# tenpy/cyten

Measured on AMD Instinct MI355X. Metric: block-sparse tdot+SVD GFLOP/s (fp64), higher is better.
Workload: dtype f64

## Files before the change

### cyten_amd/csrc/blocked_qr.hip

```cpp
#include "blocked_qr.h"

#include <algorithm>
#include <cstdlib>
#include <utility>

namespace cyb {
namespace {

#define GLOBAL_AS __attribute__((address_space(1)))
typedef GLOBAL_AS double* gp;
typedef const GLOBAL_AS double* gcp;
typedef double d4 __attribute__((ext_vector_type(4)));

constexpr int PNT = 512;
constexpr int PNW = PNT / 64;

__device__ __forceinline__ double wave_sum(double v)
{
#pragma unroll
    for (int o = 32; o > 0; o >>= 1) v += __shfl_xor(v, o);
    return v;
}

struct PanelDesc {
// ... 866 lines not shown
            if (tid == 0) {
                __builtin_amdgcn_fence(__ATOMIC_RELEASE, "agent");
                __hip_atomic_store(la_flags + (d.next_off - 1), la_tag, __ATOMIC_RELAXED, __HIP_MEMORY_SCOPE_AGENT);
            }
        }
    }
    if constexpr (FUSE_PANEL) {
        __shared__ PanelShared psh;
        if (d.next_off) {
            __syncthreads();
            const PanelDesc pd = *reinterpret_cast<const PanelDesc*>(reinterpret_cast<const char*>(descs) + d.next_off);
            panel_reg_body<RP_RPT_FUSED>(pd, psh, tid);
        }
    }
}

struct ChunkDesc {
    double* C;
    const double* V;
    const double* T;
    double* wpart;
    int64_t ldc, ldv;
    int32_t mr, nc, pw, transT;
    int32_t slot, n_slots, row0, step;
    const double* ctl;
    double* part_out;
};

__global__ void __launch_bounds__(ST_NT) strip_w1_kernel(const ChunkDesc* __restrict__ descs)
{
    __shared__ double part[ST_NW][NBK][ST_LS];
    const ChunkDesc d = descs[blockIdx.x];
    if (d.ctl) {
        const double stopped = *(gcp)d.ctl;
        if (stopped != 0.0 && (double)d.step >= stopped - 1.0) return;
    }
    const int tid = threadIdx.x, lane = tid & 63, wave = tid >> 6;
    const int x = lane & 15, kq = lane >> 4;
    gcp V = (gcp)d.V;
    gp C = (gp)d.C;
    const int mr = d.mr, nc = d.nc, pw = d.pw;
    const int64_t ldv = d.ldv, ldc = d.ldc;
    {
        const int64_t vo0 = (int64_t)(x < pw ? x : 0) * ldv, vo1 = (int64_t)(x + 16 < pw ? x + 16 : 0) * ldv;
        const int64_t co0 = (int64_t)(x < nc ? x : 0) * ldc, co1 = (int64_t)(x + 16 < nc ? x + 16 : 0) * ldc;
        d4 acc[2][2];
#pragma unroll
        for (int i = 0; i < 2; ++i)
#pragma unroll
            for (int j = 0; j < 2; ++j) acc[i][j] = d4{0.0, 0.0, 0.0, 0.0};
        const int nstep = (mr + 7) / 8;
        double va[ST_UN][2][2], ca[ST_UN][2][2], vn[ST_UN][2][2], cn[ST_UN][2][2];
        auto load = [&](double (&v)[ST_UN][2][2], double (&c)[ST_UN][2][2], int s0) {
#pragma unroll
            for (int u = 0; u < ST_UN; ++u) {
                const int i = (s0 + ST_NW * u) * 8 + 2 * kq;
#pragma unroll
                for (int h = 0; h < 2; ++h) {
                    const bool ok = i + h < mr;
                    const int ii = ok ? i + h : 0;
                    v[u][0][h] = ok ? V[vo0 + ii] : 0.0;
                    v[u][1][h] = ok ? V[vo1 + ii] : 0.0;
                    c[u][0][h] = ok ? C[co0 + ii] : 0.0;
                    c[u][1][h] = ok ? C[co1 + ii] : 0.0;
                }
            }
        };
        if (wave < nstep) load(va, ca, wave);
        for (int s0 = wave; s0 < nstep; s0 += ST_NW * ST_UN) {
            const bool more = s0 + ST_NW * ST_UN < nstep;
            if (more) load(vn, cn, s0 + ST_NW * ST_UN);
#pragma unroll
            for (int u = 0; u < ST_UN; ++u) {
                if (s0 + ST_NW * u < nstep) {
#pragma unroll
                    for (int h = 0; h < 2; ++h)
#pragma unroll
                        for (int i = 0; i < 2; ++i)
#pragma unroll
                            for (int j = 0; j < 2; ++j)
                                acc[i][j] = __builtin_amdgcn_mfma_f64_16x16x4f64(va[u][i][h], ca[u][j][h], acc[i][j], 0, 0, 0);
                }
            }
            if (more) {
#pragma unroll
                for (int u = 0; u < ST_UN; ++u)
#pragma unroll
                    for (int i = 0; i < 2; ++i)
#pragma unroll
                        for (int h = 0; h < 2; ++h) {
                            va[u][i][h] = vn[u][i][h];
                            ca[u][i][h] = cn[u][i][h];
                        }
            }
        }
#pragma unroll
        for (int i = 0; i < 2; ++i)
#pragma unroll
            for (int j = 0; j < 2; ++j)
#pragma unroll
                for (int r = 0; r < 4; ++r) part[wave][i * 16 + kq + 4 * r][j * 16 + x] = acc[i][j][r];
    }
    __syncthreads();
    gp out = (gp)d.wpart + (size_t)d.slot * (NBK * NBK);
    for (int e = tid; e < NBK * NBK; e += ST_NT) {
        const int a = e / NBK, c = e % NBK;
        double t = 0.0;
#pragma unroll
        for (int w = 0; w < ST_NW; ++w) t += part[w][a][c];
        out[e] = t;
    }
}

template <bool NORM>
__global__ void __launch_bounds__(ST_NT) strip_apply_kernel(const ChunkDesc* __restrict__ descs)
{
    __shared__ double W1s[NBK][ST_LS], W2s[NBK][ST_LS], Ps[NBK][ST_LS];
    const ChunkDesc d = descs[blockIdx.x];
    if (d.ctl) {
        const double stopped = *(gcp)d.ctl;
        if (stopped != 0.0 && (double)d.step >= stopped - 1.0) return;
    }
    const int tid = threadIdx.x, lane = tid & 63, wave = tid >> 6;
    const int x = lane & 15, kq = lane >> 4;
    gcp V = (gcp)d.V;
    gp C = (gp)d.C;
    gcp T = (gcp)d.T;
    const int mr = d.mr, nc = d.nc, pw = d.pw;
    const int64_t ldv = d.ldv, ldc = d.ldc;
    gcp wp = (gcp)d.wpart;
    for (int e = tid; e < NBK * NBK; e += ST_NT) {
        const int a = e / NBK, b = e % NBK;
        Ps[a][b] = T[d.transT ? b * NBK + a : e];
        double t = 0.0;
        for (int sl = 0; sl < d.n_slots; ++sl) t += wp[(size_t)sl * (NBK * NBK) + e];
        W1s[a][b] = t;
    }
    __syncthreads();
    if (wave < 4) {
        const int ta = wave >> 1, tc = wave & 1;
        d4 acc = d4{0.0, 0.0, 0.0, 0.0};
#pragma unroll
        for (int kk = 0; kk < NBK / 4; ++kk)
            acc = __builtin_amdgcn_mfma_f64_16x16x4f64(Ps[ta * 16 + x][4 * kk + kq], W1s[4 * kk + kq][tc * 16 + x], acc, 0, 0, 0);
#pragma unroll
        for (int r = 0; r < 4; ++r) W2s[ta * 16 + kq + 4 * r][tc * 16 + x] = acc[r];
    }
    __syncthreads();
    {
        double w2[2][NBK / 4];
#pragma unroll
        for (int ct = 0; ct < 2; ++ct)
#pragma unroll
            for (int kk = 0; kk < NBK / 4; ++kk) w2[ct][kk] = -W2s[4 * kk + kq][ct * 16 + x];
        int64_t vcol[NBK / 4], ccol[2][4];
#pragma unroll
        for (int kk = 0; kk < NBK / 4; ++kk) vcol[kk] = (int64_t)(4 * kk + kq < pw ? 4 * kk + kq : 0) * ldv;
#pragma unroll
        for (int ct = 0; ct < 2; ++ct)
#pragma unroll
            for (int r = 0; r < 4; ++r) {
                const int c = ct * 16 + kq + 4 * r;
                ccol[ct][r] = (int64_t)(c < nc ? c : 0) * ldc;
            }
        const int ntile = (mr + 15) / 16;
        struct Tile {
            double v[NBK / 4];
            d4 c[2];
        };
        auto load = [&](Tile& t, int rt) {
            const int i = rt * 16 + x;
            const bool ok = i < mr;
            const int ii = ok ? i : 0;
#pragma unroll
            for (int kk = 0; kk < NBK / 4; ++kk) t.v[kk] = ok ? V[vcol[kk] + ii] : 0.0;
#pragma unroll
            for (int ct = 0; ct < 2; ++ct)
#pragma unroll
                for (int r = 0; r < 4; ++r) t.c[ct][r] = C[ccol[ct][r] + ii];
        };
        double nrm2 = 0.0;
        auto finish = [&](Tile& t, int rt) {
#pragma unroll
            for (int kk = 0; kk < NBK / 4; ++kk) {
                t.c[0] = __builtin_amdgcn_mfma_f64_16x16x4f64(w2[0][kk], t.v[kk], t.c[0], 0, 0, 0);
                t.c[1] = __builtin_amdgcn_mfma_f64_16x16x4f64(w2[1][kk], t.v[kk], t.c[1], 0, 0, 0);
            }
            const int i = rt * 16 + x;
            if (i < mr) {
                const double below = i + d.row0 >= pw ? 1.0 : 0.0;
#pragma unroll
                for (int ct = 0; ct < 2; ++ct)
#pragma unroll
                    for (int r = 0; r < 4; ++r)
                        if (ct * 16 + kq + 4 * r < nc) {
                            C[ccol[ct][r] + i] = t.c[ct][r];
                            if constexpr (NORM) nrm2 = fma(below * t.c[ct][r], t.c[ct][r], nrm2);
                        }
            }
        };
        Tile t0, t1, t2;
        if (wave < ntile) load(t0, wave);
        if (wave + ST_NW < ntile) load(t1, wave + ST_NW);
        for (int rt = wave; rt < ntile; rt += 3 * ST_NW) {
            if (rt + 2 * ST_NW < ntile) load(t2, rt + 2 * ST_NW);
            finish(t0, rt);
            if (rt + ST_NW < ntile) {
                if (rt + 3 * ST_NW < ntile) load(t0, rt + 3 * ST_NW);
                finish(t1, rt + ST_NW);
            }
            if (rt + 2 * ST_NW < ntile) {
                if (rt + 4 * ST_NW < ntile) load(t1, rt + 4 * ST_NW);
                finish(t2, rt + 2 * ST_NW);
            }
        }
        if constexpr (NORM) if (d.part_out) {
#pragma unroll
            for (int o = 32; o > 0; o >>= 1) nrm2 += __shfl_xor(nrm2, o);
            __syncthreads();
            if (lane == 0) W1s[0][wave] = nrm2;
            __syncthreads();
            if (tid == 0) {
                double t = 0.0;
#pragma unroll
                for (int w = 0; w < ST_NW; ++w) t += W1s[0][w];
                *(gp)d.part_out = t;
            }
        }
    }
}

struct MergeDesc {
    const double* G;
    const double* T;
    double* TS;
    int64_t g_stride;
    int32_t w, W, n_gp, pad;
};
constexpr int MG_NT = 256;
template <int AMAX>
__global__ void __launch_bounds__(MG_NT) merge_t_kernel(const MergeDesc* __restrict__ descs)
{
    constexpr bool TS_LDS = AMAX <= 96;
    __shared__ double Gs[AMAX][NBK + 1], X[AMAX][NBK + 1];
    __shared__ double Tb[NBK][NBK + 1];
    __shared__ double TSs[TS_LDS ? AMAX : 1][TS_LDS ? AMAX + 1 : 1];
    const MergeDesc d = descs[blockIdx.x];
    const int tid = threadIdx.x;
    const int W = d.W, w = d.w;
    gcp G = (gcp)d.G;
    gcp T = (gcp)d.T;
    gp TS = (gp)d.TS;
    for (int e = tid; e < W * W; e += MG_NT) {
        const int r = e / W, c = e % W;
        double v = 0.0;
        if (r / NBK == c / NBK && r < w && c < w) v = T[(size_t)(r / NBK) * (NBK * NBK) + (r % NBK) * NBK + (c % NBK)];
        TS[e] = v;
        if constexpr (TS_LDS)
            if (r < AMAX && c < AMAX) TSs[r][c] = v;
    }
    const int nb = (w + NBK - 1) / NBK;
    for (int b = 1; b < nb; ++b) {
        const int a = b * NBK, wb = min(NBK, w - a);
        __syncthreads();
        for (int e = tid; e < NBK * NBK; e += MG_NT) Tb[e / NBK][e % NBK] = T[(size_t)b * (NBK * NBK) + e];
        for (int e = tid; e < a * NBK; e += MG_NT) {
            const int i = e / NBK, l = e % NBK;
            double g = 0.0;
            if (l < wb)
                for (int p = 0; p < d.n_gp; ++p) g += G[(size_t)p * d.g_stride + (size_t)i * W + a + l];
            Gs[i][l] = g;
        }
        __syncthreads();
        for (int e = tid; e < a * NBK; e += MG_NT) {
            const int i = e / NBK, c = e % NBK;
            double acc = 0.0;
#pragma unroll
            for (int l = 0; l < NBK; ++l) acc += Gs[i][l] * Tb[l][c];
            X[i][c] = acc;
        }
        __syncthreads();
        for (int e = tid; e < a * NBK; e += MG_NT) {
            const int i = e / NBK, c = e % NBK;
            double acc = 0.0;
            if constexpr (TS_LDS) {
                for (int l = i; l < a; ++l) acc += TSs[i][l] * X[l][c];
            } else {
                for (int l = i; l < a; ++l) acc += TS[(size_t)i * W + l] * X[l][c];
            }
            if (c < wb) {
                TS[(size_t)i * W + a + c] = -acc;
                if constexpr (TS_LDS)
                    if (a + c < AMAX) TSs[i][a + c] = -acc;
            }
        }
    }
}

struct SumDesc {
    double* W1;
    int64_t n, stride;
    int32_t ns, pad;
};
__global__ void __launch_bounds__(256) sum_partials_kernel(const SumDesc* __restrict__ descs)
{
    const SumDesc d = descs[blockIdx.y];
    gp W1 = (gp)d.W1;
    for (int64_t e = (int64_t)blockIdx.x * 256 + threadIdx.x; e < d.n; e += (int64_t)gridDim.x * 256) {
        double t = W1[e];
        for (int sidx = 1; sidx < d.ns; ++sidx) t += W1[e + (int64_t)sidx * d.stride];
        W1[e] = t;
    }
}

inline size_t al256(size_t b) { return (b + 255) / 256 * 256; }

__global__ void __launch_bounds__(256) xpose_kernel(const XposeDesc* __restrict__ descs)
{
    __shared__ double tile[32][33];
    const XposeDesc d = descs[blockIdx.y];
    gcp in = (gcp)d.in;
    gp out = (gp)d.out;
    const int tx = threadIdx.x & 31, ty = threadIdx.x >> 5;
    if (d.plain) {
        const int64_t tot = (int64_t)d.R * d.C;
        for (int64_t e = (int64_t)blockIdx.x * 256 + threadIdx.x; e < tot; e += (int64_t)gridDim.x * 256) {
            const int64_t r = e / d.C, c = e % d.C;
            out[r * d.ldo + c] = in[r * d.ldi + c];
        }
        return;
    }
    const int tr = (d.R + 31) / 32, tc = (d.C + 31) / 32;
    for (int t = blockIdx.x; t < tr * tc; t += gridDim.x) {
        const int r0 = (t / tc) * 32, c0 = (t % tc) * 32;
        __syncthreads();
#pragma unroll
        for (int q = 0; q < 4; ++q) {
            const int c = c0 + ty + 8 * q, r = r0 + tx;
            tile[ty + 8 * q][tx] = (c < d.C && r < d.R) ? in[(int64_t)c * d.ldi + r] : 0.0;
        }
        __syncthreads();
#pragma unroll
        for (int q = 0; q < 4; ++q) {
            const int r = r0 + ty + 8 * q, c = c0 + tx;
            if (r < d.R && c < d.C) {
                double v = tile[tx][ty + 8 * q];
                if (d.upper && (r > c || r >= d.rlim)) v = 0.0;
                out[(int64_t)r * d.ldo + c] = v;
            }
        }
    }
}

__global__ void __launch_bounds__(256) eye_cols_kernel(const EyeDesc* __restrict__ descs)
{
    const EyeDesc d = descs[blockIdx.y];
    gp C = (gp)d.C;
    const int64_t tot = (int64_t)d.m * d.kc;
    for (int64_t e = (int64_t)blockIdx.x * 256 + threadIdx.x; e < tot; e += (int64_t)gridDim.x * 256) {
        const int64_t c = e / d.m, i = e % d.m;
        C[c * d.ld + i] = (i == c + d.col0) ? 1.0 : 0.0;
    }
}

}

int xpose_batched(cyb_ctx_t ctx, const std::vector<XposeDesc>& descs)
{
    if (descs.empty()) return CYB_OK;
    void* d = nullptr;
    CYB_TRY(ctx->upload(descs.data(), sizeof(XposeDesc) * descs.size(), &d));
    hipLaunchKernelGGL(xpose_kernel, dim3(helper_grid_x(descs.size()), (unsigned)descs.size()), dim3(256), 0, ctx->stream, static_cast<const XposeDesc*>(d));
    CYB_HIP(hipGetLastError());
    return CYB_OK;
}

int eye_cols_batched(cyb_ctx_t ctx, const std::vector<EyeDesc>& descs)
{
    if (descs.empty()) return CYB_OK;
    void* d = nullptr;
    CYB_TRY(ctx->upload(descs.data(), sizeof(EyeDesc) * descs.size(), &d));
    hipLaunchKernelGGL(eye_cols_kernel, dim3(64, (unsigned)descs.size()), dim3(256), 0, ctx->stream, static_cast<const EyeDesc*>(d));
    CYB_HIP(hipGetLastError());
    return CYB_OK;
}

constexpr int kWSplit = 8;
static inline int w_split(int64_t mr)
{
    static const int env = getenv("CYB_QR_WSPLIT") ? atoi(getenv("CYB_QR_WSPLIT")) : 0;
    if (env > 0) return (int)std::min<int64_t>(std::min(env, kWSplit), std::max<int64_t>(1, (mr + 255) / 256));
    return mr >= 2600 ? 4 : mr >= 1800 ? 3 : mr >= 700 ? 2 : 1;
}

static inline bool use_strips()
{
    static const bool off = getenv("CYB_QR_GEMM_UPDATE") != nullptr;
    return !off;
}
static void add_strips(std::vector<StripDesc>& out, double* C, int64_t ldc, int64_t ncols, const double* V, int64_t ldv,
                       const double* T, int64_t mr, int pw, int transT, int64_t next_tag = -1)
{
    for (int64_t c0 = 0; c0 < ncols; c0 += NBK)
        out.push_back(StripDesc{C + (size_t)c0 * ldc, V, T, ldc, ldv, (int32_t)mr, (int32_t)std::min<int64_t>(NBK, ncols - c0), pw, transT,
                                c0 == 0 && next_tag >= 0 ? next_tag + 1 : 0});
}
static void sort_strips(std::vector<StripDesc>& v)
{
    std::stable_sort(v.begin(), v.end(), [](const StripDesc& a, const StripDesc& b) { return a.mr > b.mr; });
}

constexpr int kChunkRowsMin = 192;
static const int kChunkRowsChoices[] = {192, 256, 384, 512, 768, 1024, 1536};
static int strip_split_mode()
{
    static const int v = getenv("CYB_QR_CHUNK_ROWS") ? atoi(getenv("CYB_QR_CHUNK_ROWS")) : -1;
    return v < 0 ? -1 : v / 16 * 16;
}
int bqr_strip_slots(int64_t rows)
{
    if (strip_split_mode() == 0) return 1;
    const int ch = strip_split_mode() > 0 ? std::min(strip_split_mode(), kChunkRowsMin) : kChunkRowsMin;
    return (int)std::max<int64_t>(1, (rows + ch - 1) / ch);
}
static int strip_chunk_share(int mr, int ch)
{
    if (ch <= 0 || mr <= ch) return std::max(mr, 1);
    const int ns = (mr + ch - 1) / ch;
    return ((mr + ns - 1) / ns + 15) / 16 * 16;
}
static int strip_chunks(int mr, int ch)
{
    const int share = strip_chunk_share(mr, ch);
    return std::max(1, (mr + share - 1) / share);
}
static int choose_chunk_rows(const std::vector<std::pair<int, int>>& strips, int n_cu)
{
    const int mode = strip_split_mode();
    if (mode == 0) return 0;
    if (mode > 0) return mode;
    int64_t n_strips = 0;
    for (const auto& s : strips) n_strips += s.second;
    if (n_strips == 0 || n_strips * 4 > (int64_t)n_cu * 3) return 0;
    static const int ch_min = getenv("CYB_QR_CHUNK_MIN") ? atoi(getenv("CYB_QR_CHUNK_MIN")) : kChunkRowsMin;
    for (int ch : kChunkRowsChoices) {
        if (ch < ch_min) continue;
        int64_t tot = 0;
        bool any = false;
        for (const auto& s : strips) {
            const int c = strip_chunks(s.first, ch);
            tot += (int64_t)c * s.second;
            any = any || c > 1;
        }
        if (tot <= n_cu) return any ? ch : 0;
    }
    return 0;
}
static void make_chunks(const std::vector<StripDesc>& sd, double* wbase, int ch, std::vector<ChunkDesc>& out)
{
    out.clear();
    size_t slot_base = 0;
    for (const StripDesc& d : sd) {
        const int share = strip_chunk_share(d.mr, ch), nch = strip_chunks(d.mr, ch);
        for (int sl = 0; sl < nch; ++sl) {
            const int r0 = sl * share;
            out.push_back(ChunkDesc{d.C + r0, d.V + r0, d.T, wbase + slot_base * (size_t)(NBK * NBK), d.ldc, d.ldv, std::min(share, d.mr - r0), d.nc, d.pw,
                                    d.transT, sl, nch, r0, d.step, d.ctl, d.part_out ? d.part_out + sl : nullptr});
        }
        slot_base += (size_t)nch;
    }
}

static int wide_mode()
{
    static const int v = getenv("CYB_QR_APPLY_WIDE") ? (atoi(getenv("CYB_QR_APPLY_WIDE")) != 0 ? 1 : 0) : -1;
    return v;
}
static int wide_width()
{
    static const int v = [] {
        const int e = getenv("CYB_QR_APPLY_WIDTH") ? atoi(getenv("CYB_QR_APPLY_WIDTH")) : 128;
        return (e == 64 || e == 256) ? e : 128;
    }();
    return v;
}
constexpr int64_t kWideMinK = 256, kWideMinKc = 256, kWideMinCols = 4096;
static bool wide_target(const BqrMat& q, const BqrTarget& t)
{
    const int mode = wide_mode();
    if (mode == 0 || q.k <= NBK || t.kc <= 0) return false;
    if (q.ctl && q.stop_rel2 > 0.0 && t.n_pan < 0) return false;
    if (mode == 1) return true;
    return q.k >= kWideMinK && t.kc >= kWideMinKc;
}
static size_t scratch_doubles(int64_t m, int64_t n, int64_t kc)
{
    const size_t strips = (size_t)(1 + kWSplit) * NBK * (size_t)std::max<int64_t>(std::max(n, kc), 1);
    const size_t wide = (size_t)w_split(m) * (size_t)wide_width() * (size_t)std::max<int64_t>(kc, 1);
    return std::max(strips, wide);
}

size_t bqr_aux_bytes(int64_t m, int64_t n, int64_t ld, int64_t kc)
{
    const int64_t k = std::min(m, n);
    const int64_t npan = (k + NBK - 1) / NBK;
    return al256(sizeof(double) * (size_t)ld * (size_t)std::max<int64_t>(k, 1)) + al256(sizeof(double) * (size_t)npan * NBK * NBK) +
           al256(sizeof(double) * (size_t)std::max<int64_t>(k, 1)) + al256(sizeof(double) * scratch_doubles(m, n, kc));
}

size_t bqr_carve(BqrMat& q, char* base, int64_t kc)
{
    const int64_t k = q.k;
    const int64_t npan = (k + NBK - 1) / NBK;
    size_t off = 0;
    q.V = reinterpret_cast<double*>(base + off);
    off += al256(sizeof(double) * (size_t)q.ld * (size_t)std::max<int64_t>(k, 1));
    q.T = reinterpret_cast<double*>(base + off);
    off += al256(sizeof(double) * (size_t)npan * NBK * NBK);
    q.tau = reinterpret_cast<double*>(base + off);
    off += al256(sizeof(double) * (size_t)std::max<int64_t>(k, 1));
    q.scratch = reinterpret_cast<double*>(base + off);
    q.scr_half = (int64_t)NBK * std::max<int64_t>(std::max<int64_t>(q.n, kc), 1);
    q.scr_total = (int64_t)scratch_doubles(q.m, q.n, kc);
    off += al256(sizeof(double) * (size_t)q.scr_total);
    return off;
}

int bqr_factor(cyb_ctx_t ctx, const std::vector<BqrMat>& mats)
{
    auto pflags = [](const BqrMat& q) { return (q.v_zeroed ? PANEL_V_ZEROED : 0) | (q.reflect_always ? PANEL_REFLECT_ALWAYS : 0); };
    int max_pan = 0;
    for (const auto& q : mats) max_pan = std::max(max_pan, (q.k + NBK - 1) / NBK);
    static const bool want_la = getenv("CYB_QR_LOOKAHEAD") != nullptr;
    hipStream_t side = nullptr;
    const bool strips = use_strips();
    const bool lookahead = !strips && want_la && max_pan >= 6 && ctx->aux(&side) == CYB_OK;
    struct Step {
        size_t off_pd = 0, off_pdr = 0;
        unsigned n_pd = 0, n_pdr = 0;
        GemmStaged s1, s3;
        GemmStaged r1, r3;
        bool has_rest = false;
        size_t off_sd = 0;
        unsigned n_sd = 0;
        bool fused = false;
        bool norm = false;
        unsigned n_la = 0;
        size_t off_pn = 0;
        size_t off_cd = 0;
        unsigned n_cd = 0;
        int wave = 0;
        size_t off_pdm = 0;
        unsigned n_pdm = 0;
    };
    std::vector<Step> steps;
    std::vector<char> image;
    auto put = [&image](const void* src, size_t bytes) {
        const size_t off = (image.size() + 255) / 256 * 256;
        image.resize(off + bytes);
        memcpy(image.data() + off, src, bytes);
        return off;
    };
    static const bool no_fuse = getenv("CYB_QR_FUSE") == nullptr;
    static const int fuse_rows = getenv("CYB_QR_FUSE_ROWS") ? atoi(getenv("CYB_QR_FUSE_ROWS")) : 768;
    std::vector<char> fused(mats.size(), 0);
    static const bool la_on = getenv("CYB_QR_LA") && atoi(getenv("CYB_QR_LA")) != 0;
    static const int la_min_rows = getenv("CYB_QR_LA_MIN") ? atoi(getenv("CYB_QR_LA_MIN")) : 4 * RP_WAVE_ROWS;
    unsigned int* la_flags = nullptr;
    const int la_err = (int)mats.size();
    bool la_used = false;
    static const bool no_multi = getenv("CYB_QR_NOMULTI") != nullptr;
    std::vector<size_t> x_off(mats.size(), 0);
    size_t x_bytes = 0, n_multi_wg = 0;
    const size_t t_bytes = (sizeof(unsigned int) * NBK * mats.size() + 255) / 256 * 256;
    for (size_t qi = 0; qi < mats.size(); ++qi) {
        const int wmax = (mats[qi].m + RPM_ROWS - 1) / RPM_ROWS;
        if (mats[qi].m > RPM_ROWS && std::min(mats[qi].m, mats[qi].n) > 0) {
            x_off[qi] = t_bytes + 256 + x_bytes;
            x_bytes += sizeof(double) * NBK * (size_t)wmax * 64;
            n_multi_wg += (size_t)wmax;
        }
    }
    const bool multi = !no_multi && x_bytes > 0 && n_multi_wg <= (size_t)ctx->n_cu;
    char* xbase = nullptr;
    bool la_any = false;
    if (la_on && use_strips())
        for (const auto& q : mats) la_any = la_any || (q.k > NBK && q.m - NBK > la_min_rows);
    if (multi || la_any) {
        const size_t x_total = multi ? (t_bytes + 256 + x_bytes + 255) / 256 * 256 : 0;
        void* xw = nullptr;
        CYB_TRY(ctx->workspace(x_total + 256 + sizeof(unsigned int) * (mats.size() + 1), &xw, 3));
        xbase = static_cast<char*>(xw);
        if (multi) CYB_HIP(hipMemsetAsync(xbase + t_bytes, 0, 256, ctx->stream));
        if (la_any) {
            la_flags = reinterpret_cast<unsigned int*>(xbase + x_total);
            CYB_HIP(hipMemsetAsync(la_flags, 0, sizeof(unsigned int) * (mats.size() + 1), ctx->stream));
        }
    }
    const bool multi_ok = multi;
    static const bool no_stop = getenv("CYB_QR_NOSTOP") != nullptr;
    static const bool no_reg_g = getenv("CYB_QR_PANEL_GLOBAL") != nullptr;
    auto stoppable = [&](const BqrMat& q) {
        return !no_stop && strips && !no_reg_g && q.ctl && q.parts && q.stop_rel2 > 0.0 && (q.m <= RP_NT * RP_RPT || multi_ok);
    };
    const bool split = strips && strip_split_mode() != 0 && no_fuse && !la_on;
    double* wsplit = nullptr;
    if (split) {
        size_t n_ch = 0;
        for (const auto& q : mats) n_ch += (size_t)((q.n + NBK - 1) / NBK) * (size_t)bqr_strip_slots(q.m);
        void* w = nullptr;
        CYB_TRY(ctx->workspace(sizeof(double) * NBK * NBK * std::max<size_t>(n_ch, 1), &w, 4));
        wsplit = static_cast<double*>(w);
    }
    std::vector<int> n_parts_prev(mats.size(), 0);
    static const int stop_every = std::max(1, getenv("CYB_QR_STOP_EVERY") ? atoi(getenv("CYB_QR_STOP_EVERY")) : 2);
    bool all_done = false;
    int last_rest = -1;
    const int side_cu = ctx->n_cu - (ctx->n_cu + 15) / 16;
    int chunk = lookahead ? max_pan : 2;
    for (int c0 = 0; c0 < max_pan && !all_done; c0 += chunk, chunk *= 3) {
    const int c1 = std::min(max_pan, c0 + chunk);
    steps.clear();
    image.clear();
    for (int p = c0; p < c1; ++p) {
        std::vector<PanelDesc> pd, pd_reg, pd_next;
        std::vector<PanelDescM> pdm;
        std::vector<StripDesc> sd;
        GemmBatch g1, g3, h1, h3;
        int n_active = 0;
        int max_m = 0;
        for (const auto& q : mats)
            if (p * NBK < q.k) max_m = std::max(max_m, q.m);
        const bool step_fuse = !no_fuse && max_m <= fuse_rows;
        const bool step_la = la_on && strips && !step_fuse && la_flags != nullptr;
        bool step_has_la = false;
        bool step_norm = false;
        int step_ch = 0;
        if (split && !step_fuse) {
            std::vector<std::pair<int, int>> cnt;
            for (const auto& q : mats) {
                const int j0 = p * NBK;
                if (j0 >= q.k) continue;
                const int64_t nt = q.n - (j0 + std::min(NBK, q.k - j0));
                if (nt > 0) cnt.push_back({q.m - j0, (int)((nt + NBK - 1) / NBK)});
            }
            step_ch = choose_chunk_rows(cnt, ctx->n_cu);
        }
        for (size_t qi = 0; qi < mats.size(); ++qi) {
            const auto& q = mats[qi];
            const int j0 = p * NBK;
            if (j0 >= q.k) continue;
            ++n_active;
            const int pw = std::min(NBK, q.k - j0);
            static const bool no_reg = getenv("CYB_QR_PANEL_GLOBAL") != nullptr;
            if (fused[qi]) fused[qi] = 0;
            else if (!no_reg && q.m - j0 <= RP_NT * RP_RPT) {
                pd_reg.push_back(PanelDesc{q.Ac, q.V, q.T + (size_t)p * NBK * NBK, q.tau, q.ld, q.m, j0, pw, pflags(q)});
                if (stoppable(q)) {
                    PanelDesc& d = pd_reg.back();
                    d.ctl = q.ctl;
                    d.parts = q.parts;
                    d.rel2 = q.stop_rel2;
                    d.n_parts = n_parts_prev[qi];
                    d.step = p;
                }
            } else if (multi && !no_reg) {
                const int n_wg = (q.m - j0 + RPM_ROWS - 1) / RPM_ROWS;
                for (int w = 0; w < n_wg; ++w)
                {
                    pdm.push_back(PanelDescM{q.Ac, q.V, q.T + (size_t)p * NBK * NBK, q.tau, reinterpret_cast<double*>(xbase + x_off[qi]),
                                             reinterpret_cast<unsigned int*>(xbase) + qi * NBK, reinterpret_cast<unsigned int*>(xbase + t_bytes),
                                             q.ld, q.m, j0, pw, pflags(q), w, n_wg, 0, 0});
                    if (stoppable(q)) {
                        PanelDescM& d = pdm.back();
                        d.ctl = q.ctl;
                        d.parts = q.parts;
                        d.rel2 = q.stop_rel2;
                        d.n_parts = n_parts_prev[qi];
                        d.step = p;
                    }
                }
            } else
                pd.push_back(PanelDesc{q.Ac, q.V, q.T + (size_t)p * NBK * NBK, q.tau, q.ld, q.m, j0, pw, pflags(q) & PANEL_REFLECT_ALWAYS});
            const int j1 = j0 + pw;
            const int64_t nt = q.n - j1, mr = q.m - j0;
// ... 106 lines not shown
            CYB_TRY(h3.stage(ctx, image, st.r3));
            st.has_rest = true;
        }
        steps.push_back(st);
    }
    if (steps.empty()) break;
    void* d_image = nullptr;
    CYB_TRY(ctx->upload(image.data(), image.size(), &d_image));
    char* dbase = static_cast<char*>(d_image);
    if (lookahead) CYB_TRY(ctx->events(2 * steps.size()));
    for (size_t p = 0; p < steps.size(); ++p) {
        const Step& st = steps[p];
        if (st.n_pd)
            hipLaunchKernelGGL(qr_panel_kernel, dim3(st.n_pd), dim3(PNT), 0, ctx->stream,
                               reinterpret_cast<const PanelDesc*>(dbase + st.off_pd));
        if (st.n_pdm) {
            CYB_HIP(hipMemsetAsync(xbase, 0, t_bytes, ctx->stream));
            hipLaunchKernelGGL(qr_panel_multi_kernel, dim3(st.n_pdm), dim3(RP_NT), 0, ctx->stream,
                               reinterpret_cast<const PanelDescM*>(dbase + st.off_pdm));
        }
        if (st.n_pdr && st.wave == 1)
            hipLaunchKernelGGL(qr_panel_wave_kernel, dim3(st.n_pdr), dim3(64), 0, ctx->stream,
                               reinterpret_cast<const PanelDesc*>(dbase + st.off_pdr));
        else if (st.n_pdr && st.wave == 2)
            hipLaunchKernelGGL(qr_panel_wave2_kernel, dim3(st.n_pdr), dim3(128), 0, ctx->stream,
                               reinterpret_cast<const PanelDesc*>(dbase + st.off_pdr));
        else if (st.n_pdr && st.wave == 4)
            hipLaunchKernelGGL(qr_panel_wave4_kernel, dim3(st.n_pdr), dim3(256), 0, ctx->stream,
                               reinterpret_cast<const PanelDesc*>(dbase + st.off_pdr));
        else if (st.n_pdr)
            hipLaunchKernelGGL(qr_panel_reg_kernel, dim3(st.n_pdr), dim3(RP_NT), 0, ctx->stream,
                               reinterpret_cast<const PanelDesc*>(dbase + st.off_pdr));
        CYB_HIP(hipGetLastError());
        if (lookahead && st.has_rest) {
            hipEvent_t evP = ctx->ev_pool[2 * p], evR = ctx->ev_pool[2 * p + 1];
            CYB_HIP(hipEventRecord(evP, ctx->stream));
            CYB_HIP(hipStreamWaitEvent(side, evP, 0));
            CYB_TRY(gemm_launch_staged(ctx, st.r1, d_image, side, side_cu));
            CYB_TRY(gemm_launch_staged(ctx, st.r3, d_image, side, side_cu));
            CYB_HIP(hipEventRecord(evR, side));
            if (last_rest >= 0) CYB_HIP(hipStreamWaitEvent(ctx->stream, ctx->ev_pool[2 * (size_t)last_rest + 1], 0));
            last_rest = (int)p;
        } else if (lookahead && last_rest >= 0) {
            CYB_HIP(hipStreamWaitEvent(ctx->stream, ctx->ev_pool[2 * (size_t)last_rest + 1], 0));
            last_rest = -1;
        }
        if (st.n_sd) {
            const StripDesc* sdp = reinterpret_cast<const StripDesc*>(dbase + st.off_sd);
            const PanelDesc* pnp = reinterpret_cast<const PanelDesc*>(dbase + st.off_pn);
            const unsigned la_tag = (unsigned)(c0 + (int)p + 1);
            const PanelDesc* no_pn = nullptr;
            unsigned int* no_fl = nullptr;
            if (st.n_cd) {
                const ChunkDesc* cdp = reinterpret_cast<const ChunkDesc*>(dbase + st.off_cd);
                hipLaunchKernelGGL(strip_w1_kernel, dim3(st.n_cd), dim3(ST_NT), 0, ctx->stream, cdp);
                if (st.norm) hipLaunchKernelGGL(strip_apply_kernel<true>, dim3(st.n_cd), dim3(ST_NT), 0, ctx->stream, cdp);
                else hipLaunchKernelGGL(strip_apply_kernel<false>, dim3(st.n_cd), dim3(ST_NT), 0, ctx->stream, cdp);
            } else if (st.n_la && st.norm)
                hipLaunchKernelGGL((reflector_strip_kernel<false, true, true>), dim3(st.n_sd + st.n_la), dim3(ST_NT), 0, ctx->stream, sdp,
                                   (int)st.n_sd, pnp, la_flags, la_tag, la_err);
            else if (st.n_la)
                hipLaunchKernelGGL((reflector_strip_kernel<false, false, true>), dim3(st.n_sd + st.n_la), dim3(ST_NT), 0, ctx->stream, sdp,
                                   (int)st.n_sd, pnp, la_flags, la_tag, la_err);
            else if (st.fused)
                hipLaunchKernelGGL(reflector_strip_kernel<true>, dim3(st.n_sd), dim3(ST_NT), 0, ctx->stream, sdp, (int)st.n_sd, no_pn, no_fl, 0u, 0);
            else if (st.norm)
                hipLaunchKernelGGL((reflector_strip_kernel<false, true>), dim3(st.n_sd), dim3(ST_NT), 0, ctx->stream, sdp, (int)st.n_sd, no_pn, no_fl, 0u, 0);
            else
                hipLaunchKernelGGL(reflector_strip_kernel<false>, dim3(st.n_sd), dim3(ST_NT), 0, ctx->stream, sdp, (int)st.n_sd, no_pn, no_fl, 0u, 0);
            CYB_HIP(hipGetLastError());
        }
        CYB_TRY(gemm_launch_staged(ctx, st.s1, d_image));
        CYB_TRY(gemm_launch_staged(ctx, st.s3, d_image));
    }
    }
    if (last_rest >= 0) CYB_HIP(hipStreamWaitEvent(ctx->stream, ctx->ev_pool[2 * (size_t)last_rest + 1], 0));
    if (la_used) {
        unsigned int h_err = 0;
        CYB_HIP(hipMemcpyAsync(&h_err, la_flags + la_err, sizeof(unsigned int), hipMemcpyDeviceToHost, ctx->stream));
        CYB_HIP(hipStreamSynchronize(ctx->stream));
        if (h_err) {
            set_error("blocked QR: a look-ahead panel workgroup waited more than a second for its strip");
            return CYB_ERR_HIP;
        }
    }
    if (multi) {
        unsigned int h_err = 0;
        CYB_HIP(hipMemcpyAsync(&h_err, xbase + t_bytes, sizeof(unsigned int), hipMemcpyDeviceToHost, ctx->stream));
        CYB_HIP(hipStreamSynchronize(ctx->stream));
        if (h_err) {
            set_error("blocked QR: a workgroup of the multi-workgroup panel kernel waited more than a second for its partners");
            return CYB_ERR_HIP;
        }
    }
    return CYB_OK;
}

static int apply_q_strips(cyb_ctx_t ctx, const std::vector<BqrMat>& mats, const std::vector<BqrTarget>& targets)
{
    int max_pan = 0;
    for (const auto& t : targets) max_pan = std::max(max_pan, (mats[(size_t)t.mat].k + NBK - 1) / NBK);
    const bool strips = use_strips();
    struct Step {
        GemmStaged s1, s3;
        size_t off_sd = 0;
        unsigned n_sd = 0;
        size_t off_cd = 0;
        unsigned n_cd = 0;
    };
    const bool split = strips && strip_split_mode() != 0;
    double* wsplit = nullptr;
    if (split) {
        size_t n_ch = 0;
        for (const auto& t : targets) n_ch += (size_t)((t.kc + NBK - 1) / NBK) * (size_t)bqr_strip_slots(mats[(size_t)t.mat].m);
        void* w = nullptr;
        CYB_TRY(ctx->workspace(sizeof(double) * NBK * NBK * std::max<size_t>(n_ch, 1), &w, 4));
        wsplit = static_cast<double*>(w);
    }
    std::vector<Step> steps;
    std::vector<char> image;
    int chunk = 2;
    for (int c0 = max_pan - 1; c0 >= 0; c0 -= chunk, chunk *= 3) {
    const int c1 = std::max(-1, c0 - chunk);
    steps.clear();
    image.clear();
    for (int p = c0; p > c1; --p) {
        GemmBatch g1, g3;
        std::vector<StripDesc> sd;
        for (const auto& t : targets) {
            const BqrMat& q = mats[(size_t)t.mat];
            const int j0 = p * NBK;
            if (j0 >= q.k || t.kc <= 0) continue;
            const int pw = std::min(NBK, q.k - j0);
            const int64_t mr = q.m - j0;
            double* W1 = q.scratch + q.scr_half;
            CYB_REQUIRE((int64_t)NBK * t.kc <= q.scr_half, "bqr_apply_q: target wider than the carved scratch");
            const double* Vp = q.V + (size_t)j0 * q.ld + j0;
            double* Ct = t.C + j0;
            const double* Tp = q.T + (size_t)p * NBK * NBK;
            if (strips) {
                const size_t s_begin = sd.size();
                add_strips(sd, Ct, t.ldc, t.kc, Vp, q.ld, Tp, mr, pw, 0);
                if (q.ctl && q.stop_rel2 > 0.0)
                    for (size_t si = s_begin; si < sd.size(); ++si) {
                        sd[si].ctl = q.ctl;
                        sd[si].step = p;
                    }
                continue;
            }
            const int ns = w_split(mr);
            const int64_t chunk = ((mr + ns - 1) / ns + 15) / 16 * 16;
            const int32_t seg0 = (int32_t)g3.segs.size();
            for (int sidx = 0; sidx < ns; ++sidx) {
                const int64_t r0 = chunk * sidx, rows = std::min(chunk, mr - r0);
                if (rows <= 0) break;
                double* W2s = W1 + (size_t)sidx * q.scr_half;
                g1.add_post(W2s, pw, t.kc, t.kc, Vp + r0, q.ld, 1, Ct + r0, 1, t.ldc, rows, 1.0, 0.0, Tp, NBK, 1);
                g3.segs.push_back(cyb_gemm_seg{W2s, Vp, pw, 1, t.kc, q.ld, 1});
            }
            g3.probs.push_back(cyb_gemm_prob{Ct, t.kc, mr, t.ldc, seg0, (int32_t)g3.segs.size(), -1.0, 1.0});
        }
        if (g1.empty() && sd.empty()) continue;
        Step st;
        if (!g1.empty()) {
            CYB_TRY(g1.stage(ctx, image, st.s1));
            CYB_TRY(g3.stage(ctx, image, st.s3));
        }
        if (!sd.empty()) {
            sort_strips(sd);
            st.n_sd = (unsigned)sd.size();
            const size_t off = (image.size() + 255) / 256 * 256;
            image.resize(off + sizeof(StripDesc) * sd.size());
            memcpy(image.data() + off, sd.data(), sizeof(StripDesc) * sd.size());
            st.off_sd = off;
            std::vector<std::pair<int, int>> cnt;
            for (const auto& d : sd) cnt.push_back({d.mr, 1});
            const int step_ch = split ? choose_chunk_rows(cnt, ctx->n_cu) : 0;
            if (step_ch > 0) {
                std::vector<ChunkDesc> cd;
                make_chunks(sd, wsplit, step_ch, cd);
                st.n_cd = (unsigned)cd.size();
                const size_t offc = (image.size() + 255) / 256 * 256;
                image.resize(offc + sizeof(ChunkDesc) * cd.size());
                memcpy(image.data() + offc, cd.data(), sizeof(ChunkDesc) * cd.size());
                st.off_cd = offc;
            }
        }
        steps.push_back(st);
    }
    if (steps.empty()) continue;
    void* d_image = nullptr;
    CYB_TRY(ctx->upload(image.data(), image.size(), &d_image));
    for (const auto& st : steps) {
        if (st.n_cd) {
            const ChunkDesc* cdp = reinterpret_cast<const ChunkDesc*>(static_cast<char*>(d_image) + st.off_cd);
            hipLaunchKernelGGL(strip_w1_kernel, dim3(st.n_cd), dim3(ST_NT), 0, ctx->stream, cdp);
            hipLaunchKernelGGL(strip_apply_kernel<false>, dim3(st.n_cd), dim3(ST_NT), 0, ctx->stream, cdp);
            CYB_HIP(hipGetLastError());
        } else if (st.n_sd) {
            hipLaunchKernelGGL(reflector_strip_kernel<false>, dim3(st.n_sd), dim3(ST_NT), 0, ctx->stream,
                               reinterpret_cast<const StripDesc*>(static_cast<char*>(d_image) + st.off_sd), (int)st.n_sd,
                               static_cast<const PanelDesc*>(nullptr), static_cast<unsigned int*>(nullptr), 0u, 0);
            CYB_HIP(hipGetLastError());
        }
        CYB_TRY(gemm_launch_staged(ctx, st.s1, d_image));
        CYB_TRY(gemm_launch_staged(ctx, st.s3, d_image));
    }
    }
    return CYB_OK;
}

static int apply_q_wide(cyb_ctx_t ctx, const std::vector<BqrMat>& mats, const std::vector<BqrTarget>& targets)
{
    const int W = wide_width();
    struct Tgt {
        const BqrMat* q;
        const BqrTarget* t;
        int k_eff, ng;
        double* VT;
        double* TS;
        double* G;
        std::vector<int> n_gp;
    };
    std::vector<Tgt> tg;
    size_t bytes = 0;
    int max_ng = 0;
    for (const auto& t : targets) {
        const BqrMat& q = mats[(size_t)t.mat];
        const int npan = (q.k + NBK - 1) / NBK;
        const int nf = t.n_pan >= 0 ? std::min(npan, (int)t.n_pan) : npan;
        const int k_eff = std::min<int>(q.k, nf * NBK);
        if (k_eff <= 0 || t.kc <= 0) continue;
        Tgt g{&q, &t, k_eff, (k_eff + W - 1) / W, nullptr, nullptr, nullptr, {}};
        CYB_REQUIRE((int64_t)w_split(q.m) * W * t.kc <= q.scr_total, "bqr_apply_q: target wider than the carved scratch");
        for (int s = 0; s < g.ng; ++s) {
            const int j0 = s * W, w = std::min(W, k_eff - j0);
            const int min_rows = q.m - j0 - (w - 1) / NBK * NBK;
            g.n_gp.push_back(std::max(1, std::min(4, min_rows / 256)));
        }
        max_ng = std::max(max_ng, g.ng);
        tg.push_back(std::move(g));
    }
    if (tg.empty()) return CYB_OK;
    std::vector<size_t> o_vt(tg.size()), o_ts(tg.size()), o_g(tg.size());
    for (size_t i = 0; i < tg.size(); ++i) {
        size_t n_g = 0;
        for (int n : tg[i].n_gp) n_g += (size_t)n;
        o_vt[i] = bytes;
        bytes += al256(sizeof(double) * (size_t)tg[i].q->ld * (size_t)tg[i].k_eff);
        o_ts[i] = bytes;
        bytes += al256(sizeof(double) * (size_t)tg[i].ng * W * W);
        o_g[i] = bytes;
        bytes += al256(sizeof(double) * n_g * W * W);
    }
    void* ws = nullptr;
    CYB_TRY(ctx->workspace(bytes, &ws, 5));
    for (size_t i = 0; i < tg.size(); ++i) {
        tg[i].VT = reinterpret_cast<double*>(static_cast<char*>(ws) + o_vt[i]);
        tg[i].TS = reinterpret_cast<double*>(static_cast<char*>(ws) + o_ts[i]);
        tg[i].G = reinterpret_cast<double*>(static_cast<char*>(ws) + o_g[i]);
    }
    std::vector<char> image;
    {
        GemmBatch gg, gv;
        std::vector<MergeDesc> md;
        for (const Tgt& g : tg) {
            const BqrMat& q = *g.q;
            size_t gp0 = 0;
            for (int s = 0; s < g.ng; ++s) {
                const int j0 = s * W, w = std::min(W, g.k_eff - j0), n_gp = g.n_gp[(size_t)s];
                const double* Vs = q.V + (size_t)j0 * q.ld + j0;
                double* Gs = g.G + gp0 * (size_t)W * W;
                double* TSs = g.TS + (size_t)s * W * W;
                for (int a = NBK; a < w; a += NBK) {
                    const int wb = std::min(NBK, w - a);
                    const int64_t rows = q.m - j0 - a, chunk = (rows + n_gp - 1) / n_gp;
                    for (int p = 0; p < n_gp; ++p) {
                        const int64_t r0 = a + chunk * p, kr = std::min(chunk, rows - chunk * p);
                        gg.add(Gs + (size_t)p * W * W + a, a, wb, W, Vs + r0, q.ld, 1, Vs + (size_t)a * q.ld + r0, 1, q.ld, kr, 1.0, 0.0);
                    }
                }
                md.push_back(MergeDesc{Gs, q.T + (size_t)(j0 / NBK) * NBK * NBK, TSs, (int64_t)W * W, w, W, n_gp, 0});
                gv.add(g.VT + (size_t)j0 * q.ld + j0, w, q.m - j0, q.ld, TSs, 1, W, Vs, q.ld, 1, w, 1.0, 0.0);
                gp0 += (size_t)n_gp;
            }
        }
        GemmStaged sg, sv;
        CYB_TRY(gg.stage(ctx, image, sg));
        CYB_TRY(gv.stage(ctx, image, sv));
        const size_t off_md = (image.size() + 255) / 256 * 256;
        image.resize(off_md + sizeof(MergeDesc) * md.size());
        memcpy(image.data() + off_md, md.data(), sizeof(MergeDesc) * md.size());
        void* d_image = nullptr;
        CYB_TRY(ctx->upload(image.data(), image.size(), &d_image));
        CYB_TRY(gemm_launch_staged(ctx, sg, d_image));
        const MergeDesc* mdp = reinterpret_cast<const MergeDesc*>(static_cast<char*>(d_image) + off_md);
        if (W <= 128) hipLaunchKernelGGL(merge_t_kernel<96>, dim3((unsigned)md.size()), dim3(MG_NT), 0, ctx->stream, mdp);
        else hipLaunchKernelGGL(merge_t_kernel<224>, dim3((unsigned)md.size()), dim3(MG_NT), 0, ctx->stream, mdp);
        CYB_HIP(hipGetLastError());
        CYB_TRY(gemm_launch_staged(ctx, sv, d_image));
    }
    struct Step {
        GemmStaged s1, s2;
        size_t off_sum = 0;
        unsigned n_sum = 0;
    };
    std::vector<Step> steps;
    int chunk = 2;
    for (int c0 = max_ng - 1; c0 >= 0; c0 -= chunk, chunk *= 3) {
        const int c1 = std::max(-1, c0 - chunk);
        steps.clear();
        image.clear();
        for (int s = c0; s > c1; --s) {
            GemmBatch g1, g2;
            std::vector<SumDesc> sums;
            for (const Tgt& g : tg) {
                if (s >= g.ng) continue;
                const BqrMat& q = *g.q;
                const BqrTarget& t = *g.t;
                const int j0 = s * W, w = std::min(W, g.k_eff - j0);
                const int64_t mr = q.m - j0;
                const double* Vs = q.V + (size_t)j0 * q.ld + j0;
                const double* VTs = g.VT + (size_t)j0 * q.ld + j0;
                double* Ct = t.C + j0;
                const int ns = w_split(mr);
                const int64_t rch = ((mr + ns - 1) / ns + 15) / 16 * 16;
                const int64_t stride = (int64_t)W * t.kc;
                int n_part = 0;
                for (int sidx = 0; sidx < ns; ++sidx) {
                    const int64_t r0 = rch * sidx, rows = std::min(rch, mr - r0);
                    if (rows <= 0) break;
                    g1.add(q.scratch + (size_t)sidx * (size_t)stride, w, t.kc, t.kc, Vs + r0, q.ld, 1, Ct + r0, 1, t.ldc, rows, 1.0, 0.0);
                    ++n_part;
                }
                if (n_part > 1) sums.push_back(SumDesc{q.scratch, (int64_t)w * t.kc, stride, n_part, 0});
                g2.add(Ct, t.kc, mr, t.ldc, q.scratch, 1, t.kc, VTs, q.ld, 1, w, -1.0, 1.0);
            }
            if (g1.empty()) continue;
            Step st;
            CYB_TRY(g1.stage(ctx, image, st.s1));
            CYB_TRY(g2.stage(ctx, image, st.s2));
            if (!sums.empty()) {
                st.n_sum = (unsigned)sums.size();
                st.off_sum = (image.size() + 255) / 256 * 256;
                image.resize(st.off_sum + sizeof(SumDesc) * sums.size());
                memcpy(image.data() + st.off_sum, sums.data(), sizeof(SumDesc) * sums.size());
            }
            steps.push_back(st);
        }
        if (steps.empty()) continue;
        void* d_image = nullptr;
        CYB_TRY(ctx->upload(image.data(), image.size(), &d_image));
        for (const auto& st : steps) {
            CYB_TRY(gemm_launch_staged(ctx, st.s1, d_image));
            if (st.n_sum) {
                hipLaunchKernelGGL(sum_partials_kernel, dim3(helper_grid_x(st.n_sum), st.n_sum), dim3(256), 0, ctx->stream,
                                   reinterpret_cast<const SumDesc*>(static_cast<char*>(d_image) + st.off_sum));
                CYB_HIP(hipGetLastError());
            }
            CYB_TRY(gemm_launch_staged(ctx, st.s2, d_image));
        }
    }
    return CYB_OK;
}

int bqr_apply_q(cyb_ctx_t ctx, const std::vector<BqrMat>& mats, const std::vector<BqrTarget>& targets)
{
    std::vector<BqrTarget> narrow, wide;
    for (const auto& t : targets) (wide_target(mats[(size_t)t.mat], t) ? wide : narrow).push_back(t);
    int64_t cols = 0;
    for (const auto& t : wide) cols += t.kc;
    if (wide_mode() < 0 && cols < kWideMinCols) {
        narrow = targets;
        wide.clear();
    }
    if (!narrow.empty()) CYB_TRY(apply_q_strips(ctx, mats, narrow));
    if (!wide.empty()) CYB_TRY(apply_q_wide(ctx, mats, wide));
    return CYB_OK;
}

}
```

### cyten_amd/csrc/common.h

```cpp
#pragma once
#include <hip/hip_runtime.h>
#include <cstdarg>
#include <cstdint>
#include <cstdio>
#include <cstring>
#include <string>
#include <initializer_list>
#include <vector>

#include "../../include/cyten_amd.h"

namespace cyb {

void set_error(const char* fmt, ...);

#define CYB_HIP(call)                                                                   \
    do {                                                                                \
        hipError_t _e = (call);                                                         \
        if (_e != hipSuccess) {                                                         \
            cyb::set_error("%s failed: %s (%s:%d)", #call, hipGetErrorString(_e),       \
                           __FILE__, __LINE__);                                         \
            return CYB_ERR_HIP;                                                         \
        }                                                                               \
    } while (0)

#define CYB_REQUIRE(cond, ...)                                                          \
    do {                                                                                \
        if (!(cond)) {                                                                  \
            cyb::set_error(__VA_ARGS__);                                                \
            return CYB_ERR_INVALID;                                                     \
        }                                                                               \
    } while (0)

#define CYB_TRY(call)                                                                   \
    do {                                                                                \
        int _s = (call);                                                                \
        if (_s != CYB_OK) return _s;                                                    \
    } while (0)

}

struct cyb_ctx_s {
    int device = 0;
    hipStream_t stream = nullptr;
    int n_cu = 256;
    int lds_bytes = 160 * 1024;
    int64_t hbm_bytes = 0;
    char arch[64] = {0};

    static constexpr int kSlots = 32;
    static constexpr int kEvStride = 8;
    struct Slot {
        void* dev = nullptr;
        void* host = nullptr;
        size_t cap = 0;
        hipEvent_t ev = nullptr;
        hipEvent_t copied = nullptr;
        bool ev_valid = false;
    };
    hipStream_t copy_stream = nullptr;
    hipStream_t aux_stream = nullptr;
    int aux_state = 0;
    std::vector<hipEvent_t> ev_pool;
    int aux(hipStream_t* out);
    int events(size_t n);
    Slot slots[kSlots];
    uint64_t n_uploads = 0;
    uint64_t ev_waited = 0;
    static constexpr size_t kBigBytes = 128 * 1024;
    static constexpr int kBig = 8;
    Slot big[kBig];
    uint64_t n_big = 0;
    size_t slot_cap_max = 0;

    int upload(const void* src, size_t bytes, void** dev_out);

    static constexpr int kWork = 7;
    void* work[kWork] = {nullptr, nullptr, nullptr, nullptr, nullptr, nullptr, nullptr};
    size_t work_cap[kWork] = {0, 0, 0, 0, 0, 0, 0};
    int workspace(size_t bytes, void** out, int slot = 0);
    static constexpr size_t kReadback = 64 * 1024;
    void* readback = nullptr;
    int d2h(void* dst, const void* src, size_t bytes);
    hipEvent_t time_start = nullptr, time_stop = nullptr;
};

namespace cyb {
struct UploadPart {
    const void* src;
    size_t bytes;
    void** out;
};
inline int upload_packed(cyb_ctx_t ctx, std::initializer_list<UploadPart> parts)
{
    size_t tot = 0;
    for (const auto& p : parts) tot = (tot + 255) / 256 * 256 + p.bytes;
    if (tot == 0) {
        for (const auto& p : parts) *p.out = nullptr;
        return CYB_OK;
    }
    std::vector<char> img(tot);
    size_t off = 0;
    for (const auto& p : parts) {
        off = (off + 255) / 256 * 256;
        if (p.bytes) memcpy(img.data() + off, p.src, p.bytes);
        off += p.bytes;
    }
    void* d = nullptr;
    int rc = ctx->upload(img.data(), tot, &d);
    if (rc != CYB_OK) return rc;
    off = 0;
    for (const auto& p : parts) {
        off = (off + 255) / 256 * 256;
        *p.out = p.bytes ? static_cast<char*>(d) + off : nullptr;
        off += p.bytes;
    }
    return CYB_OK;
}
}

namespace cyb {
struct GemmPost {
    const double* L;
    int64_t rs, cs;
};
int gemm_launch_async(cyb_ctx_t ctx, const cyb_gemm_prob* probs, int64_t n_probs, const cyb_gemm_seg* segs, int64_t n_segs,
                      const GemmPost* post = nullptr);

struct GemmStaged {
    size_t offset = 0;
    size_t off_p = 0, off_s = 0, off_t = 0, off_c = 0;
    int64_t n_tiles = 0;
};
int gemm_stage(cyb_ctx_t ctx, const cyb_gemm_prob* probs, int64_t n_probs, const cyb_gemm_seg* segs, int64_t n_segs,
               const GemmPost* post, std::vector<char>& image, GemmStaged& st);
int gemm_launch_staged(cyb_ctx_t ctx, const GemmStaged& st, void* dev_image, hipStream_t stream = nullptr, int n_cu = 0);

struct GemmBatch {
    std::vector<cyb_gemm_prob> probs;
    std::vector<cyb_gemm_seg> segs;
    std::vector<GemmPost> post;
    void add(double* C, int64_t M, int64_t N, int64_t ldc, const double* A, int64_t a_rs, int64_t a_cs, const double* B,
             int64_t b_rs, int64_t b_cs, int64_t K, double alpha, double beta)
    {
        if (M <= 0 || N <= 0) return;
        cyb_gemm_seg s{A, B, K, a_rs, a_cs, b_rs, b_cs};
        cyb_gemm_prob p{C, M, N, ldc, (int32_t)segs.size(), (int32_t)segs.size() + 1, alpha, beta};
        segs.push_back(s);
        probs.push_back(p);
    }
    void add_post(double* C, int64_t M, int64_t N, int64_t ldc, const double* A, int64_t a_rs, int64_t a_cs, const double* B,
                  int64_t b_rs, int64_t b_cs, int64_t K, double alpha, double beta, const double* L, int64_t l_rs, int64_t l_cs)
    {
        if (M <= 0 || N <= 0) return;
        post.resize(probs.size(), GemmPost{nullptr, 0, 0});
        add(C, M, N, ldc, A, a_rs, a_cs, B, b_rs, b_cs, K, alpha, beta);
        post.push_back(GemmPost{L, l_rs, l_cs});
    }
    int launch(cyb_ctx_t ctx)
    {
        if (!post.empty()) post.resize(probs.size(), GemmPost{nullptr, 0, 0});
        return gemm_launch_async(ctx, probs.data(), (int64_t)probs.size(), segs.data(), (int64_t)segs.size(),
                                 post.empty() ? nullptr : post.data());
    }
    int stage(cyb_ctx_t ctx, std::vector<char>& image, GemmStaged& st)
    {
        if (!post.empty()) post.resize(probs.size(), GemmPost{nullptr, 0, 0});
        return gemm_stage(ctx, probs.data(), (int64_t)probs.size(), segs.data(), (int64_t)segs.size(),
                          post.empty() ? nullptr : post.data(), image, st);
    }
    bool empty() const { return probs.empty(); }
};
}

namespace cyb {
struct MatRef {
    const double* A;
    int64_t lda, m, n;
};
struct ScaleJob {
    const double* src;
    int64_t lds;
    double* dst;
    int64_t ldd, rows, cols;
    double s;
};
int matrix_amax(cyb_ctx_t ctx, const std::vector<MatRef>& mats, std::vector<double>& amax);
double range_scale(double amax);
int scale_copy_batched(cyb_ctx_t ctx, const std::vector<ScaleJob>& jobs);
inline unsigned helper_grid_x(size_t n_lists)
{
    const size_t g = 2048 / (n_lists ? n_lists : 1);
    return (unsigned)(g < 64 ? 64 : (g > 512 ? 512 : g));
}

}

static inline int64_t cdiv64(int64_t a, int64_t b) { return (a + b - 1) / b; }
```

### cyten_amd/csrc/scaling.hip

```cpp
#include "common.h"

#include <algorithm>
#include <cmath>

namespace cyb {
namespace {

#define GLOBAL_AS __attribute__((address_space(1)))
typedef const GLOBAL_AS double* gcp;
typedef GLOBAL_AS double* gp;

struct AmaxDesc {
    const double* A;
    int64_t lda;
    int32_t m, n;
    double* out;
};

__global__ void __launch_bounds__(256) matrix_amax_kernel(const AmaxDesc* __restrict__ descs)
{
    __shared__ double red[4];
    const AmaxDesc d = descs[blockIdx.y];
    gcp A = (gcp)d.A;
    double mx = 0.0;
    bool bad = false;
    if (d.lda == d.n) {
        const int64_t tot = (int64_t)d.m * d.n;
        for (int64_t e = (int64_t)blockIdx.x * 256 + threadIdx.x; e < tot; e += (int64_t)gridDim.x * 256) {
            const double v = A[e];
            bad = bad || !(fabs(v) <= 1.7e308);
            mx = fmax(mx, fabs(v));
        }
    } else {
        for (int r = blockIdx.x; r < d.m; r += gridDim.x) {
            gcp row = A + (int64_t)r * d.lda;
            for (int c = threadIdx.x; c < d.n; c += 256) {
                const double v = row[c];
                bad = bad || !(fabs(v) <= 1.7e308);
                mx = fmax(mx, fabs(v));
            }
        }
    }
    if (bad) mx = __builtin_nan("");
#pragma unroll
    for (int o = 32; o > 0; o >>= 1) {
        const double other = __shfl_xor(mx, o);
        mx = (mx != mx || other != other) ? __builtin_nan("") : fmax(mx, other);
    }
    if ((threadIdx.x & 63) == 0) red[threadIdx.x >> 6] = mx;
    __syncthreads();
    if (threadIdx.x == 0) {
        double r = red[0];
        for (int w = 1; w < 4; ++w) r = (r != r || red[w] != red[w]) ? __builtin_nan("") : fmax(r, red[w]);
        ((gp)d.out)[blockIdx.x] = r;
    }
}

struct ScaleDesc {
    const double* src;
    int64_t lds;
    double* dst;
    int64_t ldd;
    int32_t rows, cols;
    double s;
};

__global__ void __launch_bounds__(256) scale_copy_kernel(const ScaleDesc* __restrict__ descs)
{
    const ScaleDesc d = descs[blockIdx.y];
    gcp src = (gcp)d.src;
    gp dst = (gp)d.dst;
    const int64_t tot = (int64_t)d.rows * d.cols;
    for (int64_t e = (int64_t)blockIdx.x * 256 + threadIdx.x; e < tot; e += (int64_t)gridDim.x * 256) {
        const int64_t r = e / d.cols, c = e % d.cols;
        dst[r * d.ldd + c] = src[r * d.lds + c] * d.s;
    }
}

}

int matrix_amax(cyb_ctx_t ctx, const std::vector<MatRef>& mats, std::vector<double>& amax)
{
    const size_t n = mats.size();
    amax.assign(n, 0.0);
    if (n == 0) return CYB_OK;
    constexpr int kParts = 32;
    void* d_out = nullptr;
    CYB_TRY(ctx->workspace(sizeof(double) * n * kParts, &d_out, 2));
    std::vector<AmaxDesc> ds(n);
    for (size_t i = 0; i < n; ++i)
        ds[i] = AmaxDesc{mats[i].A, mats[i].lda, (int32_t)mats[i].m, (int32_t)mats[i].n, static_cast<double*>(d_out) + i * kParts};
    void* d_ds = nullptr;
    CYB_TRY(ctx->upload(ds.data(), sizeof(AmaxDesc) * n, &d_ds));
    hipLaunchKernelGGL(matrix_amax_kernel, dim3(kParts, (unsigned)n), dim3(256), 0, ctx->stream, static_cast<const AmaxDesc*>(d_ds));
    CYB_HIP(hipGetLastError());
    std::vector<double> parts(n * kParts);
    CYB_TRY(ctx->d2h(parts.data(), d_out, sizeof(double) * parts.size()));
    for (size_t i = 0; i < n; ++i) {
        double r = 0.0;
        for (int p = 0; p < kParts; ++p) {
            const double v = parts[i * kParts + p];
            r = (r != r || v != v) ? std::nan("") : std::max(r, v);
        }
        amax[i] = r;
    }
    return CYB_OK;
}

double range_scale(double amax)
{
    if (!(amax > 0.0) || !(amax <= 1.7e308)) return 1.0;
    if (amax <= 1e90 && amax >= 1e-90) return 1.0;
    int e = 0;
    (void)std::frexp(amax, &e);
    return std::ldexp(1.0, -e);
}

int scale_copy_batched(cyb_ctx_t ctx, const std::vector<ScaleJob>& jobs)
{
    if (jobs.empty()) return CYB_OK;
    std::vector<ScaleDesc> ds(jobs.size());
    for (size_t i = 0; i < jobs.size(); ++i)
        ds[i] = ScaleDesc{jobs[i].src, jobs[i].lds, jobs[i].dst, jobs[i].ldd, (int32_t)jobs[i].rows, (int32_t)jobs[i].cols, jobs[i].s};
    void* d_ds = nullptr;
    CYB_TRY(ctx->upload(ds.data(), sizeof(ScaleDesc) * ds.size(), &d_ds));
    hipLaunchKernelGGL(scale_copy_kernel, dim3(64, (unsigned)ds.size()), dim3(256), 0, ctx->stream, static_cast<const ScaleDesc*>(d_ds));
    CYB_HIP(hipGetLastError());
    return CYB_OK;
}

}
```

### cyten_amd/csrc/svd_jacobi.hip

```cpp
#include "blocked_qr.h"
#include "jacobi_engine.h"

#include <algorithm>
#include <cmath>
#include <cstdlib>

namespace cyb {
namespace {

#define GLOBAL_AS __attribute__((address_space(1)))
typedef GLOBAL_AS double* gp;
typedef const GLOBAL_AS double* gcp;

struct PrepDesc {
    const double* A;
    int64_t lda;
    int32_t m, n;
    double* W;
    double* J;
    int32_t nvp, lenp;
    int32_t transpose;
    int32_t pad;
    const double* shift;
};

__global__ void __launch_bounds__(256) prep_kernel(const PrepDesc* __restrict__ descs)
{
    __shared__ double tile[32][33];
    const PrepDesc d = descs[blockIdx.y];
    gcp A = (gcp)d.A;
    gp W = (gp)d.W;
    const int tx = threadIdx.x & 31, ty = threadIdx.x >> 5;
    const int tiles_n = (d.n + 31) / 32, tiles_m = (d.m + 31) / 32;
    const double shift = d.shift ? *(gcp)d.shift : 0.0;
    for (int t = blockIdx.x; t < tiles_m * tiles_n; t += gridDim.x) {
        const int ti = t / tiles_n, tj = t % tiles_n;
        const int i0 = ti * 32, j0 = tj * 32;
        if (d.transpose) {
#pragma unroll
            for (int r = 0; r < 4; ++r) {
                const int i = i0 + ty + 8 * r, j = j0 + tx;
                tile[ty + 8 * r][tx] = (i < d.m && j < d.n) ? A[(int64_t)i * d.lda + j] : 0.0;
            }
            __syncthreads();
#pragma unroll
            for (int r = 0; r < 4; ++r) {
                const int j = j0 + ty + 8 * r, i = i0 + tx;
                if (j < d.n && i < d.m) W[(int64_t)j * d.lenp + i] = tile[tx][ty + 8 * r];
            }
            __syncthreads();
        } else {
#pragma unroll
            for (int r = 0; r < 4; ++r) {
                const int i = i0 + ty + 8 * r, j = j0 + tx;
                if (i < d.m && j < d.n) {
                    double v = A[(int64_t)i * d.lda + j];
                    if (i == j) v += shift;
                    W[(int64_t)i * d.lenp + j] = v;
                }
            }
        }
    }
    if (d.J) {
        gp J = (gp)d.J;
        for (int i = blockIdx.x * 256 + threadIdx.x; i < d.nvp; i += gridDim.x * 256) J[(int64_t)i * d.nvp + i] = 1.0;
    }
}

struct NormDesc {
    const double* A;
    int64_t lda;
    int32_t m, n;
    double* out;
};
__global__ void __launch_bounds__(256) fro_shift_kernel(const NormDesc* __restrict__ descs)
{
    __shared__ double red[4];
    const NormDesc d = descs[blockIdx.x];
    gcp A = (gcp)d.A;
    double s = 0.0;
    const int64_t tot = (int64_t)d.m * d.n;
    for (int64_t e = threadIdx.x; e < tot; e += 256) {
        const double v = A[(e / d.n) * d.lda + (e % d.n)];
        s += v * v;
    }
#pragma unroll
    for (int o = 32; o > 0; o >>= 1) s += __shfl_xor(s, o);
    if ((threadIdx.x & 63) == 0) red[threadIdx.x >> 6] = s;
    __syncthreads();
    if (threadIdx.x == 0) {
        const double f = sqrt(red[0] + red[1] + red[2] + red[3]);
        *(gp)d.out = (f > 0.0) ? 2.0 * f : 1.0;
    }
}

struct PostDesc {
    const double* W;
    const double* J;
    int32_t nvp, lenp, nv, len;
    int32_t transposed;
    int32_t mode;
    double* sig;
    int32_t* rank;
    double* S;
    double* U;
    int64_t ldu;
    double* Vh;
    int64_t ldvh;
    const double* shift;
    double* scratch;
    int32_t* n_null;
    double null_scale;
    int32_t cplx = 0;
    int32_t pad_ = 0;
    const double* sig_lq = nullptr;
};

__global__ void __launch_bounds__(256) row_norm_kernel(const PostDesc* __restrict__ descs)
{
    const PostDesc d = descs[blockIdx.y];
    gcp W = (gcp)d.W;
    const int lane = threadIdx.x & 63;
    for (int j = blockIdx.x * 4 + (threadIdx.x >> 6); j < d.nv; j += gridDim.x * 4) {
        double s = 0.0;
        for (int c = lane; c < d.len; c += 64) {
            const double v = W[(int64_t)j * d.lenp + c];
            s += v * v;
        }
#pragma unroll
        for (int o = 32; o > 0; o >>= 1) s += __shfl_xor(s, o);
        if (lane == 0) {
            const double o = d.sig_lq ? ((gcp)d.sig_lq)[j] : 0.0;
            ((gp)d.sig)[j] = (o > 0.0 && s > 0.0) ? o : sqrt(s);
        }
    }
}

__global__ void __launch_bounds__(256) rank_kernel(const PostDesc* __restrict__ descs)
{
    constexpr int CH = 2048;
    __shared__ double keys[CH];
    const PostDesc d = descs[blockIdx.y];
    gcp sig = (gcp)d.sig;
    const double shift = d.shift ? *(gcp)d.shift : 0.0;
    const int msk = d.cplx ? ~1 : ~0;
    const int per = (d.nv + (int)gridDim.x * 256 - 1) / ((int)gridDim.x * 256);
    for (int it = 0; it < per; ++it) {
        const int j = (it * (int)gridDim.x + (int)blockIdx.x) * 256 + (int)threadIdx.x;
        const bool mine = j < d.nv;
        const double sj = mine ? sig[j & msk] : 0.0;
        int r = 0;
        for (int k0 = 0; k0 < d.nv; k0 += CH) {
            const int kn = min(CH, d.nv - k0);
            __syncthreads();
            for (int k = threadIdx.x; k < kn; k += 256) keys[k] = sig[(k0 + k) & msk];
            __syncthreads();
            if (mine) {
                if (d.mode == 0) {
                    for (int k = 0; k < kn; ++k) {
                        const double sk = keys[k];
                        r += (sk > sj || (sk == sj && k0 + k < j)) ? 1 : 0;
                    }
                } else {
                    for (int k = 0; k < kn; ++k) {
                        const double sk = keys[k];
                        r += (sk < sj || (sk == sj && k0 + k < j)) ? 1 : 0;
                    }
                }
            }
        }
        if (mine) {
            d.rank[j] = r;
            d.S[r] = (d.mode == 0) ? sj : sj - shift;
        }
    }
}

__global__ void __launch_bounds__(256) write_factors_kernel(const PostDesc* __restrict__ descs)
{
    __shared__ double tile[32][33];
    __shared__ int rk[32];
    __shared__ double sc[32];
    const PostDesc d = descs[blockIdx.y];
    gcp W = (gcp)d.W;
    gcp J = (gcp)d.J;
    const int tx = threadIdx.x & 31, ty = threadIdx.x >> 5;
    double smax = 0.0;
    if (d.mode == 0) smax = ((gcp)d.S)[0];
    const double thresh = fmax(smax * 1e-280, 1e-300);

    const bool col_from_W = (d.mode == 1) || d.transposed;
    gcp csrc = col_from_W ? W : J;
    const int csrc_ld = col_from_W ? d.lenp : d.nvp;
    const int c_rows = col_from_W ? d.len : d.nv;
    gcp rsrc = col_from_W ? J : W;
    const int rsrc_ld = col_from_W ? d.nvp : d.lenp;
    const int r_cols = col_from_W ? d.nv : d.len;

    const int tj = (d.nv + 31) / 32;
    if (d.U) {
        const int ti_n = (c_rows + 31) / 32;
        for (int t = blockIdx.x; t < tj * ti_n; t += gridDim.x) {
            const int j0 = (t / ti_n) * 32, i0 = (t % ti_n) * 32;
            __syncthreads();
            if (threadIdx.x < 32) {
                const int j = j0 + threadIdx.x;
                double s = 1.0;
                int r = 0;
                if (j < d.nv) {
                    r = d.rank[j];
                    if (col_from_W) {
                        const double sj = ((gcp)d.sig)[j];
                        s = (d.mode == 0 && sj <= thresh) ? d.null_scale : 1.0 / sj;
                    }
                }
                rk[threadIdx.x] = r;
                sc[threadIdx.x] = s;
            }
            __syncthreads();
#pragma unroll
            for (int q = 0; q < 4; ++q) {
                const int j = j0 + ty + 8 * q, i = i0 + tx;
                tile[ty + 8 * q][tx] = (j < d.nv && i < c_rows) ? csrc[(int64_t)j * csrc_ld + i] * sc[ty + 8 * q] : 0.0;
            }
            __syncthreads();
#pragma unroll
            for (int q = 0; q < 4; ++q) {
                const int i = i0 + ty + 8 * q, j = j0 + tx;
                if (i < c_rows && j < d.nv) ((gp)d.U)[(int64_t)i * d.ldu + rk[tx]] = tile[tx][ty + 8 * q];
            }
        }
    }
    if (d.mode == 0 && d.Vh) {
        for (int j = blockIdx.x; j < d.nv; j += gridDim.x) {
            const int r = d.rank[j];
            double s = 1.0;
            if (!col_from_W) {
                const double sj = ((gcp)d.sig)[j];
                s = (sj <= thresh) ? d.null_scale : 1.0 / sj;
            }
            for (int c = threadIdx.x; c < r_cols; c += 256)
                ((gp)d.Vh)[(int64_t)r * d.ldvh + c] = rsrc[(int64_t)j * rsrc_ld + c] * s;
        }
    }
    if (d.mode == 0 && blockIdx.x == 0) {
        __syncthreads();
        int cnt = 0;
        for (int j = threadIdx.x; j < d.nv; j += 256) cnt += (((gcp)d.sig)[j] <= thresh) ? 1 : 0;
#pragma unroll
        for (int o = 32; o > 0; o >>= 1) cnt += __shfl_xor(cnt, o);
        if ((threadIdx.x & 63) == 0) rk[threadIdx.x >> 6] = cnt;
        __syncthreads();
        if (threadIdx.x == 0) *d.n_null = rk[0] + rk[1] + rk[2] + rk[3];
    }
}

__global__ void __launch_bounds__(256) complete_null_kernel(const PostDesc* __restrict__ descs)
{
    __shared__ double red[4];
    __shared__ int redi[4];
    __shared__ int s_pick;
    const PostDesc d = descs[blockIdx.x];
    if (d.mode != 0 || *d.n_null == 0) return;
    const int tid = threadIdx.x;
    gp F = (gp)(d.transposed ? d.U : d.Vh);
    if (!F) return;
    const int64_t es = d.transposed ? d.ldu : 1;
    const int64_t vs = d.transposed ? 1 : d.ldvh;
    gp v = (gp)d.scratch;
    gp resid = v + d.lenp;
    const int n_null = *d.n_null;
    const int first_null = d.nv - n_null;
    for (int i = tid; i < d.len; i += 256) {
        double s = 1.0;
        for (int q = 0; q < first_null; ++q) {
            const double f = F[(int64_t)i * es + q * vs];
            s -= f * f;
        }
        resid[i] = s;
    }
    __syncthreads();
    for (int r = first_null; r < d.nv; ++r) {
        double best = -1.0;
        int bi = 0;
        for (int i = tid; i < d.len; i += 256)
            if (resid[i] > best) {
                best = resid[i];
                bi = i;
            }
#pragma unroll
        for (int o = 32; o > 0; o >>= 1) {
            const double ob = __shfl_xor(best, o);
            const int oi = __shfl_xor(bi, o);
            if (ob > best || (ob == best && oi < bi)) {
                best = ob;
                bi = oi;
            }
        }
        if ((tid & 63) == 0) {
            red[tid >> 6] = best;
            redi[tid >> 6] = bi;
        }
        __syncthreads();
        if (tid == 0) {
            int p = 0;
            for (int w = 1; w < 4; ++w)
                if (red[w] > red[p] || (red[w] == red[p] && redi[w] < redi[p])) p = w;
            s_pick = redi[p];
        }
        __syncthreads();
        const int cand = s_pick;
        for (int i = tid; i < d.len; i += 256) v[i] = (i == cand) ? 1.0 : 0.0;
        __syncthreads();
        for (int pass = 0; pass < 2; ++pass) {
            for (int q = 0; q < r; ++q) {
                double s = 0.0;
                for (int i = tid; i < d.len; i += 256) s += F[(int64_t)i * es + q * vs] * v[i];
#pragma unroll
                for (int o = 32; o > 0; o >>= 1) s += __shfl_xor(s, o);
                __syncthreads();
                if ((tid & 63) == 0) red[tid >> 6] = s;
                __syncthreads();
                const double dot = red[0] + red[1] + red[2] + red[3];
                for (int i = tid; i < d.len; i += 256) v[i] -= dot * F[(int64_t)i * es + q * vs];
                __syncthreads();
            }
        }
        double s = 0.0;
        for (int i = tid; i < d.len; i += 256) s += v[i] * v[i];
#pragma unroll
        for (int o = 32; o > 0; o >>= 1) s += __shfl_xor(s, o);
        __syncthreads();
        if ((tid & 63) == 0) red[tid >> 6] = s;
        __syncthreads();
        const double nrm2 = red[0] + red[1] + red[2] + red[3];
        const double inv = (nrm2 > 0.0) ? 1.0 / sqrt(nrm2) : 0.0;
        for (int i = tid; i < d.len; i += 256) {
            const double f = v[i] * inv;
            F[(int64_t)i * es + r * vs] = f;
            resid[i] = (i == cand) ? -1.0 : resid[i] - f * f;
        }
        __syncthreads();
    }
}

inline int round_up(int x, int m) { return (x + m - 1) / m * m; }

struct Layout {
    std::vector<JMat> mats;
    std::vector<PrepDesc> prep;
    std::vector<PostDesc> post;
    size_t bytes = 0;
};

}

static inline int row_blocks(int nv, int nvp)
{
    const int nb = 2 * ((nv + 2 * cyb::JB - 1) / (2 * cyb::JB));
    return std::min(std::max(nb, 4), nvp / cyb::JB);
}

static int run_jacobi(cyb_ctx_t ctx, int mode, int64_t nmat, const cyb_svd_desc* sd, const cyb_eigh_desc* ed,
                      int32_t* info, bool cplx = false)
{
    if (nmat == 0) return CYB_OK;
    hipStream_t st = ctx->stream;
    std::vector<JMat> mats((size_t)nmat);
    std::vector<PrepDesc> prep((size_t)nmat);
    std::vector<PostDesc> post((size_t)nmat);
    std::vector<NormDesc> nd;
    size_t off = 0;
    auto take = [&](size_t bytes) {
        const size_t o = off;
        off += (bytes + 255) / 256 * 256;
        return o;
    };
    struct Offs {
        size_t W, J, sig, rank, shift, scratch, nnull;
    };
    std::vector<Offs> offs((size_t)nmat);
    for (int64_t b = 0; b < nmat; ++b) {
        int m, n;
        if (mode == 0) {
            CYB_REQUIRE(sd[b].m >= 0 && sd[b].n >= 0 && sd[b].m < (1 << 30) && sd[b].n < (1 << 30),
                        "svd block %lld: bad shape", (long long)b);
            m = (int)sd[b].m;
            n = (int)sd[b].n;
            CYB_REQUIRE(m == 0 || n == 0 || (sd[b].A && sd[b].S), "svd block %lld: NULL pointer", (long long)b);
            CYB_REQUIRE(sd[b].lda >= n, "svd block %lld: lda < n", (long long)b);
        } else {
            CYB_REQUIRE(ed[b].n >= 0 && ed[b].n < (1 << 30), "eigh block %lld: bad shape", (long long)b);
            m = n = (int)ed[b].n;
            CYB_REQUIRE(n == 0 || (ed[b].A && ed[b].W), "eigh block %lld: NULL pointer", (long long)b);
            CYB_REQUIRE(ed[b].lda >= n, "eigh block %lld: lda < n", (long long)b);
        }
        const int nv = std::min(m, n), len = std::max(m, n);
        const int nvp = std::max(round_up(nv, 64), 64), lenp = std::max(round_up(len, 64), 64);
        const bool need_J = (mode == 0);
        Offs& o = offs[(size_t)b];
        o.W = take(sizeof(double) * (size_t)nvp * lenp);
        o.J = need_J ? take(sizeof(double) * (size_t)nvp * nvp) : 0;
        o.sig = take(sizeof(double) * (size_t)nvp);
        o.rank = take(sizeof(int32_t) * (size_t)nvp);
        o.shift = take(sizeof(double));
        o.scratch = take(sizeof(double) * (size_t)lenp * 2);
        o.nnull = take(sizeof(int32_t));
        JMat& jm = mats[(size_t)b];
        jm.nvp = nvp;
        jm.lenp = lenp;
        jm.nb = row_blocks(nv, nvp);
        jm.nv = nv;
        jm.len = len;
        jm.rec_j = 0;
        jm.tol = 2.220446049250313e-16 * std::max(16.0, 4.0 * std::sqrt((double)len));
        jm.thr2 = 0.0;
    }
    void* ws = nullptr;
    CYB_TRY(ctx->workspace(off, &ws));
    char* base = static_cast<char*>(ws);
    CYB_HIP(hipMemsetAsync(ws, 0, off, st));
    for (int64_t b = 0; b < nmat; ++b) {
        const Offs& o = offs[(size_t)b];
        JMat& jm = mats[(size_t)b];
        jm.W = reinterpret_cast<double*>(base + o.W);
        jm.J = (mode == 0) ? reinterpret_cast<double*>(base + o.J) : nullptr;
        PrepDesc& p = prep[(size_t)b];
        PostDesc& q = post[(size_t)b];
        if (mode == 0) {
            p.A = sd[b].A;
            p.lda = sd[b].lda;
            p.m = (int)sd[b].m;
            p.n = (int)sd[b].n;
            p.transpose = (sd[b].m >= sd[b].n) ? 1 : 0;
            p.shift = nullptr;
            q.U = sd[b].U;
            q.ldu = sd[b].ldu;
            q.Vh = sd[b].Vh;
            q.ldvh = sd[b].ldvh;
            q.S = sd[b].S;
            q.shift = nullptr;
        } else {
            p.A = ed[b].A;
            p.lda = ed[b].lda;
            p.m = p.n = (int)ed[b].n;
            p.transpose = 0;
            p.shift = reinterpret_cast<double*>(base + o.shift);
            q.U = ed[b].V;
            q.ldu = ed[b].ldv;
            q.Vh = nullptr;
            q.ldvh = 0;
            q.S = ed[b].W;
            q.shift = p.shift;
            nd.push_back(NormDesc{ed[b].A, ed[b].lda, (int)ed[b].n, (int)ed[b].n, reinterpret_cast<double*>(base + o.shift)});
        }
        p.W = jm.W;
        p.J = jm.J;
        p.nvp = jm.nvp;
        p.lenp = jm.lenp;
        p.pad = 0;
        q.W = jm.W;
        q.J = jm.J;
        q.nvp = jm.nvp;
        q.lenp = jm.lenp;
        q.nv = jm.nv;
        q.len = jm.len;
        q.transposed = p.transpose;
        q.mode = mode;
        q.sig = reinterpret_cast<double*>(base + o.sig);
        q.rank = reinterpret_cast<int32_t*>(base + o.rank);
        q.scratch = reinterpret_cast<double*>(base + o.scratch);
        q.n_null = reinterpret_cast<int32_t*>(base + o.nnull);
        q.null_scale = 0.0;
        q.cplx = cplx ? 1 : 0;
    }
    void* d_prep = nullptr;
    CYB_TRY(ctx->upload(prep.data(), sizeof(PrepDesc) * prep.size(), &d_prep));
    if (mode == 1) {
        void* d_nd = nullptr;
        CYB_TRY(ctx->upload(nd.data(), sizeof(NormDesc) * nd.size(), &d_nd));
        hipLaunchKernelGGL(fro_shift_kernel, dim3((unsigned)nmat), dim3(256), 0, st, static_cast<const NormDesc*>(d_nd));
    }
    hipLaunchKernelGGL(prep_kernel, dim3(64, (unsigned)nmat), dim3(256), 0, st, static_cast<const PrepDesc*>(d_prep));
    CYB_HIP(hipGetLastError());
    std::vector<int32_t> sweeps;
    const int jst = jacobi_orthogonalise(ctx, mats, 40, sweeps, cplx);
    if (info)
        for (int64_t b = 0; b < nmat; ++b) info[b] = sweeps[(size_t)b];
    if (jst != CYB_OK && jst != CYB_ERR_NOCONV) return jst;
    void* d_post = nullptr;
    CYB_TRY(ctx->upload(post.data(), sizeof(PostDesc) * post.size(), &d_post));
    const PostDesc* dp = static_cast<const PostDesc*>(d_post);
    hipLaunchKernelGGL(row_norm_kernel, dim3(helper_grid_x((size_t)nmat), (unsigned)nmat), dim3(256), 0, st, dp);
    hipLaunchKernelGGL(rank_kernel, dim3(8, (unsigned)nmat), dim3(256), 0, st, dp);
    hipLaunchKernelGGL(write_factors_kernel, dim3(helper_grid_x((size_t)nmat), (unsigned)nmat), dim3(256), 0, st, dp);
    if (mode == 0) hipLaunchKernelGGL(complete_null_kernel, dim3((unsigned)nmat), dim3(256), 0, st, dp);
    CYB_HIP(hipGetLastError());
    if (info) CYB_HIP(hipStreamSynchronize(st));
    return jst;
}


namespace {

struct RowsDesc {
    double* W;
    const double* sig;
    const int32_t* idx;
    double* buf;
    int32_t kp, k, cnt, pad;
    const int32_t* col;
};
__global__ void __launch_bounds__(256) gather_rows_kernel(const RowsDesc* __restrict__ descs)
{
    const RowsDesc d = descs[blockIdx.y];
    gcp W = (gcp)d.W;
    gp buf = (gp)d.buf;
    const int lane = threadIdx.x & 63;
    for (int c = blockIdx.x * 4 + (threadIdx.x >> 6); c < d.cnt; c += gridDim.x * 4) {
        const int j = d.idx[c];
        const double inv = 1.0 / ((gcp)d.sig)[j];
        for (int i = lane; i < d.k; i += 64) buf[(int64_t)c * d.k + i] = W[(int64_t)j * d.kp + i] * inv;
    }
}
__global__ void __launch_bounds__(256) scatter_rows_kernel(const RowsDesc* __restrict__ descs)
{
    const RowsDesc d = descs[blockIdx.y];
    gp W = (gp)d.W;
    gcp buf = (gcp)d.buf;
    const int lane = threadIdx.x & 63;
    for (int c = blockIdx.x * 4 + (threadIdx.x >> 6); c < d.cnt; c += gridDim.x * 4) {
        const int j = d.idx[c];
        const int cc = d.col ? d.col[c] : c;
        for (int i = lane; i < d.k; i += 64) W[(int64_t)j * d.kp + i] = buf[(int64_t)cc * d.k + i];
    }
}

struct JcqDesc {
    const double* J;
    const int32_t* rank;
    double* Cq;
    int64_t L;
    int32_t kp, k;
};
__global__ void __launch_bounds__(256) j_to_cq_kernel(const JcqDesc* __restrict__ descs)
{
    const JcqDesc d = descs[blockIdx.y];
    gcp J = (gcp)d.J;
    gp Cq = (gp)d.Cq;
    const int lane = threadIdx.x & 63;
    for (int j = blockIdx.x * 4 + (threadIdx.x >> 6); j < d.k; j += gridDim.x * 4) {
        const int r = d.rank[j];
        for (int i = lane; i < d.k; i += 64) Cq[(int64_t)r * d.L + i] = J[(int64_t)j * d.kp + i];
    }
}


struct RowMoveDesc {
    const double* src;
    double* dst;
    const int32_t* idx;
    int64_t lds, ldd;
    int32_t cnt, ncols;
    int32_t mode, pad;
};
__global__ void __launch_bounds__(256) row_move_kernel(const RowMoveDesc* __restrict__ descs)
{
    const RowMoveDesc d = descs[blockIdx.y];
    gcp src = (gcp)d.src;
    gp dst = (gp)d.dst;
    const int lane = threadIdx.x & 63;
    for (int g = blockIdx.x * 4 + (threadIdx.x >> 6); g < d.cnt; g += gridDim.x * 4) {
        const int j = d.idx[g];
        if (d.mode == 0) {
            for (int c = lane; c < d.ncols; c += 64) dst[(int64_t)g * d.ldd + c] = src[(int64_t)j * d.lds + c];
        } else if (d.mode == 1) {
            for (int c = lane; c < d.ncols; c += 64) dst[(int64_t)j * d.ldd + c] = src[(int64_t)g * d.lds + c];
        } else {
            for (int c = lane; c < d.ncols; c += 64) dst[(int64_t)j * d.ldd + c] = 0.0;
        }
    }
}
__global__ void __launch_bounds__(256) j_scatter_kernel(const RowMoveDesc* __restrict__ descs)
{
    const RowMoveDesc d = descs[blockIdx.y];
    gcp src = (gcp)d.src;
    gp dst = (gp)d.dst;
    const int lane = threadIdx.x & 63;
    for (int g = blockIdx.x * 4 + (threadIdx.x >> 6); g < d.cnt; g += gridDim.x * 4) {
        const int j = d.idx[g];
        for (int h = lane; h < d.cnt; h += 64) dst[(int64_t)j * d.ldd + d.idx[h]] = src[(int64_t)g * d.lds + h];
    }
}

struct PairDesc {
    double* W;
    int64_t ld;
    int32_t nv, len;
};
__global__ void __launch_bounds__(256) embed_pairs_kernel(const PairDesc* __restrict__ descs)
{
    const PairDesc d = descs[blockIdx.y];
    gp W = (gp)d.W;
    const int lane = threadIdx.x & 63;
    for (int a = blockIdx.x * 4 + (threadIdx.x >> 6); a < d.nv / 2; a += gridDim.x * 4) {
        gp e = W + (int64_t)(2 * a) * d.ld, o = e + d.ld;
        for (int j = lane; j < d.len / 2; j += 64) {
            const double x = 0.5 * (e[2 * j] + o[2 * j + 1]), y = 0.5 * (o[2 * j] - e[2 * j + 1]);
            e[2 * j] = x;
            e[2 * j + 1] = -y;
            o[2 * j] = y;
            o[2 * j + 1] = x;
        }
    }
}

struct LqDesc {
    double* Wq;
    double* Jc;
    double* Wc;
    double* Cq2;
    double* sig2;
    double* bad;
    double thr2;
    int32_t rp, kp, k, r0;
    int32_t cplx, jrec;
    double* Ws;
    double* G;
    double* dev;
    double* sigo;
    const int32_t* idx;
};
constexpr double JREC_BOUND = 2e-11;
constexpr int JREC_NB = 128;
__global__ void __launch_bounds__(256) lq_pack_kernel(const LqDesc* __restrict__ descs)
{
    const LqDesc d = descs[blockIdx.y];
    gcp Jc = (gcp)d.Jc;
    gp C = (gp)d.Cq2;
    const int lane = threadIdx.x & 63;
    for (int i = blockIdx.x * 4 + (threadIdx.x >> 6); i < d.k; i += gridDim.x * 4) {
        for (int c = lane; c < d.k; c += 64) {
            double v;
            if (i < d.r0) {
                if (c < d.r0 && d.jrec) continue;
                v = c < d.r0 ? Jc[(int64_t)i * d.rp + c] : 0.0;
            } else v = c == i ? 1.0 : 0.0;
            C[(int64_t)i * d.k + c] = v;
        }
    }
}
__global__ void __launch_bounds__(256) lq_rows_kernel(const LqDesc* __restrict__ descs)
{
    const LqDesc d = descs[blockIdx.y];
    gcp Wq = (gcp)d.Wq;
    gp Jc = (gp)d.Jc;
    const int lane = threadIdx.x & 63;
    for (int i = blockIdx.x * 4 + (threadIdx.x >> 6); i < d.r0; i += gridDim.x * 4) {
        double s = 0.0;
        for (int c = lane; c < d.r0; c += 64) {
            const double v = Wq[(int64_t)i * d.rp + c];
            s += v * v;
        }
#pragma unroll
        for (int o = 32; o > 0; o >>= 1) s += __shfl_xor(s, o);
        const double sg = sqrt(s);
        if (lane == 0) {
            ((gp)d.sig2)[i] = sg;
            if (!(sg > 0.0)) *(gp)d.bad = 1.0;
            if (d.jrec && !(sg * sg > d.thr2)) *(gp)d.bad = 1.0;
        }
        const double inv = sg > 0.0 ? 1.0 / sg : 0.0;
        for (int c = lane; c < d.r0; c += 64) Jc[(int64_t)i * d.rp + c] = Wq[(int64_t)i * d.rp + c] * inv;
        if (d.jrec) {
            gp Ws = (gp)d.Ws;
            const double inv2 = inv * inv;
            for (int c = lane; c < d.r0; c += 64) Ws[(int64_t)i * d.r0 + c] = Wq[(int64_t)i * d.rp + c] * inv2;
        }
    }
}
__global__ void __launch_bounds__(256) jrec_check_kernel(const LqDesc* __restrict__ descs)
{
    const LqDesc d = descs[blockIdx.y];
    if (!d.jrec) return;
    gcp G = (gcp)d.G;
    const int lane = threadIdx.x & 63;
    double mx = 0.0;
    bool nan = false;
    for (int i = blockIdx.x * 4 + (threadIdx.x >> 6); i < d.r0; i += gridDim.x * 4) {
        for (int c = i / JREC_NB * JREC_NB + lane; c < d.r0; c += 64) {
            const double v = fabs(G[(int64_t)i * d.r0 + c] - (c == i ? 1.0 : 0.0));
            nan = nan || !(v == v);
            mx = fmax(mx, v);
        }
    }
#pragma unroll
    for (int o = 32; o > 0; o >>= 1) mx = fmax(mx, __shfl_xor(mx, o));
    nan = __any(nan);
    if (lane == 0) {
        if (nan) mx = __builtin_huge_val();
        atomicMax((unsigned long long*)d.dev, (unsigned long long)__double_as_longlong(mx));
        if (!(mx <= JREC_BOUND)) *(gp)d.bad = 1.0;
    }
}
__global__ void __launch_bounds__(256) lq_check_kernel(const LqDesc* __restrict__ descs)
{
    const LqDesc d = descs[blockIdx.y];
    gcp Jc = (gcp)d.Jc;
    const int lane = threadIdx.x & 63;
    const int wid = blockIdx.x * 4 + (threadIdx.x >> 6), nw = gridDim.x * 4;
    for (int i0 = 0; i0 < d.r0; i0 += 64) {
        bool fl = false;
        if (i0 + lane < d.r0) {
            const double sg = ((gcp)d.sig2)[i0 + lane];
            fl = !(sg * sg > d.thr2);
        }
        unsigned long long msk = __ballot(fl);
        while (msk) {
            const int i = i0 + __ffsll((long long)msk) - 1;
            msk &= msk - 1;
            double worst = 0.0;
            for (int j = wid; j < d.r0; j += nw) {
                if (j == i) continue;
                double t = 0.0;
                for (int c = lane; c < d.r0; c += 64) t = fma(Jc[(int64_t)i * d.rp + c], Jc[(int64_t)j * d.rp + c], t);
#pragma unroll
                for (int o = 32; o > 0; o >>= 1) t += __shfl_xor(t, o);
                worst = fmax(worst, fabs(t));
            }
            if (lane == 0 && !(worst <= 1e-12)) *(gp)d.bad = 1.0;
        }
    }
}
__global__ void __launch_bounds__(256) lq_unpack_kernel(const LqDesc* __restrict__ descs)
{
    const LqDesc d = descs[blockIdx.y];
    gcp C = (gcp)d.Cq2;
    gp Wc = (gp)d.Wc;
    const int lane = threadIdx.x & 63;
    for (int i = blockIdx.x * 4 + (threadIdx.x >> 6); i < d.r0; i += gridDim.x * 4) {
        const double sg = ((gcp)d.sig2)[i];
        const double sm = d.cplx ? fmax(sg, ((gcp)d.sig2)[i ^ 1]) : sg;
        double f = sm * sm > d.thr2 ? sg : 0.0;
        double n2 = 0.0;
        for (int c = lane; c < d.k; c += 64) n2 = fma(C[(int64_t)i * d.k + c], C[(int64_t)i * d.k + c], n2);
#pragma unroll
        for (int o = 32; o > 0; o >>= 1) n2 += __shfl_xor(n2, o);
        if (lane == 0) ((gp)d.sigo)[d.idx[i]] = n2 > 0.0 ? f : 0.0;
        f = n2 > 0.0 ? f / sqrt(n2) : 0.0;
        for (int c = lane; c < d.kp; c += 64) Wc[(int64_t)i * d.kp + c] = c < d.k ? f * C[(int64_t)i * d.k + c] : 0.0;
    }
}

static int launch_row_moves(cyb_ctx_t ctx, const std::vector<RowMoveDesc>& v, bool jscatter = false)
{
    if (v.empty()) return CYB_OK;
    void* d = nullptr;
    CYB_TRY(ctx->upload(v.data(), sizeof(RowMoveDesc) * v.size(), &d));
    if (jscatter)
        hipLaunchKernelGGL(j_scatter_kernel, dim3(64, (unsigned)v.size()), dim3(256), 0, ctx->stream, static_cast<const RowMoveDesc*>(d));
    else
        hipLaunchKernelGGL(row_move_kernel, dim3(helper_grid_x(v.size()), (unsigned)v.size()), dim3(256), 0, ctx->stream, static_cast<const RowMoveDesc*>(d));
    CYB_HIP(hipGetLastError());
    return CYB_OK;
}

}

static int run_svd_qr(cyb_ctx_t ctx, int64_t nmat, const cyb_svd_desc* sd, int32_t* info, int flags, int32_t* rank_out)
{
    if (nmat == 0) return CYB_OK;
    const bool cplx = (flags & CYB_SVD_EMBEDDED_COMPLEX) != 0;
    hipStream_t st = ctx->stream;
    auto al = [](size_t b) { return (b + 255) / 256 * 256; };
    struct Lay {
        int m, n, k, L, kp;
        bool tall;
        size_t Ac, aux, W, J, sig, rank, thr, nnull, Cq, Fc, aux2, Cn, idx, Wc, Jc;
        size_t bad, Wq, aux3, Cq2, sig2;
        size_t stop;
        size_t ctl;
        int n_fac = -1;
        size_t sigo;
        size_t dev;
        bool lq = false;
        bool jrec = false;
        int r0 = 0;
        std::vector<int32_t> good0;
    };
    std::vector<Lay> lay((size_t)nmat);
    size_t off = 0;
    size_t sig_begin = off;
    for (int64_t b = 0; b < nmat; ++b) {
        Lay& l = lay[(size_t)b];
        l.m = (int)sd[b].m;
        l.n = (int)sd[b].n;
        l.k = std::min(l.m, l.n);
        l.L = std::max(l.m, l.n);
        l.kp = round_up(l.k, 64);
        l.tall = l.m >= l.n;
        l.sig = off;
        off += sizeof(double) * (size_t)l.kp;
    }
    for (int64_t b = 0; b < nmat; ++b) {
        lay[(size_t)b].thr = off;
        off += sizeof(double);
    }
    for (int64_t b = 0; b < nmat; ++b) {
        lay[(size_t)b].bad = off;
        off += sizeof(double);
    }
    for (int64_t b = 0; b < nmat; ++b) {
        lay[(size_t)b].dev = off;
        off += sizeof(double);
    }
    for (int64_t b = 0; b < nmat; ++b) {
        lay[(size_t)b].ctl = off;
        off += 2 * sizeof(double);
    }
    const size_t sig_bytes = off - sig_begin;
    off = al(off);
    for (int64_t b = 0; b < nmat; ++b) {
        Lay& l = lay[(size_t)b];
        auto take = [&](size_t bytes) {
            const size_t o = off;
            off += al(bytes);
            return o;
        };
        l.Ac = take(sizeof(double) * (size_t)l.L * l.k);
        l.aux = take(bqr_aux_bytes(l.L, l.k, l.L, l.k));
        l.stop = take(sizeof(double) * (size_t)std::max(1, (l.k + cyb::NBK - 1) / cyb::NBK * cyb::bqr_strip_slots(l.L)));
        l.W = take(sizeof(double) * (size_t)l.kp * l.kp);
        l.J = take(sizeof(double) * (size_t)l.kp * l.kp);
        l.rank = take(sizeof(int32_t) * (size_t)l.kp);
        l.nnull = take(sizeof(int32_t));
        l.Cq = take(sizeof(double) * (size_t)l.L * l.k);
        l.Fc = take(sizeof(double) * (size_t)l.k * l.k);
        l.aux2 = take(bqr_aux_bytes(l.k, l.k, l.k, l.k));
        l.Cn = take(sizeof(double) * (size_t)l.k * l.k);
        l.Wc = take(sizeof(double) * (size_t)l.kp * l.kp);
        l.Jc = take(sizeof(double) * (size_t)l.kp * l.kp);
        l.Wq = take(sizeof(double) * (size_t)l.kp * l.kp);
        l.aux3 = take(bqr_aux_bytes(l.k, l.k, l.kp, l.k));
        l.Cq2 = take(sizeof(double) * (size_t)l.k * l.k);
        l.sig2 = take(sizeof(double) * (size_t)l.kp);
        l.sigo = take(sizeof(double) * (size_t)l.kp);
    }
    const size_t idx_begin = off;
    for (int64_t b = 0; b < nmat; ++b) {
        lay[(size_t)b].idx = off;
        off += sizeof(int32_t) * (size_t)lay[(size_t)b].k;
    }
    off = al(off);
    void* ws = nullptr;
    CYB_TRY(ctx->workspace(off, &ws, 0));
    char* base = static_cast<char*>(ws);
    CYB_HIP(hipMemsetAsync(ws, 0, off, st));
    auto dp = [&](size_t o) { return reinterpret_cast<double*>(base + o); };

    std::vector<BqrMat> qm((size_t)nmat);
    std::vector<XposeDesc> x_in, x_r;
    std::vector<EyeDesc> eyeJ;
    std::vector<JMat> jm((size_t)nmat);
    for (int64_t b = 0; b < nmat; ++b) {
        const Lay& l = lay[(size_t)b];
        BqrMat& q = qm[(size_t)b];
        q.Ac = dp(l.Ac);
        q.ld = l.L;
        q.m = l.L;
        q.n = l.k;
        q.k = l.k;
        bqr_carve(q, base + l.aux, l.k);
        q.v_zeroed = 1;
        q.reflect_always = cplx ? 1 : 0;
        q.ctl = dp(l.ctl);
        q.parts = dp(l.stop);
        q.stop_rel2 = ((double)l.L * 2.220446049250313e-16) * ((double)l.L * 2.220446049250313e-16);
        if (l.tall)
            x_in.push_back(XposeDesc{sd[b].A, q.Ac, sd[b].lda, l.L, l.n, l.m, 0, 0, 0, 0});
        else
            x_in.push_back(XposeDesc{sd[b].A, q.Ac, sd[b].lda, l.L, l.m, l.n, 0, 0, 1, 0});
        x_r.push_back(XposeDesc{q.Ac, dp(l.W), l.L, l.kp, l.k, l.k, 1, l.k, 0, 0});
        eyeJ.push_back(EyeDesc{dp(l.J), l.kp, l.kp, l.kp, 0, 0});
        JMat& j = jm[(size_t)b];
        j.W = dp(l.W);
        j.J = dp(l.J);
        j.nvp = l.kp;
        j.lenp = l.kp;
        j.nb = row_blocks(l.k, l.kp);
        j.nv = l.k;
        j.len = l.k;
        j.rec_j = 0;
        j.tol = 2.220446049250313e-16 * std::max(16.0, 4.0 * std::sqrt((double)l.k));
        j.thr2 = 0.0;
    }
    CYB_TRY(xpose_batched(ctx, x_in));
    CYB_TRY(bqr_factor(ctx, qm));
    CYB_TRY(xpose_batched(ctx, x_r));
    CYB_TRY(eye_cols_batched(ctx, eyeJ));
    std::vector<PostDesc> post((size_t)nmat);
    for (int64_t b = 0; b < nmat; ++b) {
        const Lay& l = lay[(size_t)b];
        PostDesc& q = post[(size_t)b];
        q.W = dp(l.W);
        q.J = dp(l.J);
        q.nvp = l.kp;
        q.lenp = l.kp;
        q.nv = l.k;
        q.len = l.k;
        q.transposed = l.tall ? 0 : 1;
        q.mode = 0;
        q.sig = dp(l.sig);
        q.rank = reinterpret_cast<int32_t*>(base + l.rank);
        q.S = sd[b].S;
        q.U = l.tall ? nullptr : sd[b].U;
        q.ldu = sd[b].ldu;
        q.Vh = l.tall ? sd[b].Vh : nullptr;
        q.ldvh = sd[b].ldvh;
        q.shift = nullptr;
        q.scratch = nullptr;
        q.n_null = reinterpret_cast<int32_t*>(base + l.nnull);
        q.null_scale = 1.0;
        q.cplx = cplx ? 1 : 0;
    }
    void* d_post = nullptr;
    const PostDesc* dpost = nullptr;
    std::vector<double> h_sig(sig_bytes / sizeof(double));
    auto sig_of = [&](const Lay& l) { return h_sig.data() + (l.sig - sig_begin) / sizeof(double); };
    CYB_TRY(ctx->upload(post.data(), sizeof(PostDesc) * post.size(), &d_post));
    dpost = static_cast<const PostDesc*>(d_post);
    hipLaunchKernelGGL(row_norm_kernel, dim3(helper_grid_x((size_t)nmat), (unsigned)nmat), dim3(256), 0, st, dpost);
    CYB_HIP(hipGetLastError());
    CYB_TRY(ctx->d2h(h_sig.data(), base + sig_begin, sig_bytes));
    {
        std::vector<int32_t> idx_all;
        std::vector<size_t> idx_off((size_t)nmat, 0);
        for (int64_t b = 0; b < nmat; ++b) {
            Lay& l = lay[(size_t)b];
            const double* sg = sig_of(l);
            const double stopped = h_sig[(l.ctl - sig_begin) / sizeof(double)];
            l.n_fac = stopped != 0.0 ? (int)stopped - 1 : -1;
            double fro2 = 0.0;
            for (int j = 0; j < l.k; ++j) fro2 += sg[j] * sg[j];
            const double sc = (double)l.L * 2.220446049250313e-16;
            const double thr2 = fro2 * sc * sc;
            jm[(size_t)b].thr2 = thr2;
            std::vector<int32_t> nul;
            for (int j = 0; j < l.k; ++j) {
                const double v = cplx ? std::max(sg[j & ~1], sg[std::min(j | 1, l.k - 1)]) : sg[j];
                (v * v > thr2 ? l.good0 : nul).push_back(j);
            }
            l.r0 = (int)l.good0.size();
            idx_off[(size_t)b] = idx_all.size();
            idx_all.insert(idx_all.end(), l.good0.begin(), l.good0.end());
            idx_all.insert(idx_all.end(), nul.begin(), nul.end());
        }
        static const bool no_lq = getenv("CYB_SVD_NOLQ") != nullptr;
        static const bool lq_always = getenv("CYB_SVD_LQ_ALWAYS") != nullptr;
        static const int lq_skip_k = getenv("CYB_SVD_LQ_SKIP_K") ? atoi(getenv("CYB_SVD_LQ_SKIP_K")) : 128;
        static const double lq_skip_ratio = getenv("CYB_SVD_LQ_SKIP_RATIO") ? atof(getenv("CYB_SVD_LQ_SKIP_RATIO")) : 1e4;
        for (int64_t b = 0; b < nmat; ++b) {
            Lay& l = lay[(size_t)b];
            bool skip = false;
            if (!lq_always && l.r0 == l.k && l.k >= lq_skip_k) {
                const double* sg = sig_of(l);
                double lo = 1e300, hi = 0.0;
                for (int j = 0; j < l.k; ++j) {
                    lo = std::min(lo, sg[j]);
                    hi = std::max(hi, sg[j]);
                }
                skip = hi <= lq_skip_ratio * lo;
            }
            l.lq = !no_lq && l.r0 >= 2 && !skip;
        }
        static const bool no_jrec = getenv("CYB_SVD_NOJREC") != nullptr;
        static const double jrec_ratio = getenv("CYB_SVD_JREC_RATIO") ? atof(getenv("CYB_SVD_JREC_RATIO")) : 1e1;
        static const int jrec_min = getenv("CYB_SVD_JREC_MIN") ? atoi(getenv("CYB_SVD_JREC_MIN")) : 256;
        for (int64_t b = 0; b < nmat; ++b) {
            Lay& l = lay[(size_t)b];
            if (!l.lq || no_jrec || cplx || l.r0 < jrec_min) continue;
            const double* sg = sig_of(l);
            double lo = 1e300, hi = 0.0;
            for (int32_t j : l.good0) {
                lo = std::min(lo, sg[j]);
                hi = std::max(hi, sg[j]);
            }
            l.jrec = hi <= jrec_ratio * lo;
        }
        void* d_idx_v = nullptr;
        CYB_TRY(ctx->upload(idx_all.data(), sizeof(int32_t) * idx_all.size(), &d_idx_v));
        CYB_HIP(hipMemcpyAsync(base + idx_begin, d_idx_v, sizeof(int32_t) * idx_all.size(), hipMemcpyDeviceToDevice, st));
    }
    const std::vector<JMat> jm0 = jm;
    std::vector<BqrMat> qm3;
    std::vector<int> qm3_of((size_t)nmat, -1);
    std::vector<int32_t> sweeps;
    auto iterate = [&](bool allow_lq, int& jst) -> int {
        jm = jm0;
        qm3.clear();
        std::fill(qm3_of.begin(), qm3_of.end(), -1);
        std::vector<RowMoveDesc> gat, zer;
        std::vector<EyeDesc> eyeJc;
        std::vector<XposeDesc> x_r2;
        std::vector<LqDesc> lqd;
        std::vector<int> jrec_blocks;
        std::vector<BqrTarget> tg3;
        for (int64_t b = 0; b < nmat; ++b) {
            Lay& l = lay[(size_t)b];
            l.lq = l.lq && allow_lq;
            if (l.r0 == l.k && !l.lq) continue;
            const int32_t* didx = reinterpret_cast<const int32_t*>(base + l.idx);
            const int rp = std::max(round_up(l.r0, 64), 64);
            gat.push_back(RowMoveDesc{dp(l.W), dp(l.Wc), didx, l.kp, l.kp, l.r0, l.kp, 0, 0});
            if (l.r0 < l.k) zer.push_back(RowMoveDesc{nullptr, dp(l.W), didx + l.r0, 0, l.kp, l.k - l.r0, l.kp, 2, 0});
            const bool jrec = l.lq && l.jrec && allow_lq;
            if (!jrec) eyeJc.push_back(EyeDesc{dp(l.Jc), rp, rp, rp, 0, 0});
            JMat& j = jm[(size_t)b];
            j.W = dp(l.Wc);
            j.J = dp(l.Jc);
            j.nvp = rp;
            j.nb = row_blocks(l.r0, rp);
            j.nv = l.r0;
            if (l.lq) {
                BqrMat q;
                q.Ac = dp(l.Wc);
                q.ld = l.kp;
                q.m = l.k;
                q.n = l.r0;
                q.k = l.r0;
                bqr_carve(q, base + l.aux3, l.k);
                q.v_zeroed = allow_lq ? 1 : 0;
                q.reflect_always = cplx ? 1 : 0;
                x_r2.push_back(XposeDesc{dp(l.Wc), dp(l.Wq), l.kp, rp, l.r0, l.r0, 1, l.r0, 0, 0});
                j.W = dp(l.Wq);
                j.lenp = rp;
                j.len = l.r0;
                const double thr2 = j.thr2;
                j.thr2 = 0.0;
                lqd.push_back(LqDesc{dp(l.Wq), dp(l.Jc), dp(l.Wc), dp(l.Cq2), dp(l.sig2), dp(l.bad), thr2, rp, l.kp, l.k, l.r0, cplx ? 1 : 0,
                                     jrec ? 1 : 0, dp(l.Fc), dp(l.Fc), dp(l.dev), dp(l.sigo), didx});
                if (jrec) {
                    j.J = nullptr;
                    j.rec_j = 1;
                    x_r2.push_back(XposeDesc{dp(l.Wc), dp(l.Cn), l.kp, l.r0, l.r0, l.r0, 1, l.r0, 0, 0});
                    jrec_blocks.push_back((int)b);
                }
                tg3.push_back(BqrTarget{(int)qm3.size(), dp(l.Cq2), l.k, l.k});
                qm3_of[(size_t)b] = (int)qm3.size();
                qm3.push_back(q);
            }
        }
        CYB_TRY(launch_row_moves(ctx, gat));
        CYB_TRY(launch_row_moves(ctx, zer));
        CYB_TRY(eye_cols_batched(ctx, eyeJc));
        if (!qm3.empty()) {
            CYB_TRY(bqr_factor(ctx, qm3));
            CYB_TRY(xpose_batched(ctx, x_r2));
        }
        if (cplx) {
            std::vector<PairDesc> prs;
            for (const JMat& j : jm)
                if (j.nv >= 2) prs.push_back(PairDesc{const_cast<double*>(j.W), j.lenp, j.nv & ~1, j.len & ~1});
            if (!prs.empty()) {
                void* d = nullptr;
                CYB_TRY(ctx->upload(prs.data(), sizeof(PairDesc) * prs.size(), &d));
                hipLaunchKernelGGL(embed_pairs_kernel, dim3(64, (unsigned)prs.size()), dim3(256), 0, st, static_cast<const PairDesc*>(d));
                CYB_HIP(hipGetLastError());
            }
        }
        jst = jacobi_orthogonalise(ctx, jm, 40, sweeps, cplx);
        if (jst != CYB_OK && jst != CYB_ERR_NOCONV) return jst;
        if (!qm3.empty()) {
            void* d = nullptr;
            CYB_TRY(ctx->upload(lqd.data(), sizeof(LqDesc) * lqd.size(), &d));
            const LqDesc* dl = static_cast<const LqDesc*>(d);
            hipLaunchKernelGGL(lq_pack_kernel, dim3(64, (unsigned)lqd.size()), dim3(256), 0, st, dl);
            hipLaunchKernelGGL(lq_rows_kernel, dim3(64, (unsigned)lqd.size()), dim3(256), 0, st, dl);
            if (!jrec_blocks.empty()) {
                int64_t tiles = 0;
                for (int b : jrec_blocks) tiles += (int64_t)((lay[(size_t)b].r0 + 127) / 128) * ((lay[(size_t)b].r0 + 127) / 128);
                const int nbc = tiles >= 2 * (int64_t)ctx->n_cu ? 128 : 64;
                GemmBatch g_rec, g_chk;
                for (int b : jrec_blocks) {
                    const Lay& l = lay[(size_t)b];
                    const int64_t r0 = l.r0, k = l.k;
                    for (int64_t c0 = 0; c0 < r0; c0 += nbc)
                        g_rec.add(dp(l.Cq2) + c0, r0, std::min<int64_t>(nbc, r0 - c0), k, dp(l.Fc) + c0, r0, 1, dp(l.Cn) + c0 * r0 + c0, 1, r0,
                                  r0 - c0, 1.0, 0.0);
                    for (int64_t i0 = 0; i0 < r0; i0 += JREC_NB)
                        g_chk.add(dp(l.Fc) + i0 * r0 + i0, std::min<int64_t>(JREC_NB, r0 - i0), r0 - i0, r0, dp(l.Cq2) + i0 * k, k, 1,
                                  dp(l.Cq2) + i0 * k, 1, k, r0, 1.0, 0.0);
                }
                CYB_TRY(g_rec.launch(ctx));
                CYB_TRY(g_chk.launch(ctx));
                CYB_TRY(ctx->upload(lqd.data(), sizeof(LqDesc) * lqd.size(), &d));
                dl = static_cast<const LqDesc*>(d);
                hipLaunchKernelGGL(jrec_check_kernel, dim3(16, (unsigned)lqd.size()), dim3(256), 0, st, dl);
            }
            hipLaunchKernelGGL(lq_check_kernel, dim3(helper_grid_x(lqd.size()), (unsigned)lqd.size()), dim3(256), 0, st, dl);
            CYB_HIP(hipGetLastError());
            CYB_TRY(bqr_apply_q(ctx, qm3, tg3));
            CYB_TRY(ctx->upload(lqd.data(), sizeof(LqDesc) * lqd.size(), &d));
            hipLaunchKernelGGL(lq_unpack_kernel, dim3(64, (unsigned)lqd.size()), dim3(256), 0, st, static_cast<const LqDesc*>(d));
            CYB_HIP(hipGetLastError());
        }
        return CYB_OK;
    };
    int jst = CYB_OK;
    CYB_TRY(iterate(true, jst));
    if (!qm3.empty()) {
        std::vector<double> bad((size_t)nmat * 2, 0.0);
        CYB_TRY(ctx->d2h(bad.data(), base + lay[0].bad, sizeof(double) * (size_t)nmat * 2));
        const std::vector<double> jdev(bad.begin() + nmat, bad.end());
        bad.resize((size_t)nmat);
        static const bool force_redo = getenv("CYB_SVD_LQ_FORCE_REDO") != nullptr;
        static const bool force_jredo = getenv("CYB_SVD_JREC_FORCE_REDO") != nullptr;
        bool redo = jst == CYB_ERR_NOCONV || force_redo;
        for (double v : bad) redo = redo || v != 0.0;
        for (const Lay& l : lay) redo = redo || (force_jredo && l.lq && l.jrec);
        static const bool trace_redo = getenv("CYB_SVD_TRACE_REDO") != nullptr;
        if (trace_redo)
            for (int64_t b = 0; b < nmat; ++b) {
                const Lay& l = lay[(size_t)b];
                const char* route = !l.lq ? "no LQ step" : !l.jrec ? "excluded" : redo ? "recovered then redone" : "recovered";
                fprintf(stderr, "[cyb] svd jrec: block %lld (%d x %d, r0 %d): %s (deviation %.2e, flagged %d)\n", (long long)b, l.m, l.n, l.r0,
                        route, jdev[(size_t)b], (int)(bad[(size_t)b] != 0.0));
            }
        if (redo && trace_redo) {
            int nb = 0;
            for (double v : bad) nb += v != 0.0;
            fprintf(stderr, "[cyb] svd: plain iteration after the LQ one (%d of %lld blocks flagged, noconv %d)\n", nb, (long long)nmat,
                    (int)(jst == CYB_ERR_NOCONV));
        }
        if (redo) CYB_TRY(iterate(false, jst));
    } else if (getenv("CYB_SVD_TRACE_REDO") != nullptr) {
        for (int64_t b = 0; b < nmat; ++b)
            fprintf(stderr, "[cyb] svd jrec: block %lld (%d x %d, r0 %d): no LQ step (deviation %.2e, flagged 0)\n", (long long)b,
                    lay[(size_t)b].m, lay[(size_t)b].n, lay[(size_t)b].r0, 0.0);
    }
    if (info)
        for (int64_t b = 0; b < nmat; ++b) info[b] = sweeps[(size_t)b];
    if (jst != CYB_OK && jst != CYB_ERR_NOCONV) return jst;
    {
        std::vector<RowMoveDesc> sw, sj;
        for (int64_t b = 0; b < nmat; ++b) {
            const Lay& l = lay[(size_t)b];
            if ((l.r0 == l.k && !l.lq) || l.r0 == 0) continue;
            const int32_t* didx = reinterpret_cast<const int32_t*>(base + l.idx);
            const int rp = std::max(round_up(l.r0, 64), 64);
            sw.push_back(RowMoveDesc{dp(l.Wc), dp(l.W), didx, l.kp, l.kp, l.r0, l.kp, 1, 0});
            sj.push_back(RowMoveDesc{dp(l.Jc), dp(l.J), didx, rp, l.kp, l.r0, l.r0, 0, 0});
        }
        CYB_TRY(launch_row_moves(ctx, sw));
        CYB_TRY(launch_row_moves(ctx, sj, true));
    }
    for (int64_t b = 0; b < nmat; ++b) post[(size_t)b].sig_lq = lay[(size_t)b].lq ? dp(lay[(size_t)b].sigo) : nullptr;
    CYB_TRY(ctx->upload(post.data(), sizeof(PostDesc) * post.size(), &d_post));
    dpost = static_cast<const PostDesc*>(d_post);
    hipLaunchKernelGGL(row_norm_kernel, dim3(helper_grid_x((size_t)nmat), (unsigned)nmat), dim3(256), 0, st, dpost);
    CYB_HIP(hipGetLastError());
    CYB_TRY(ctx->d2h(h_sig.data(), base + sig_begin, sig_bytes));
    {
        std::vector<int32_t> idx_all;
        struct Comp {
            int64_t b;
            size_t good_off, null_off;
            int r, q;
        };
        std::vector<Comp> comps;
        for (int64_t b = 0; b < nmat; ++b) {
            const Lay& l = lay[(size_t)b];
            const double* sg = sig_of(l);
            std::vector<int32_t> good, nul;
            for (int j = 0; j < l.k; ++j) {
                const double v = cplx ? std::max(sg[j & ~1], sg[std::min(j | 1, l.k - 1)]) : sg[j];
                (v > 0.0 ? good : nul).push_back(j);
            }
            if (rank_out) rank_out[b] = (int32_t)good.size();
            Comp c{b, idx_all.size(), 0, (int)good.size(), (int)nul.size()};
            idx_all.insert(idx_all.end(), good.begin(), good.end());
            c.null_off = idx_all.size();
            idx_all.insert(idx_all.end(), nul.begin(), nul.end());
            if (nul.empty() || (flags & CYB_SVD_SKIP_NULL_VECTORS)) continue;
            comps.push_back(c);
        }
        if (!comps.empty()) {
            void* d_idx_v = nullptr;
            CYB_TRY(ctx->upload(idx_all.data(), sizeof(int32_t) * idx_all.size(), &d_idx_v));
            CYB_HIP(hipMemcpyAsync(base + idx_begin, d_idx_v, sizeof(int32_t) * idx_all.size(), hipMemcpyDeviceToDevice, st));
            std::vector<RowsDesc> gath, scat;
            std::vector<int32_t> cols_all;
            std::vector<std::pair<size_t, size_t>> lq_scat;
            std::vector<BqrMat> qm2;
            std::vector<BqrTarget> tg2;
            std::vector<EyeDesc> eyes;
            for (const Comp& c : comps) {
                const Lay& l = lay[(size_t)c.b];
                if (l.lq) {
                    const size_t c0 = cols_all.size();
                    int t = 0;
                    size_t g = 0;
                    const int32_t* nulp = idx_all.data() + c.null_off;
                    for (int qn = 0; qn < c.q; ++qn) {
                        const int32_t j = nulp[qn];
                        while (g < l.good0.size() && l.good0[g] < j) ++g;
                        if (g < l.good0.size() && l.good0[g] == j) cols_all.push_back((int32_t)g);
                        else cols_all.push_back((int32_t)(l.r0 + t++));
                    }
                    lq_scat.push_back({scat.size(), c0});
                    scat.push_back(RowsDesc{dp(l.W), dp(l.sig), reinterpret_cast<const int32_t*>(base + l.idx) + c.r, dp(l.Cq2), l.kp,
                                            l.k, c.q, 0, nullptr});
                    continue;
                }
                if (c.r > 0) {
                    gath.push_back(RowsDesc{dp(l.W), dp(l.sig), reinterpret_cast<const int32_t*>(base + l.idx), dp(l.Fc), l.kp, l.k, c.r, 0, nullptr});
                    BqrMat q;
                    q.Ac = dp(l.Fc);
                    q.ld = l.k;
                    q.m = l.k;
                    q.n = c.r;
                    q.k = std::min(l.k, c.r);
                    bqr_carve(q, base + l.aux2, c.q);
                    tg2.push_back(BqrTarget{(int)qm2.size(), dp(l.Cn), l.k, c.q});
                    qm2.push_back(q);
                }
                eyes.push_back(EyeDesc{dp(l.Cn), l.k, l.k, c.q, c.r, 0});
                scat.push_back(RowsDesc{dp(l.W), dp(l.sig), reinterpret_cast<const int32_t*>(base + l.idx) + c.r, dp(l.Cn), l.kp, l.k, c.q, 0, nullptr});
            }
            if (!gath.empty()) {
                void* d = nullptr;
                CYB_TRY(ctx->upload(gath.data(), sizeof(RowsDesc) * gath.size(), &d));
                hipLaunchKernelGGL(gather_rows_kernel, dim3(64, (unsigned)gath.size()), dim3(256), 0, st,
                                   static_cast<const RowsDesc*>(d));
                CYB_HIP(hipGetLastError());
                CYB_TRY(bqr_factor(ctx, qm2));
            }
            CYB_TRY(eye_cols_batched(ctx, eyes));
            if (!tg2.empty()) CYB_TRY(bqr_apply_q(ctx, qm2, tg2));
            void* d = nullptr;
            if (!cols_all.empty()) {
                void* d_cols = nullptr;
                CYB_TRY(ctx->upload(cols_all.data(), sizeof(int32_t) * cols_all.size(), &d_cols));
                for (const auto& pr : lq_scat) scat[pr.first].col = static_cast<const int32_t*>(d_cols) + pr.second;
            }
            CYB_TRY(ctx->upload(scat.data(), sizeof(RowsDesc) * scat.size(), &d));
            hipLaunchKernelGGL(scatter_rows_kernel, dim3(64, (unsigned)scat.size()), dim3(256), 0, st,
                               static_cast<const RowsDesc*>(d));
            CYB_HIP(hipGetLastError());
        }
    }
    CYB_TRY(ctx->upload(post.data(), sizeof(PostDesc) * post.size(), &d_post));
    dpost = static_cast<const PostDesc*>(d_post);
    hipLaunchKernelGGL(rank_kernel, dim3(8, (unsigned)nmat), dim3(256), 0, st, dpost);
    hipLaunchKernelGGL(write_factors_kernel, dim3(helper_grid_x((size_t)nmat), (unsigned)nmat), dim3(256), 0, st, dpost);
    CYB_HIP(hipGetLastError());
    std::vector<JcqDesc> jc;
    std::vector<BqrTarget> tg;
    std::vector<XposeDesc> x_out;
    for (int64_t b = 0; b < nmat; ++b) {
        const Lay& l = lay[(size_t)b];
        jc.push_back(JcqDesc{dp(l.J), reinterpret_cast<const int32_t*>(base + l.rank), dp(l.Cq), l.L, l.kp, l.k});
        tg.push_back(BqrTarget{(int)b, dp(l.Cq), l.L, l.k, l.n_fac >= 0 ? l.n_fac : (l.k + cyb::NBK - 1) / cyb::NBK});
        if (l.tall)
            x_out.push_back(XposeDesc{dp(l.Cq), sd[b].U, l.L, sd[b].ldu, l.m, l.k, 0, 0, 0, 0});
        else
            x_out.push_back(XposeDesc{dp(l.Cq), sd[b].Vh, l.L, sd[b].ldvh, l.k, l.n, 0, 0, 1, 0});
    }
    {
        void* d = nullptr;
        CYB_TRY(ctx->upload(jc.data(), sizeof(JcqDesc) * jc.size(), &d));
        hipLaunchKernelGGL(j_to_cq_kernel, dim3(helper_grid_x((size_t)nmat), (unsigned)nmat), dim3(256), 0, st, static_cast<const JcqDesc*>(d));
        CYB_HIP(hipGetLastError());
    }
    CYB_TRY(bqr_apply_q(ctx, qm, tg));
    CYB_TRY(xpose_batched(ctx, x_out));
    if (info) CYB_HIP(hipStreamSynchronize(st));
    return jst;
}

}

namespace cyb {
bool svd_small_fits(int64_t m, int64_t n);
int svd_small_batched(cyb_ctx_t ctx, const cyb_svd_desc* descs, int64_t n, int32_t* sweeps_out);
int eigh_small_batched(cyb_ctx_t ctx, const cyb_eigh_desc* descs, int64_t n, int32_t* sweeps_out);
}

extern "C" {

static int svd_batched_impl(cyb_ctx_t ctx, const cyb_svd_desc* descs, int64_t n, int32_t* info, int flags = 0,
                            int32_t* rank_out = nullptr)
{
    CYB_REQUIRE(ctx, "cyb_svd_batched_f64: ctx is NULL");
    CYB_REQUIRE(n >= 0 && (n == 0 || descs), "cyb_svd_batched_f64: bad descriptor list");
    std::vector<cyb_svd_desc> nz;
    std::vector<int64_t> idx;
    for (int64_t b = 0; b < n; ++b) {
        if (info) info[b] = 0;
        if (rank_out) rank_out[b] = (int32_t)std::min(descs[b].m, descs[b].n);
        if (descs[b].m > 0 && descs[b].n > 0) {
            CYB_REQUIRE(descs[b].U && descs[b].Vh, "svd block %lld: U / Vh is NULL", (long long)b);
            nz.push_back(descs[b]);
            idx.push_back(b);
        }
    }
    static const bool no_qr = getenv("CYB_SVD_NOQR") != nullptr;
    static const bool no_small = getenv("CYB_SVD_NOSMALL") != nullptr;
    size_t n_fit = 0;
    for (const auto& d : nz) n_fit += cyb::svd_small_fits(d.m, d.n) ? 1 : 0;
    const bool embedded = (flags & CYB_SVD_EMBEDDED_COMPLEX) != 0;
    const bool use_small = !embedded && !no_small && (n_fit == nz.size() || n_fit >= 16);
    std::vector<cyb_svd_desc> tiny, small, large;
    std::vector<int64_t> idx_t, idx_s, idx_l;
    static const bool no_merge = getenv("CYB_SVD_NOMERGE") != nullptr;
    bool any_large = false;
    for (const auto& d : nz) any_large = any_large || (!no_qr && std::min(d.m, d.n) >= 48 && !(use_small && cyb::svd_small_fits(d.m, d.n)));
    (void)any_large;
    const int64_t large_min = embedded ? 1 : no_merge ? 48 : 2;
    for (size_t k = 0; k < nz.size(); ++k) {
        if (use_small && cyb::svd_small_fits(nz[k].m, nz[k].n)) {
            CYB_REQUIRE(nz[k].S, "svd block %lld: S is NULL", (long long)idx[k]);
            tiny.push_back(nz[k]);
            idx_t.push_back(idx[k]);
        } else if (!no_qr && std::min(nz[k].m, nz[k].n) >= large_min) {
            large.push_back(nz[k]);
            idx_l.push_back(idx[k]);
        } else {
            small.push_back(nz[k]);
            idx_s.push_back(idx[k]);
        }
    }
    std::vector<int32_t> inf_t(tiny.size()), inf_s(small.size()), inf_l(large.size());
    const int st_t = cyb::svd_small_batched(ctx, tiny.data(), (int64_t)tiny.size(), inf_t.data());
    if (st_t != CYB_OK && st_t != CYB_ERR_NOCONV) return st_t;
    if (info)
        for (size_t k = 0; k < tiny.size(); ++k) info[idx_t[k]] = inf_t[k];
    if (small.empty() && large.empty()) return st_t;
    std::vector<int32_t> rank_l(large.size());
    const int st_l = cyb::run_svd_qr(ctx, (int64_t)large.size(), large.data(), info ? inf_l.data() : nullptr, flags,
                                     rank_out ? rank_l.data() : nullptr);
    if (rank_out)
        for (size_t k = 0; k < large.size(); ++k) rank_out[idx_l[k]] = rank_l[k];
    if (st_l != CYB_OK && st_l != CYB_ERR_NOCONV) return st_l;
    const int st_s = cyb::run_jacobi(ctx, 0, (int64_t)small.size(), small.data(), nullptr, info ? inf_s.data() : nullptr);
    if (info) {
        for (size_t k = 0; k < small.size(); ++k) info[idx_s[k]] = inf_s[k];
        for (size_t k = 0; k < large.size(); ++k) info[idx_l[k]] = inf_l[k];
    }
    return st_s != CYB_OK ? st_s : (st_l != CYB_OK ? st_l : st_t);
}

static int eigh_batched_impl(cyb_ctx_t ctx, const cyb_eigh_desc* descs, int64_t n, int32_t* info, int flags = 0)
{
    CYB_REQUIRE(ctx, "cyb_eigh_batched_f64: ctx is NULL");
    CYB_REQUIRE(n >= 0 && (n == 0 || descs), "cyb_eigh_batched_f64: bad descriptor list");
    std::vector<cyb_eigh_desc> nz;
    std::vector<int64_t> idx;
    for (int64_t b = 0; b < n; ++b) {
        if (info) info[b] = 0;
        if (descs[b].n > 0) {
            nz.push_back(descs[b]);
            idx.push_back(b);
        }
    }
    std::vector<int32_t> inf(nz.size());
    static const bool no_small = getenv("CYB_SVD_NOSMALL") != nullptr;
    const bool embedded = (flags & CYB_EIGH_EMBEDDED_COMPLEX) != 0;
    bool all_small = !no_small && !nz.empty() && !embedded;
    for (const auto& d : nz) all_small = all_small && d.n <= 64;
    const int st = all_small ? cyb::eigh_small_batched(ctx, nz.data(), (int64_t)nz.size(), inf.data())
                             : cyb::run_jacobi(ctx, 1, (int64_t)nz.size(), nullptr, nz.data(), info ? inf.data() : nullptr, embedded);
    if (info)
        for (size_t k = 0; k < nz.size(); ++k) info[idx[k]] = inf[k];
    return st;
}

static int svd_batched_ranged(cyb_ctx_t ctx, const cyb_svd_desc* descs, int64_t n, int32_t* info, int flags, int32_t* rank)
{
    std::vector<cyb::MatRef> refs;
    std::vector<int64_t> which;
    for (int64_t b = 0; b < n; ++b)
        if (descs[b].m > 0 && descs[b].n > 0 && descs[b].A) {
            refs.push_back(cyb::MatRef{descs[b].A, descs[b].lda, descs[b].m, descs[b].n});
            which.push_back(b);
        }
    std::vector<double> amax;
    CYB_TRY(cyb::matrix_amax(ctx, refs, amax));
    std::vector<cyb_svd_desc> mod;
    std::vector<void*> temps;
    std::vector<cyb::ScaleJob> pre, post;
    for (size_t k = 0; k < refs.size(); ++k) {
        const double sc = cyb::range_scale(amax[k]);
        if (sc == 1.0) continue;
        if (mod.empty()) mod.assign(descs, descs + n);
        cyb_svd_desc& d = mod[(size_t)which[k]];
        void* t = nullptr;
        CYB_HIP(hipMalloc(&t, sizeof(double) * (size_t)d.m * (size_t)d.n));
        temps.push_back(t);
        pre.push_back(cyb::ScaleJob{d.A, d.lda, static_cast<double*>(t), d.n, d.m, d.n, sc});
        d.A = static_cast<const double*>(t);
        d.lda = d.n;
        post.push_back(cyb::ScaleJob{d.S, 1, d.S, 1, std::min(d.m, d.n), 1, 1.0 / sc});
    }
    if (mod.empty()) return svd_batched_impl(ctx, descs, n, info, flags, rank);
    int st = cyb::scale_copy_batched(ctx, pre);
    if (st == CYB_OK) st = svd_batched_impl(ctx, mod.data(), n, info, flags, rank);
    if (st == CYB_OK || st == CYB_ERR_NOCONV) {
        const int st2 = cyb::scale_copy_batched(ctx, post);
        if (st2 != CYB_OK) st = st2;
    }
    (void)hipStreamSynchronize(ctx->stream);
    for (void* t : temps) (void)hipFree(t);
    return st;
}

int cyb_svd_batched_f64(cyb_ctx_t ctx, const cyb_svd_desc* descs, int64_t n, int32_t* info)
{
    CYB_REQUIRE(ctx, "cyb_svd_batched_f64: ctx is NULL");
    CYB_REQUIRE(n >= 0 && (n == 0 || descs), "cyb_svd_batched_f64: bad descriptor list");
    return svd_batched_ranged(ctx, descs, n, info, 0, nullptr);
}

int cyb_svd_batched_ex_f64(cyb_ctx_t ctx, const cyb_svd_desc* descs, int64_t n, int32_t* info, int32_t flags, int32_t* rank)
{
    CYB_REQUIRE(ctx, "cyb_svd_batched_ex_f64: ctx is NULL");
    CYB_REQUIRE(n >= 0 && (n == 0 || descs), "cyb_svd_batched_ex_f64: bad descriptor list");
    CYB_REQUIRE((flags & ~(CYB_SVD_SKIP_NULL_VECTORS | CYB_SVD_EMBEDDED_COMPLEX)) == 0, "cyb_svd_batched_ex_f64: unknown flag bits 0x%x", flags);
    if (flags & CYB_SVD_EMBEDDED_COMPLEX)
        for (int64_t b = 0; b < n; ++b)
            CYB_REQUIRE(descs[b].m % 2 == 0 && descs[b].n % 2 == 0, "svd block %lld: an embedded complex block has even extents", (long long)b);
    const int st = svd_batched_ranged(ctx, descs, n, info, flags, rank);
    if (rank && !info) CYB_HIP(hipStreamSynchronize(ctx->stream));
    return st;
}

static int eigh_batched_ranged(cyb_ctx_t ctx, const cyb_eigh_desc* descs, int64_t n, int32_t* info, int flags)
{
    std::vector<cyb::MatRef> refs;
    std::vector<int64_t> which;
    for (int64_t b = 0; b < n; ++b)
        if (descs[b].n > 0 && descs[b].A) {
            refs.push_back(cyb::MatRef{descs[b].A, descs[b].lda, descs[b].n, descs[b].n});
            which.push_back(b);
        }
    std::vector<double> amax;
    CYB_TRY(cyb::matrix_amax(ctx, refs, amax));
    std::vector<cyb_eigh_desc> mod;
    std::vector<void*> temps;
    std::vector<cyb::ScaleJob> pre, post;
    for (size_t k = 0; k < refs.size(); ++k) {
        const double sc = cyb::range_scale(amax[k]);
        if (sc == 1.0) continue;
        if (mod.empty()) mod.assign(descs, descs + n);
        cyb_eigh_desc& d = mod[(size_t)which[k]];
        void* t = nullptr;
        CYB_HIP(hipMalloc(&t, sizeof(double) * (size_t)d.n * (size_t)d.n));
        temps.push_back(t);
        pre.push_back(cyb::ScaleJob{d.A, d.lda, static_cast<double*>(t), d.n, d.n, d.n, sc});
        d.A = static_cast<const double*>(t);
        d.lda = d.n;
        post.push_back(cyb::ScaleJob{d.W, 1, d.W, 1, d.n, 1, 1.0 / sc});
    }
    if (mod.empty()) return eigh_batched_impl(ctx, descs, n, info, flags);
    int st = cyb::scale_copy_batched(ctx, pre);
    if (st == CYB_OK) st = eigh_batched_impl(ctx, mod.data(), n, info, flags);
    if (st == CYB_OK || st == CYB_ERR_NOCONV) {
        const int st2 = cyb::scale_copy_batched(ctx, post);
        if (st2 != CYB_OK) st = st2;
    }
    (void)hipStreamSynchronize(ctx->stream);
    for (void* t : temps) (void)hipFree(t);
    return st;
}

int cyb_eigh_batched_f64(cyb_ctx_t ctx, const cyb_eigh_desc* descs, int64_t n, int32_t* info)
{
    CYB_REQUIRE(ctx, "cyb_eigh_batched_f64: ctx is NULL");
    CYB_REQUIRE(n >= 0 && (n == 0 || descs), "cyb_eigh_batched_f64: bad descriptor list");
    return eigh_batched_ranged(ctx, descs, n, info, 0);
}

int cyb_eigh_batched_ex_f64(cyb_ctx_t ctx, const cyb_eigh_desc* descs, int64_t n, int32_t* info, int32_t flags)
{
    CYB_REQUIRE(ctx, "cyb_eigh_batched_ex_f64: ctx is NULL");
    CYB_REQUIRE(n >= 0 && (n == 0 || descs), "cyb_eigh_batched_ex_f64: bad descriptor list");
    CYB_REQUIRE((flags & ~CYB_EIGH_EMBEDDED_COMPLEX) == 0, "cyb_eigh_batched_ex_f64: unknown flag bits 0x%x", flags);
    if (flags & CYB_EIGH_EMBEDDED_COMPLEX)
        for (int64_t b = 0; b < n; ++b)
            CYB_REQUIRE(descs[b].n % 2 == 0, "eigh block %lld: an embedded complex block has an even extent", (long long)b);
    return eigh_batched_ranged(ctx, descs, n, info, flags);
}

}
```

### cyten_amd/csrc/truncation.hip

```cpp
#include "common.h"

#include <algorithm>
#include <vector>

namespace {

constexpr int NT = 1024;
constexpr int NMAX = 8192;
constexpr int NBIG = 65536;

struct SDesc {
    const double* S;
    int64_t n, offset;
    double w;
};

struct Opts {
    int64_t chi_max, chi_min;
    double degeneracy_tol, trunc_cut, svd_min;
    int32_t has_svd_min, minimize_error;
};

__device__ __forceinline__ bool key_less(double ka, int ia, double kb, int ib) { return ka < kb || (ka == kb && ia < ib); }

__device__ int block_any(bool v, int* scratch)
{
    const unsigned long long b = __ballot(v);
    __syncthreads();
    if ((threadIdx.x & 63) == 0) scratch[threadIdx.x >> 6] = b != 0;
    __syncthreads();
    int r = 0;
    for (int q = 0; q < NT / 64; ++q) r |= scratch[q];
    return r;
}

template <typename T>
__device__ T block_excl_scan(T v, T* wave_tot, T* total)
{
    const int lane = threadIdx.x & 63, wave = threadIdx.x >> 6;
    T inc = v;
#pragma unroll
    for (int o = 1; o < 64; o <<= 1) {
        const T up = __shfl_up(inc, o);
        if (lane >= o) inc += up;
    }
    __syncthreads();
    if (lane == 63) wave_tot[wave] = inc;
    __syncthreads();
    T base = 0, all = 0;
    for (int w = 0; w < NT / 64; ++w) {
        if (w < wave) base += wave_tot[w];
        all += wave_tot[w];
    }
    if (total) *total = all;
    return base + inc - v;
}

template <bool BIG>
__global__ void __launch_bounds__(NT) truncate_select_kernel(const SDesc* __restrict__ descs, int n_sectors, int n, int n2, Opts o,
                                                             double* __restrict__ s_all,
                                                             int64_t* __restrict__ keep_idx, uint8_t* __restrict__ mask_out,
                                                             double* __restrict__ result,
                                                             double* __restrict__ gkey, int* __restrict__ gidx,
                                                             unsigned char* __restrict__ ggood)
{
    __shared__ double lkey[NMAX];
    __shared__ int lidx[NMAX];
    __shared__ unsigned char lgood[BIG ? 1 : NMAX];
    double* key = BIG ? gkey : lkey;
    int* idx = BIG ? gidx : lidx;
    unsigned char* good = BIG ? ggood : lgood;
    __shared__ int scratch[NT / 64];
    __shared__ double dtot[NT / 64];
    __shared__ int s_cut;
    const int tid = threadIdx.x;
    for (int s = 0; s < n_sectors; ++s) {
        const SDesc d = descs[s];
        for (int64_t e = tid; e < d.n; e += NT) {
            const double v = d.S[e];
            s_all[d.offset + e] = v;
            key[d.offset + e] = d.w * (v * v);
            idx[d.offset + e] = (int)(d.offset + e);
        }
    }
    for (int e = n + tid; e < n2; e += NT) {
        key[e] = __builtin_huge_val();
        idx[e] = e;
    }
    __syncthreads();
    auto cmpx = [&](double* kk, int* ii, int e, int p, bool up) {
        const double ka = kk[e], kb = kk[p];
        const int ia = ii[e], ib = ii[p];
        const bool swap = up ? key_less(kb, ib, ka, ia) : key_less(ka, ia, kb, ib);
        if (swap) {
            kk[e] = kb, kk[p] = ka;
            ii[e] = ib, ii[p] = ia;
        }
    };
    if (!BIG) {
        for (int k = 2; k <= n2; k <<= 1) {
            for (int j = k >> 1; j > 0; j >>= 1) {
                for (int t = tid; t < n2 / 2; t += NT) {
                    const int e = ((t & ~(j - 1)) << 1) | (t & (j - 1));
                    cmpx(key, idx, e, e + j, (e & k) == 0);
                }
                __syncthreads();
            }
        }
    } else {
        auto chunk_steps = [&](int base, int k, int jmax) {
            for (int e = tid; e < NMAX; e += NT) {
                lkey[e] = gkey[base + e];
                lidx[e] = gidx[base + e];
            }
            __syncthreads();
            for (int kk = (jmax == 0 ? 2 : k); kk <= k; kk <<= 1) {
                for (int j = min(kk >> 1, NMAX >> 1); j > 0; j >>= 1) {
                    for (int t = tid; t < NMAX / 2; t += NT) {
                        const int e = ((t & ~(j - 1)) << 1) | (t & (j - 1));
                        cmpx(lkey, lidx, e, e + j, ((base + e) & kk) == 0);
                    }
                    __syncthreads();
                }
            }
            for (int e = tid; e < NMAX; e += NT) {
                gkey[base + e] = lkey[e];
                gidx[base + e] = lidx[e];
            }
            __syncthreads();
        };
        for (int base = 0; base < n2; base += NMAX) chunk_steps(base, NMAX, 0);
        for (int k = 2 * NMAX; k <= n2; k <<= 1) {
            for (int j = k >> 1; j >= NMAX; j >>= 1) {
                for (int t = tid; t < n2 / 2; t += NT) {
                    const int e = ((t & ~(j - 1)) << 1) | (t & (j - 1));
                    cmpx(gkey, gidx, e, e + j, (e & k) == 0);
                }
                __syncthreads();
            }
            for (int base = 0; base < n2; base += NMAX) chunk_steps(base, k, 1);
        }
    }
    for (int e = tid; e < n; e += NT) good[e] = 1;
    __syncthreads();
    auto combine = [&](auto g2) {
        bool any = false;
        for (int e = tid; e < n; e += NT) any |= good[e] && g2(e);
        if (block_any(any, scratch)) {
            for (int e = tid; e < n; e += NT) good[e] = good[e] && g2(e);
        }
        __syncthreads();
    };
    if (o.chi_max >= 0 && o.chi_max < n) combine([&](int e) { return e >= n - (int)o.chi_max; });
    if (o.chi_min > 1) combine([&](int e) { return e < n - (int)o.chi_min + 1; });
    if (o.degeneracy_tol > 0.0)
        combine([&](int e) {
            if (e == 0) return true;
            const double a = s_all[idx[e]], b = s_all[idx[e - 1]];
            return log(a <= 1e-100 ? 1e-100 : a) - log(b <= 1e-100 ? 1e-100 : b) >= o.degeneracy_tol;
        });
    if (o.has_svd_min) combine([&](int e) { return s_all[idx[e]] >= o.svd_min; });
    {
        const int chunk = (n + NT - 1) / NT;
        const int b0 = min(tid * chunk, n), b1 = min(b0 + chunk, n);
        double run = 0.0;
        for (int e = b0; e < b1; ++e) {
            run += key[e];
            key[e] = run;
        }
        const double base = block_excl_scan<double>(run, dtot, nullptr);
        for (int e = b0; e < b1; ++e) key[e] += base;
        __syncthreads();
    }
    {
        const double tc2 = o.trunc_cut * o.trunc_cut;
        combine([&](int e) { return key[e] > tc2; });
    }
    {
        int best = o.minimize_error ? n : -1;
        for (int e = tid; e < n; e += NT)
            if (good[e]) best = o.minimize_error ? min(best, e) : max(best, e);
        for (int off = 32; off > 0; off >>= 1) {
            const int other = __shfl_xor(best, off);
            best = o.minimize_error ? min(best, other) : max(best, other);
        }
        if ((tid & 63) == 0) scratch[tid >> 6] = best;
        __syncthreads();
        if (tid == 0) {
            int b = scratch[0];
            for (int q = 1; q < NT / 64; ++q) b = o.minimize_error ? min(b, scratch[q]) : max(b, scratch[q]);
            s_cut = b;
            const double total = key[n - 1];
            const double err = b > 0 ? key[b - 1] : 0.0;
            result[0] = err;
            result[1] = total - err;
        }
        __syncthreads();
    }
    const int cut = s_cut;
    for (int e = tid; e < n; e += NT) good[idx[e]] = 0;
    __syncthreads();
    for (int e = cut + tid; e < n; e += NT) good[idx[e]] = 1;
    __syncthreads();
    for (int e = tid; e < n; e += NT) mask_out[e] = good[e];
    int64_t* counts = reinterpret_cast<int64_t*>(result + 2);
    for (int s = 0; s < n_sectors; ++s) {
        const SDesc d = descs[s];
        const int ns = (int)d.n, o0 = (int)d.offset;
        const int chunk = (ns + NT - 1) / NT;
        const int b0 = min(tid * chunk, ns), b1 = min(b0 + chunk, ns);
        int cnt = 0;
        for (int e = b0; e < b1; ++e) cnt += good[o0 + e];
        int kept = 0;
        int w = block_excl_scan<int>(cnt, scratch, &kept);
        if (tid == 0) counts[s] = kept;
        for (int e = b0; e < b1; ++e)
            if (good[o0 + e]) keep_idx[o0 + w++] = e;
        __syncthreads();
    }
}

}

extern "C" int cyb_truncate_select_f64(cyb_ctx_t ctx, const cyb_vec_desc* descs, int64_t n_sectors, const cyb_trunc_opts* opts,
                                       int64_t* keep_idx_dev, uint8_t* mask_dev, double* result_dev)
{
    return cyb_truncate_select_weighted_f64(ctx, descs, n_sectors, nullptr, opts, keep_idx_dev, mask_dev, result_dev);
}

extern "C" int cyb_truncate_select_weighted_f64(cyb_ctx_t ctx, const cyb_vec_desc* descs, int64_t n_sectors, const double* sector_weights,
                                                const cyb_trunc_opts* opts, int64_t* keep_idx_dev, uint8_t* mask_dev, double* result_dev)
{
    CYB_REQUIRE(ctx && opts && result_dev, "cyb_truncate_select_f64: NULL argument");
    CYB_REQUIRE(n_sectors >= 0 && (n_sectors == 0 || descs), "cyb_truncate_select_f64: bad sector list");
    std::vector<SDesc> hd((size_t)n_sectors);
    int64_t n = 0;
    for (int64_t s = 0; s < n_sectors; ++s) {
        CYB_REQUIRE(descs[s].n >= 0 && (descs[s].n == 0 || descs[s].x), "cyb_truncate_select_f64: sector %lld is malformed", (long long)s);
        const double w = sector_weights ? sector_weights[s] : 1.0;
        CYB_REQUIRE(w > 0.0 && w < 1e300, "cyb_truncate_select_weighted_f64: weight of sector %lld is not a positive finite number", (long long)s);
        hd[(size_t)s] = SDesc{descs[s].x, descs[s].n, n, w};
        n += descs[s].n;
    }
    CYB_REQUIRE(n >= 1, "cyb_truncate_select_f64: no singular values");
    CYB_REQUIRE(keep_idx_dev && mask_dev, "cyb_truncate_select_f64: NULL output");
    if (n > NBIG) {
        cyb::set_error("cyb_truncate_select_f64: %lld values exceed the %d one workgroup sorts", (long long)n, NBIG);
        return CYB_ERR_UNSUPPORTED;
    }
    CYB_REQUIRE(opts->chi_min >= 1, "cyb_truncate_select_f64: chi_min must be >= 1");
    int n2 = 2;
    while (n2 < n) n2 <<= 1;
    void *d_descs = nullptr, *ws = nullptr;
    CYB_TRY(ctx->upload(hd.data(), sizeof(SDesc) * hd.size(), &d_descs));
    const bool big = n > NMAX;
    if (big) n2 = std::max(n2, 2 * NMAX);
    const size_t off_key = (sizeof(double) * (size_t)n + 255) & ~(size_t)255;
    const size_t off_idx = off_key + sizeof(double) * (size_t)n2, off_good = off_idx + sizeof(int) * (size_t)n2;
    CYB_TRY(ctx->workspace(big ? off_good + (size_t)n2 : sizeof(double) * (size_t)n, &ws, 2));
    Opts o{opts->chi_max, opts->chi_min, opts->degeneracy_tol, opts->trunc_cut, opts->svd_min, opts->has_svd_min,
           opts->minimize_error};
    char* w8 = static_cast<char*>(ws);
    if (big)
        hipLaunchKernelGGL(truncate_select_kernel<true>, dim3(1), dim3(NT), 0, ctx->stream, static_cast<const SDesc*>(d_descs),
                           (int)n_sectors, (int)n, n2, o, static_cast<double*>(ws), keep_idx_dev, mask_dev, result_dev,
                           reinterpret_cast<double*>(w8 + off_key), reinterpret_cast<int*>(w8 + off_idx),
                           reinterpret_cast<unsigned char*>(w8 + off_good));
    else
        hipLaunchKernelGGL(truncate_select_kernel<false>, dim3(1), dim3(NT), 0, ctx->stream, static_cast<const SDesc*>(d_descs),
                           (int)n_sectors, (int)n, n2, o, static_cast<double*>(ws), keep_idx_dev, mask_dev, result_dev,
                           (double*)nullptr, (int*)nullptr, (unsigned char*)nullptr);
    CYB_HIP(hipGetLastError());
    return CYB_OK;
}
```

Baseline: 5467.

## Balance batched helper kernels with byte-weighted work items and parallel truncation rank

Replaces the fixed 2D grids (blockIdx.y per matrix, fixed blockIdx.x split) of many helper kernels (transpose, eye, scale-copy, amax, sum-partials, prep, scatter, etc.) with a flat list of work items sized by bytes so large and small matrices share workgroups evenly. Amax also gets a vectorized double2 load path. The small-case truncation select drops its single-workgroup bitonic sort in favour of a multi-block rank-counting kernel that computes each value's sorted position in parallel. The cost is extra host-side item construction and uploads, plus O(n^2) comparisons in the rank kernel.

```diff
diff --git a/cyten_amd/csrc/blocked_qr.hip b/cyten_amd/csrc/blocked_qr.hip
--- a/cyten_amd/csrc/blocked_qr.hip
+++ b/cyten_amd/csrc/blocked_qr.hip
@@ -1192,11 +1192,13 @@
     int64_t n, stride;
     int32_t ns, pad;
 };
-__global__ void __launch_bounds__(256) sum_partials_kernel(const SumDesc* __restrict__ descs)
-{
-    const SumDesc d = descs[blockIdx.y];
+__global__ void __launch_bounds__(256) sum_partials_kernel(const SumDesc* __restrict__ descs, const WorkItem* __restrict__ items)
+{
+    const WorkItem it = items[blockIdx.x];
+    const SumDesc d = descs[it.mat];
     gp W1 = (gp)d.W1;
-    for (int64_t e = (int64_t)blockIdx.x * 256 + threadIdx.x; e < d.n; e += (int64_t)gridDim.x * 256) {
+    const int64_t e1 = (int64_t)it.end * 256 < d.n ? (int64_t)it.end * 256 : d.n;
+    for (int64_t e = (int64_t)it.begin * 256 + threadIdx.x; e < e1; e += 256) {
         double t = W1[e];
         for (int sidx = 1; sidx < d.ns; ++sidx) t += W1[e + (int64_t)sidx * d.stride];
         W1[e] = t;
@@ -1205,23 +1207,21 @@
 
 inline size_t al256(size_t b) { return (b + 255) / 256 * 256; }
 
-__global__ void __launch_bounds__(256) xpose_kernel(const XposeDesc* __restrict__ descs)
+__global__ void __launch_bounds__(256) xpose_kernel(const XposeDesc* __restrict__ descs, const WorkItem* __restrict__ items)
 {
     __shared__ double tile[32][33];
-    const XposeDesc d = descs[blockIdx.y];
+    const WorkItem it = items[blockIdx.x];
+    const XposeDesc d = descs[it.mat];
     gcp in = (gcp)d.in;
     gp out = (gp)d.out;
     const int tx = threadIdx.x & 31, ty = threadIdx.x >> 5;
     if (d.plain) {
-        const int64_t tot = (int64_t)d.R * d.C;
-        for (int64_t e = (int64_t)blockIdx.x * 256 + threadIdx.x; e < tot; e += (int64_t)gridDim.x * 256) {
-            const int64_t r = e / d.C, c = e % d.C;
-            out[r * d.ldo + c] = in[r * d.ldi + c];
-        }
+        for (int64_t r = it.begin; r < it.end; ++r)
+            for (int c = threadIdx.x; c < d.C; c += 256) out[r * d.ldo + c] = in[r * d.ldi + c];
         return;
     }
-    const int tr = (d.R + 31) / 32, tc = (d.C + 31) / 32;
-    for (int t = blockIdx.x; t < tr * tc; t += gridDim.x) {
+    const int tc = (d.C + 31) / 32;
+    for (int t = it.begin; t < it.end; ++t) {
         const int r0 = (t / tc) * 32, c0 = (t % tc) * 32;
         __syncthreads();
 #pragma unroll
@@ -1242,15 +1242,13 @@
     }
 }
 
-__global__ void __launch_bounds__(256) eye_cols_kernel(const EyeDesc* __restrict__ descs)
-{
-    const EyeDesc d = descs[blockIdx.y];
+__global__ void __launch_bounds__(256) eye_cols_kernel(const EyeDesc* __restrict__ descs, const WorkItem* __restrict__ items)
+{
+    const WorkItem it = items[blockIdx.x];
+    const EyeDesc d = descs[it.mat];
     gp C = (gp)d.C;
-    const int64_t tot = (int64_t)d.m * d.kc;
-    for (int64_t e = (int64_t)blockIdx.x * 256 + threadIdx.x; e < tot; e += (int64_t)gridDim.x * 256) {
-        const int64_t c = e / d.m, i = e % d.m;
-        C[c * d.ld + i] = (i == c + d.col0) ? 1.0 : 0.0;
-    }
+    for (int64_t c = it.begin; c < it.end; ++c)
+        for (int64_t i = threadIdx.x; i < d.m; i += 256) C[c * d.ld + i] = (i == c + d.col0) ? 1.0 : 0.0;
 }
 
 }
@@ -1258,9 +1256,20 @@
 int xpose_batched(cyb_ctx_t ctx, const std::vector<XposeDesc>& descs)
 {
     if (descs.empty()) return CYB_OK;
-    void* d = nullptr;
-    CYB_TRY(ctx->upload(descs.data(), sizeof(XposeDesc) * descs.size(), &d));
-    hipLaunchKernelGGL(xpose_kernel, dim3(helper_grid_x(descs.size()), (unsigned)descs.size()), dim3(256), 0, ctx->stream, static_cast<const XposeDesc*>(d));
+    std::vector<WorkList> wl(descs.size());
+    for (size_t b = 0; b < descs.size(); ++b) {
+        const XposeDesc& x = descs[b];
+        if (x.R <= 0 || x.C <= 0) wl[b] = WorkList{0, 0};
+        else if (x.plain) wl[b] = WorkList{x.R, 8 * (int64_t)x.C};
+        else wl[b] = WorkList{(int64_t)((x.R + 31) / 32) * ((x.C + 31) / 32), 8 * 32 * 32};
+    }
+    std::vector<WorkItem> items;
+    make_work_items(wl.data(), wl.size(), 1, items);
+    if (items.empty()) return CYB_OK;
+    const XposeDesc* d = nullptr;
+    const WorkItem* di = nullptr;
+    CYB_TRY(upload_with_items(ctx, descs, items, &d, &di));
+    hipLaunchKernelGGL(xpose_kernel, dim3((unsigned)items.size()), dim3(256), 0, ctx->stream, d, di);
     CYB_HIP(hipGetLastError());
     return CYB_OK;
 }
@@ -1268,9 +1277,15 @@
 int eye_cols_batched(cyb_ctx_t ctx, const std::vector<EyeDesc>& descs)
 {
     if (descs.empty()) return CYB_OK;
-    void* d = nullptr;
-    CYB_TRY(ctx->upload(descs.data(), sizeof(EyeDesc) * descs.size(), &d));
-    hipLaunchKernelGGL(eye_cols_kernel, dim3(64, (unsigned)descs.size()), dim3(256), 0, ctx->stream, static_cast<const EyeDesc*>(d));
+    std::vector<WorkList> wl(descs.size());
+    for (size_t b = 0; b < descs.size(); ++b) wl[b] = WorkList{descs[b].m > 0 ? (int64_t)descs[b].kc : 0, 8 * (int64_t)descs[b].m};
+    std::vector<WorkItem> items;
+    make_work_items(wl.data(), wl.size(), 1, items);
+    if (items.empty()) return CYB_OK;
+    const EyeDesc* d = nullptr;
+    const WorkItem* di = nullptr;
+    CYB_TRY(upload_with_items(ctx, descs, items, &d, &di));
+    hipLaunchKernelGGL(eye_cols_kernel, dim3((unsigned)items.size()), dim3(256), 0, ctx->stream, d, di);
     CYB_HIP(hipGetLastError());
     return CYB_OK;
 }
@@ -1983,7 +1998,7 @@
     }
     struct Step {
         GemmStaged s1, s2;
-        size_t off_sum = 0;
+        size_t off_sum = 0, off_items = 0;
         unsigned n_sum = 0;
     };
     std::vector<Step> steps;
@@ -2022,10 +2037,16 @@
             CYB_TRY(g1.stage(ctx, image, st.s1));
             CYB_TRY(g2.stage(ctx, image, st.s2));
             if (!sums.empty()) {
-                st.n_sum = (unsigned)sums.size();
+                std::vector<WorkList> wl(sums.size());
+                for (size_t b = 0; b < sums.size(); ++b) wl[b] = WorkList{(sums[b].n + 255) / 256, 8 * 256 * (int64_t)sums[b].ns};
+                std::vector<WorkItem> items;
+                make_work_items(wl.data(), wl.size(), 1, items);
+                st.n_sum = (unsigned)items.size();
                 st.off_sum = (image.size() + 255) / 256 * 256;
-                image.resize(st.off_sum + sizeof(SumDesc) * sums.size());
+                st.off_items = (st.off_sum + sizeof(SumDesc) * sums.size() + 255) / 256 * 256;
+                image.resize(st.off_items + sizeof(WorkItem) * items.size());
                 memcpy(image.data() + st.off_sum, sums.data(), sizeof(SumDesc) * sums.size());
+                memcpy(image.data() + st.off_items, items.data(), sizeof(WorkItem) * items.size());
             }
             steps.push_back(st);
         }
@@ -2035,8 +2056,9 @@
         for (const auto& st : steps) {
             CYB_TRY(gemm_launch_staged(ctx, st.s1, d_image));
             if (st.n_sum) {
-                hipLaunchKernelGGL(sum_partials_kernel, dim3(helper_grid_x(st.n_sum), st.n_sum), dim3(256), 0, ctx->stream,
-                                   reinterpret_cast<const SumDesc*>(static_cast<char*>(d_image) + st.off_sum));
+                hipLaunchKernelGGL(sum_partials_kernel, dim3(st.n_sum), dim3(256), 0, ctx->stream,
+                                   reinterpret_cast<const SumDesc*>(static_cast<char*>(d_image) + st.off_sum),
+                                   reinterpret_cast<const WorkItem*>(static_cast<char*>(d_image) + st.off_items));
                 CYB_HIP(hipGetLastError());
             }
             CYB_TRY(gemm_launch_staged(ctx, st.s2, d_image));
diff --git a/cyten_amd/csrc/common.h b/cyten_amd/csrc/common.h
--- a/cyten_amd/csrc/common.h
+++ b/cyten_amd/csrc/common.h
@@ -9,6 +9,7 @@
 #include <vector>
 
 #include "../../include/cyten_amd.h"
+#include "work_items.h"
 
 namespace cyb {
 
@@ -188,6 +189,20 @@
 int matrix_amax(cyb_ctx_t ctx, const std::vector<MatRef>& mats, std::vector<double>& amax);
 double range_scale(double amax);
 int scale_copy_batched(cyb_ctx_t ctx, const std::vector<ScaleJob>& jobs);
+template <class D>
+inline int upload_with_items(cyb_ctx_t ctx, const std::vector<D>& descs, const std::vector<WorkItem>& items, const D** d_descs,
+                             const WorkItem** d_items, const std::vector<WorkItem>* items2 = nullptr,
+                             const WorkItem** d_items2 = nullptr)
+{
+    void *a = nullptr, *b = nullptr, *c = nullptr;
+    CYB_TRY(upload_packed(ctx, {{descs.data(), sizeof(D) * descs.size(), &a},
+                                {items.data(), sizeof(WorkItem) * items.size(), &b},
+                                {items2 ? items2->data() : nullptr, items2 ? sizeof(WorkItem) * items2->size() : 0, &c}}));
+    *d_descs = static_cast<const D*>(a);
+    *d_items = static_cast<const WorkItem*>(b);
+    if (d_items2) *d_items2 = static_cast<const WorkItem*>(c);
+    return CYB_OK;
+}
 inline unsigned helper_grid_x(size_t n_lists)
 {
     const size_t g = 2048 / (n_lists ? n_lists : 1);
diff --git a/cyten_amd/csrc/scaling.hip b/cyten_amd/csrc/scaling.hip
--- a/cyten_amd/csrc/scaling.hip
+++ b/cyten_amd/csrc/scaling.hip
@@ -9,36 +9,44 @@
 #define GLOBAL_AS __attribute__((address_space(1)))
 typedef const GLOBAL_AS double* gcp;
 typedef GLOBAL_AS double* gp;
+typedef double dbl2 __attribute__((ext_vector_type(2)));
 
 struct AmaxDesc {
     const double* A;
     int64_t lda;
     int32_t m, n;
-    double* out;
 };
 
-__global__ void __launch_bounds__(256) matrix_amax_kernel(const AmaxDesc* __restrict__ descs)
+__global__ void __launch_bounds__(256) matrix_amax_kernel(const AmaxDesc* __restrict__ descs, const WorkItem* __restrict__ items,
+                                                          double* __restrict__ out)
 {
     __shared__ double red[4];
-    const AmaxDesc d = descs[blockIdx.y];
+    const WorkItem it = items[blockIdx.x];
+    const AmaxDesc d = descs[it.mat];
     gcp A = (gcp)d.A;
     double mx = 0.0;
     bool bad = false;
+    auto take = [&](double v) {
+        bad = bad || !(fabs(v) <= 1.7e308);
+        mx = fmax(mx, fabs(v));
+    };
     if (d.lda == d.n) {
-        const int64_t tot = (int64_t)d.m * d.n;
-        for (int64_t e = (int64_t)blockIdx.x * 256 + threadIdx.x; e < tot; e += (int64_t)gridDim.x * 256) {
-            const double v = A[e];
-            bad = bad || !(fabs(v) <= 1.7e308);
-            mx = fmax(mx, fabs(v));
+        gcp p = A + (int64_t)it.begin * d.n;
+        const int64_t tot = (int64_t)(it.end - it.begin) * d.n;
+        const int64_t head = (reinterpret_cast<uintptr_t>(d.A + (int64_t)it.begin * d.n) & 8) ? 1 : 0;
+        if (head && threadIdx.x == 0 && tot > 0) take(p[0]);
+        const int64_t n2 = tot > head ? (tot - head) / 2 : 0;
+        const GLOBAL_AS dbl2* p2 = (const GLOBAL_AS dbl2*)(p + head);
+        for (int64_t e = threadIdx.x; e < n2; e += 256) {
+            const dbl2 v = p2[e];
+            take(v.x);
+            take(v.y);
         }
+        if (threadIdx.x == 0 && head + 2 * n2 < tot) take(p[tot - 1]);
     } else {
-        for (int r = blockIdx.x; r < d.m; r += gridDim.x) {
+        for (int r = it.begin; r < it.end; ++r) {
             gcp row = A + (int64_t)r * d.lda;
-            for (int c = threadIdx.x; c < d.n; c += 256) {
-                const double v = row[c];
-                bad = bad || !(fabs(v) <= 1.7e308);
-                mx = fmax(mx, fabs(v));
-            }
+            for (int c = threadIdx.x; c < d.n; c += 256) take(row[c]);
         }
     }
     if (bad) mx = __builtin_nan("");
@@ -52,7 +60,7 @@
     if (threadIdx.x == 0) {
         double r = red[0];
         for (int w = 1; w < 4; ++w) r = (r != r || red[w] != red[w]) ? __builtin_nan("") : fmax(r, red[w]);
-        ((gp)d.out)[blockIdx.x] = r;
+        ((gp)out)[blockIdx.x] = r;
     }
 }
 
@@ -65,16 +73,14 @@
     double s;
 };
 
-__global__ void __launch_bounds__(256) scale_copy_kernel(const ScaleDesc* __restrict__ descs)
+__global__ void __launch_bounds__(256) scale_copy_kernel(const ScaleDesc* __restrict__ descs, const WorkItem* __restrict__ items)
 {
-    const ScaleDesc d = descs[blockIdx.y];
+    const WorkItem it = items[blockIdx.x];
+    const ScaleDesc d = descs[it.mat];
     gcp src = (gcp)d.src;
     gp dst = (gp)d.dst;
-    const int64_t tot = (int64_t)d.rows * d.cols;
-    for (int64_t e = (int64_t)blockIdx.x * 256 + threadIdx.x; e < tot; e += (int64_t)gridDim.x * 256) {
-        const int64_t r = e / d.cols, c = e % d.cols;
-        dst[r * d.ldd + c] = src[r * d.lds + c] * d.s;
-    }
+    for (int64_t r = it.begin; r < it.end; ++r)
+        for (int c = threadIdx.x; c < d.cols; c += 256) dst[r * d.ldd + c] = src[r * d.lds + c] * d.s;
 }
 
 }
@@ -84,25 +90,29 @@
     const size_t n = mats.size();
     amax.assign(n, 0.0);
     if (n == 0) return CYB_OK;
-    constexpr int kParts = 32;
+    constexpr int64_t kItems = 1024;
+    std::vector<AmaxDesc> ds(n);
+    std::vector<WorkList> wl(n);
+    for (size_t i = 0; i < n; ++i) {
+        ds[i] = AmaxDesc{mats[i].A, mats[i].lda, (int32_t)mats[i].m, (int32_t)mats[i].n};
+        wl[i] = WorkList{mats[i].n > 0 ? mats[i].m : 0, 8 * mats[i].n};
+    }
+    std::vector<WorkItem> items;
+    make_work_items(wl.data(), n, 1, items, kItems);
+    if (items.empty()) return CYB_OK;
     void* d_out = nullptr;
-    CYB_TRY(ctx->workspace(sizeof(double) * n * kParts, &d_out, 2));
-    std::vector<AmaxDesc> ds(n);
-    for (size_t i = 0; i < n; ++i)
-        ds[i] = AmaxDesc{mats[i].A, mats[i].lda, (int32_t)mats[i].m, (int32_t)mats[i].n, static_cast<double*>(d_out) + i * kParts};
-    void* d_ds = nullptr;
-    CYB_TRY(ctx->upload(ds.data(), sizeof(AmaxDesc) * n, &d_ds));
-    hipLaunchKernelGGL(matrix_amax_kernel, dim3(kParts, (unsigned)n), dim3(256), 0, ctx->stream, static_cast<const AmaxDesc*>(d_ds));
+    CYB_TRY(ctx->workspace(sizeof(double) * items.size(), &d_out, 2));
+    const AmaxDesc* d_ds = nullptr;
+    const WorkItem* d_it = nullptr;
+    CYB_TRY(upload_with_items(ctx, ds, items, &d_ds, &d_it));
+    hipLaunchKernelGGL(matrix_amax_kernel, dim3((unsigned)items.size()), dim3(256), 0, ctx->stream, d_ds, d_it, static_cast<double*>(d_out));
     CYB_HIP(hipGetLastError());
-    std::vector<double> parts(n * kParts);
+    std::vector<double> parts(items.size());
     CYB_TRY(ctx->d2h(parts.data(), d_out, sizeof(double) * parts.size()));
-    for (size_t i = 0; i < n; ++i) {
-        double r = 0.0;
-        for (int p = 0; p < kParts; ++p) {
-            const double v = parts[i * kParts + p];
-            r = (r != r || v != v) ? std::nan("") : std::max(r, v);
-        }
-        amax[i] = r;
+    for (size_t p = 0; p < items.size(); ++p) {
+        double& r = amax[(size_t)items[p].mat];
+        const double v = parts[p];
+        r = (r != r || v != v) ? std::nan("") : std::max(r, v);
     }
     return CYB_OK;
 }
@@ -122,9 +132,15 @@
     std::vector<ScaleDesc> ds(jobs.size());
     for (size_t i = 0; i < jobs.size(); ++i)
         ds[i] = ScaleDesc{jobs[i].src, jobs[i].lds, jobs[i].dst, jobs[i].ldd, (int32_t)jobs[i].rows, (int32_t)jobs[i].cols, jobs[i].s};
-    void* d_ds = nullptr;
-    CYB_TRY(ctx->upload(ds.data(), sizeof(ScaleDesc) * ds.size(), &d_ds));
-    hipLaunchKernelGGL(scale_copy_kernel, dim3(64, (unsigned)ds.size()), dim3(256), 0, ctx->stream, static_cast<const ScaleDesc*>(d_ds));
+    std::vector<WorkList> wl(ds.size());
+    for (size_t i = 0; i < ds.size(); ++i) wl[i] = WorkList{ds[i].cols > 0 ? (int64_t)ds[i].rows : 0, 8 * (int64_t)ds[i].cols};
+    std::vector<WorkItem> items;
+    make_work_items(wl.data(), wl.size(), 1, items);
+    if (items.empty()) return CYB_OK;
+    const ScaleDesc* d_ds = nullptr;
+    const WorkItem* d_it = nullptr;
+    CYB_TRY(upload_with_items(ctx, ds, items, &d_ds, &d_it));
+    hipLaunchKernelGGL(scale_copy_kernel, dim3((unsigned)items.size()), dim3(256), 0, ctx->stream, d_ds, d_it);
     CYB_HIP(hipGetLastError());
     return CYB_OK;
 }
diff --git a/cyten_amd/csrc/svd_jacobi.hip b/cyten_amd/csrc/svd_jacobi.hip
--- a/cyten_amd/csrc/svd_jacobi.hip
+++ b/cyten_amd/csrc/svd_jacobi.hip
@@ -24,16 +24,17 @@
     const double* shift;
 };
 
-__global__ void __launch_bounds__(256) prep_kernel(const PrepDesc* __restrict__ descs)
+__global__ void __launch_bounds__(256) prep_kernel(const PrepDesc* __restrict__ descs, const WorkItem* __restrict__ items)
 {
     __shared__ double tile[32][33];
-    const PrepDesc d = descs[blockIdx.y];
+    const WorkItem it = items[blockIdx.x];
+    const PrepDesc d = descs[it.mat];
     gcp A = (gcp)d.A;
     gp W = (gp)d.W;
     const int tx = threadIdx.x & 31, ty = threadIdx.x >> 5;
-    const int tiles_n = (d.n + 31) / 32, tiles_m = (d.m + 31) / 32;
+    const int tiles_n = (d.n + 31) / 32;
     const double shift = d.shift ? *(gcp)d.shift : 0.0;
-    for (int t = blockIdx.x; t < tiles_m * tiles_n; t += gridDim.x) {
+    for (int t = it.begin; t < it.end; ++t) {
         const int ti = t / tiles_n, tj = t % tiles_n;
         const int i0 = ti * 32, j0 = tj * 32;
         if (d.transpose) {
@@ -61,9 +62,9 @@
             }
         }
     }
-    if (d.J) {
+    if (d.J && it.begin == 0) {
         gp J = (gp)d.J;
-        for (int i = blockIdx.x * 256 + threadIdx.x; i < d.nvp; i += gridDim.x * 256) J[(int64_t)i * d.nvp + i] = 1.0;
+        for (int i = threadIdx.x; i < d.nvp; i += 256) J[(int64_t)i * d.nvp + i] = 1.0;
     }
 }
 
@@ -116,12 +117,13 @@
     const double* sig_lq = nullptr;
 };
 
-__global__ void __launch_bounds__(256) row_norm_kernel(const PostDesc* __restrict__ descs)
-{
-    const PostDesc d = descs[blockIdx.y];
+__global__ void __launch_bounds__(256) row_norm_kernel(const PostDesc* __restrict__ descs, const WorkItem* __restrict__ items)
+{
+    const WorkItem it = items[blockIdx.x];
+    const PostDesc d = descs[it.mat];
     gcp W = (gcp)d.W;
     const int lane = threadIdx.x & 63;
-    for (int j = blockIdx.x * 4 + (threadIdx.x >> 6); j < d.nv; j += gridDim.x * 4) {
+    for (int j = it.begin + (threadIdx.x >> 6); j < it.end; j += 4) {
         double s = 0.0;
         for (int c = lane; c < d.len; c += 64) {
             const double v = W[(int64_t)j * d.lenp + c];
@@ -136,52 +138,60 @@
     }
 }
 
-__global__ void __launch_bounds__(256) rank_kernel(const PostDesc* __restrict__ descs)
-{
-    constexpr int CH = 2048;
-    __shared__ double keys[CH];
-    const PostDesc d = descs[blockIdx.y];
+constexpr int RANK_CH = 128;
+struct RankItem {
+    int32_t mat, j0, k0, pad;
+};
+__global__ void __launch_bounds__(256) rank_count_kernel(const PostDesc* __restrict__ descs, const RankItem* __restrict__ items)
+{
+    __shared__ double keys[RANK_CH];
+    const RankItem it = items[blockIdx.x];
+    const PostDesc d = descs[it.mat];
+    gcp sig = (gcp)d.sig;
+    const int msk = d.cplx ? ~1 : ~0;
+    const int j = it.j0 + (int)threadIdx.x;
+    const bool mine = j < d.nv;
+    const double sj = mine ? sig[j & msk] : 0.0;
+    const int k0 = it.k0, kn = min(RANK_CH, d.nv - k0);
+    if ((int)threadIdx.x < kn) keys[threadIdx.x] = sig[(k0 + (int)threadIdx.x) & msk];
+    __syncthreads();
+    if (!mine) return;
+    int r = 0;
+    if (d.mode == 0) {
+        for (int k = 0; k < kn; ++k) {
+            const double sk = keys[k];
+            r += (sk > sj || (sk == sj && k0 + k < j)) ? 1 : 0;
+        }
+    } else {
+        for (int k = 0; k < kn; ++k) {
+            const double sk = keys[k];
+            r += (sk < sj || (sk == sj && k0 + k < j)) ? 1 : 0;
+        }
+    }
+    if (r) atomicAdd(&d.rank[j], r);
+}
+__global__ void __launch_bounds__(256) rank_write_kernel(const PostDesc* __restrict__ descs, const WorkItem* __restrict__ items)
+{
+    const WorkItem it = items[blockIdx.x];
+    const PostDesc d = descs[it.mat];
     gcp sig = (gcp)d.sig;
     const double shift = d.shift ? *(gcp)d.shift : 0.0;
     const int msk = d.cplx ? ~1 : ~0;
-    const int per = (d.nv + (int)gridDim.x * 256 - 1) / ((int)gridDim.x * 256);
-    for (int it = 0; it < per; ++it) {
-        const int j = (it * (int)gridDim.x + (int)blockIdx.x) * 256 + (int)threadIdx.x;
-        const bool mine = j < d.nv;
-        const double sj = mine ? sig[j & msk] : 0.0;
-        int r = 0;
-        for (int k0 = 0; k0 < d.nv; k0 += CH) {
-            const int kn = min(CH, d.nv - k0);
-            __syncthreads();
-            for (int k = threadIdx.x; k < kn; k += 256) keys[k] = sig[(k0 + k) & msk];
-            __syncthreads();
-            if (mine) {
-                if (d.mode == 0) {
-                    for (int k = 0; k < kn; ++k) {
-                        const double sk = keys[k];
-                        r += (sk > sj || (sk == sj && k0 + k < j)) ? 1 : 0;
-                    }
-                } else {
-                    for (int k = 0; k < kn; ++k) {
-                        const double sk = keys[k];
-                        r += (sk < sj || (sk == sj && k0 + k < j)) ? 1 : 0;
-                    }
-                }
-            }
-        }
-        if (mine) {
-            d.rank[j] = r;
-            d.S[r] = (d.mode == 0) ? sj : sj - shift;
-        }
-    }
-}
-
-__global__ void __launch_bounds__(256) write_factors_kernel(const PostDesc* __restrict__ descs)
+    for (int j = it.begin + (int)threadIdx.x; j < it.end; j += 256) {
+        const double sj = sig[j & msk];
+        d.S[d.rank[j]] = (d.mode == 0) ? sj : sj - shift;
+    }
+}
+
+__global__ void __launch_bounds__(256) write_factors_kernel(const PostDesc* __restrict__ descs, const WorkItem* __restrict__ col_items,
+                                                            const WorkItem* __restrict__ row_items, int n_col)
 {
     __shared__ double tile[32][33];
     __shared__ int rk[32];
     __shared__ double sc[32];
-    const PostDesc d = descs[blockIdx.y];
+    const bool col_side = (int)blockIdx.x < n_col;
+    const WorkItem it = col_side ? col_items[blockIdx.x] : row_items[(int)blockIdx.x - n_col];
+    const PostDesc d = descs[it.mat];
     gcp W = (gcp)d.W;
     gcp J = (gcp)d.J;
     const int tx = threadIdx.x & 31, ty = threadIdx.x >> 5;
@@ -197,10 +207,9 @@
     const int rsrc_ld = col_from_W ? d.nvp : d.lenp;
     const int r_cols = col_from_W ? d.nv : d.len;
 
-    const int tj = (d.nv + 31) / 32;
-    if (d.U) {
+    if (col_side) {
         const int ti_n = (c_rows + 31) / 32;
-        for (int t = blockIdx.x; t < tj * ti_n; t += gridDim.x) {
+        for (int t = it.begin; t < it.end; ++t) {
             const int j0 = (t / ti_n) * 32, i0 = (t % ti_n) * 32;
             __syncthreads();
             if (threadIdx.x < 32) {
@@ -231,8 +240,8 @@
             }
         }
     }
-    if (d.mode == 0 && d.Vh) {
-        for (int j = blockIdx.x; j < d.nv; j += gridDim.x) {
+    if (!col_side) {
+        for (int j = it.begin; j < it.end; ++j) {
             const int r = d.rank[j];
             double s = 1.0;
             if (!col_from_W) {
@@ -243,7 +252,7 @@
                 ((gp)d.Vh)[(int64_t)r * d.ldvh + c] = rsrc[(int64_t)j * rsrc_ld + c] * s;
         }
     }
-    if (d.mode == 0 && blockIdx.x == 0) {
+    if (d.mode == 0 && it.begin == 0 && (col_side || !d.U)) {
         __syncthreads();
         int cnt = 0;
         for (int j = threadIdx.x; j < d.nv; j += 256) cnt += (((gcp)d.sig)[j] <= thresh) ? 1 : 0;
@@ -345,6 +354,77 @@
 }
 
 inline int round_up(int x, int m) { return (x + m - 1) / m * m; }
+
+template <class D, class F>
+inline void row_items(const std::vector<D>& descs, F f, std::vector<WorkItem>& out)
+{
+    std::vector<WorkList> wl(descs.size());
+    for (size_t b = 0; b < descs.size(); ++b) wl[b] = f(descs[b]);
+    make_work_items(wl.data(), wl.size(), 4, out);
+}
+#define CYB_LAUNCH_ITEMS(kernel, n_items, ...)                                                                           \
+    do {                                                                                                                 \
+        if ((n_items) > 0) hipLaunchKernelGGL(kernel, dim3((unsigned)(n_items)), dim3(256), 0, ctx->stream, __VA_ARGS__); \
+    } while (0)
+
+struct PostDev {
+    const PostDesc* d = nullptr;
+    const WorkItem *rows = nullptr, *rw = nullptr, *col = nullptr, *row = nullptr;
+    const RankItem* rank = nullptr;
+    size_t n_rows = 0, n_rank = 0, n_rw = 0, n_col = 0, n_row = 0;
+};
+int upload_post(cyb_ctx_t ctx, const std::vector<PostDesc>& post, bool want_rows, bool want_rank, PostDev& out)
+{
+    std::vector<WorkItem> rows, rw, col, row;
+    std::vector<RankItem> rank;
+    if (want_rows) row_items(post, [](const PostDesc& q) { return WorkList{q.nv, 8 * (int64_t)q.len}; }, rows);
+    if (want_rank) {
+        for (size_t b = 0; b < post.size(); ++b)
+            for (int j0 = 0; j0 < post[b].nv; j0 += 256)
+                for (int k0 = 0; k0 < post[b].nv; k0 += RANK_CH) rank.push_back(RankItem{(int32_t)b, j0, k0, 0});
+        std::vector<WorkList> wl(post.size());
+        for (size_t b = 0; b < post.size(); ++b) wl[b] = WorkList{post[b].nv, 8};
+        make_work_items(wl.data(), wl.size(), 256, rw);
+        std::vector<WorkList> wc(post.size()), wr(post.size());
+        for (size_t b = 0; b < post.size(); ++b) {
+            const PostDesc& q = post[b];
+            const bool col_from_W = (q.mode == 1) || q.transposed;
+            const int c_rows = col_from_W ? q.len : q.nv, r_cols = col_from_W ? q.nv : q.len;
+            wc[b] = WorkList{q.U ? (int64_t)((q.nv + 31) / 32) * ((c_rows + 31) / 32) : 0, 8 * 32 * 32};
+            wr[b] = WorkList{(q.mode == 0 && q.Vh) ? q.nv : 0, 8 * (int64_t)r_cols};
+        }
+        make_work_items(wc.data(), wc.size(), 1, col);
+        make_work_items(wr.data(), wr.size(), 1, row);
+    }
+    void *a = nullptr, *b = nullptr, *c = nullptr, *e = nullptr, *f = nullptr, *g = nullptr;
+    CYB_TRY(upload_packed(ctx, {{post.data(), sizeof(PostDesc) * post.size(), &a},
+                                {rows.data(), sizeof(WorkItem) * rows.size(), &b},
+                                {rank.data(), sizeof(RankItem) * rank.size(), &c},
+                                {rw.data(), sizeof(WorkItem) * rw.size(), &e},
+                                {col.data(), sizeof(WorkItem) * col.size(), &f},
+                                {row.data(), sizeof(WorkItem) * row.size(), &g}}));
+    out.d = static_cast<const PostDesc*>(a);
+    out.rows = static_cast<const WorkItem*>(b);
+    out.rank = static_cast<const RankItem*>(c);
+    out.rw = static_cast<const WorkItem*>(e);
+    out.n_rows = rows.size();
+    out.n_rank = rank.size();
+    out.n_rw = rw.size();
+    out.col = static_cast<const WorkItem*>(f);
+    out.row = static_cast<const WorkItem*>(g);
+    out.n_col = col.size();
+    out.n_row = row.size();
+    return CYB_OK;
+}
+void launch_write_factors(cyb_ctx_t ctx, const PostDev& pd)
+{
+    CYB_LAUNCH_ITEMS(write_factors_kernel, pd.n_col + pd.n_row, pd.d, pd.col, pd.row, (int)pd.n_col);
+}
+void launch_rank(cyb_ctx_t ctx, const PostDev& pd)
+{
+    CYB_LAUNCH_ITEMS(rank_count_kernel, pd.n_rank, pd.d, pd.rank);
+    CYB_LAUNCH_ITEMS(rank_write_kernel, pd.n_rw, pd.d, pd.rw);
+}
 
 struct Layout {
     std::vector<JMat> mats;
@@ -474,26 +554,33 @@
         q.null_scale = 0.0;
         q.cplx = cplx ? 1 : 0;
     }
-    void* d_prep = nullptr;
-    CYB_TRY(ctx->upload(prep.data(), sizeof(PrepDesc) * prep.size(), &d_prep));
+    const PrepDesc* d_prep = nullptr;
+    const WorkItem* d_prep_items = nullptr;
+    std::vector<WorkItem> prep_items;
+    {
+        std::vector<WorkList> wl(prep.size());
+        for (size_t b = 0; b < prep.size(); ++b) wl[b] = WorkList{(int64_t)((prep[b].m + 31) / 32) * ((prep[b].n + 31) / 32), 8 * 32 * 32};
+        make_work_items(wl.data(), wl.size(), 1, prep_items);
+    }
+    CYB_TRY(upload_with_items(ctx, prep, prep_items, &d_prep, &d_prep_items));
     if (mode == 1) {
         void* d_nd = nullptr;
         CYB_TRY(ctx->upload(nd.data(), sizeof(NormDesc) * nd.size(), &d_nd));
         hipLaunchKernelGGL(fro_shift_kernel, dim3((unsigned)nmat), dim3(256), 0, st, static_cast<const NormDesc*>(d_nd));
     }
-    hipLaunchKernelGGL(prep_kernel, dim3(64, (unsigned)nmat), dim3(256), 0, st, static_cast<const PrepDesc*>(d_prep));
+    CYB_LAUNCH_ITEMS(prep_kernel, prep_items.size(), d_prep, d_prep_items);
     CYB_HIP(hipGetLastError());
     std::vector<int32_t> sweeps;
     const int jst = jacobi_orthogonalise(ctx, mats, 40, sweeps, cplx);
     if (info)
         for (int64_t b = 0; b < nmat; ++b) info[b] = sweeps[(size_t)b];
     if (jst != CYB_OK && jst != CYB_ERR_NOCONV) return jst;
-    void* d_post = nullptr;
-    CYB_TRY(ctx->upload(post.data(), sizeof(PostDesc) * post.size(), &d_post));
-    const PostDesc* dp = static_cast<const PostDesc*>(d_post);
-    hipLaunchKernelGGL(row_norm_kernel, dim3(helper_grid_x((size_t)nmat), (unsigned)nmat), dim3(256), 0, st, dp);
-    hipLaunchKernelGGL(rank_kernel, dim3(8, (unsigned)nmat), dim3(256), 0, st, dp);
-    hipLaunchKernelGGL(write_factors_kernel, dim3(helper_grid_x((size_t)nmat), (unsigned)nmat), dim3(256), 0, st, dp);
+    PostDev pd;
+    CYB_TRY(upload_post(ctx, post, true, true, pd));
+    const PostDesc* dp = pd.d;
+    CYB_LAUNCH_ITEMS(row_norm_kernel, pd.n_rows, dp, pd.rows);
+    launch_rank(ctx, pd);
+    launch_write_factors(ctx, pd);
     if (mode == 0) hipLaunchKernelGGL(complete_null_kernel, dim3((unsigned)nmat), dim3(256), 0, st, dp);
     CYB_HIP(hipGetLastError());
     if (info) CYB_HIP(hipStreamSynchronize(st));
@@ -511,25 +598,27 @@
     int32_t kp, k, cnt, pad;
     const int32_t* col;
 };
-__global__ void __launch_bounds__(256) gather_rows_kernel(const RowsDesc* __restrict__ descs)
-{
-    const RowsDesc d = descs[blockIdx.y];
+__global__ void __launch_bounds__(256) gather_rows_kernel(const RowsDesc* __restrict__ descs, const WorkItem* __restrict__ items)
+{
+    const WorkItem it = items[blockIdx.x];
+    const RowsDesc d = descs[it.mat];
     gcp W = (gcp)d.W;
     gp buf = (gp)d.buf;
     const int lane = threadIdx.x & 63;
-    for (int c = blockIdx.x * 4 + (threadIdx.x >> 6); c < d.cnt; c += gridDim.x * 4) {
+    for (int c = it.begin + (threadIdx.x >> 6); c < it.end; c += 4) {
         const int j = d.idx[c];
         const double inv = 1.0 / ((gcp)d.sig)[j];
         for (int i = lane; i < d.k; i += 64) buf[(int64_t)c * d.k + i] = W[(int64_t)j * d.kp + i] * inv;
     }
 }
-__global__ void __launch_bounds__(256) scatter_rows_kernel(const RowsDesc* __restrict__ descs)
-{
-    const RowsDesc d = descs[blockIdx.y];
+__global__ void __launch_bounds__(256) scatter_rows_kernel(const RowsDesc* __restrict__ descs, const WorkItem* __restrict__ items)
+{
+    const WorkItem it = items[blockIdx.x];
+    const RowsDesc d = descs[it.mat];
     gp W = (gp)d.W;
     gcp buf = (gcp)d.buf;
     const int lane = threadIdx.x & 63;
-    for (int c = blockIdx.x * 4 + (threadIdx.x >> 6); c < d.cnt; c += gridDim.x * 4) {
+    for (int c = it.begin + (threadIdx.x >> 6); c < it.end; c += 4) {
         const int j = d.idx[c];
         const int cc = d.col ? d.col[c] : c;
         for (int i = lane; i < d.k; i += 64) W[(int64_t)j * d.kp + i] = buf[(int64_t)cc * d.k + i];
@@ -543,13 +632,14 @@
     int64_t L;
     int32_t kp, k;
 };
-__global__ void __launch_bounds__(256) j_to_cq_kernel(const JcqDesc* __restrict__ descs)
-{
-    const JcqDesc d = descs[blockIdx.y];
+__global__ void __launch_bounds__(256) j_to_cq_kernel(const JcqDesc* __restrict__ descs, const WorkItem* __restrict__ items)
+{
+    const WorkItem it = items[blockIdx.x];
+    const JcqDesc d = descs[it.mat];
     gcp J = (gcp)d.J;
     gp Cq = (gp)d.Cq;
     const int lane = threadIdx.x & 63;
-    for (int j = blockIdx.x * 4 + (threadIdx.x >> 6); j < d.k; j += gridDim.x * 4) {
+    for (int j = it.begin + (threadIdx.x >> 6); j < it.end; j += 4) {
         const int r = d.rank[j];
         for (int i = lane; i < d.k; i += 64) Cq[(int64_t)r * d.L + i] = J[(int64_t)j * d.kp + i];
     }
@@ -564,13 +654,14 @@
     int32_t cnt, ncols;
     int32_t mode, pad;
 };
-__global__ void __launch_bounds__(256) row_move_kernel(const RowMoveDesc* __restrict__ descs)
-{
-    const RowMoveDesc d = descs[blockIdx.y];
+__global__ void __launch_bounds__(256) row_move_kernel(const RowMoveDesc* __restrict__ descs, const WorkItem* __restrict__ items)
+{
+    const WorkItem it = items[blockIdx.x];
+    const RowMoveDesc d = descs[it.mat];
     gcp src = (gcp)d.src;
     gp dst = (gp)d.dst;
     const int lane = threadIdx.x & 63;
-    for (int g = blockIdx.x * 4 + (threadIdx.x >> 6); g < d.cnt; g += gridDim.x * 4) {
+    for (int g = it.begin + (threadIdx.x >> 6); g < it.end; g += 4) {
         const int j = d.idx[g];
         if (d.mode == 0) {
             for (int c = lane; c < d.ncols; c += 64) dst[(int64_t)g * d.ldd + c] = src[(int64_t)j * d.lds + c];
@@ -581,13 +672,14 @@
         }
     }
 }
-__global__ void __launch_bounds__(256) j_scatter_kernel(const RowMoveDesc* __restrict__ descs)
-{
-    const RowMoveDesc d = descs[blockIdx.y];
+__global__ void __launch_bounds__(256) j_scatter_kernel(const RowMoveDesc* __restrict__ descs, const WorkItem* __restrict__ items)
+{
+    const WorkItem it = items[blockIdx.x];
+    const RowMoveDesc d = descs[it.mat];
     gcp src = (gcp)d.src;
     gp dst = (gp)d.dst;
     const int lane = threadIdx.x & 63;
-    for (int g = blockIdx.x * 4 + (threadIdx.x >> 6); g < d.cnt; g += gridDim.x * 4) {
+    for (int g = it.begin + (threadIdx.x >> 6); g < it.end; g += 4) {
         const int j = d.idx[g];
         for (int h = lane; h < d.cnt; h += 64) dst[(int64_t)j * d.ldd + d.idx[h]] = src[(int64_t)g * d.lds + h];
     }
@@ -633,13 +725,14 @@
 };
 constexpr double JREC_BOUND = 2e-11;
 constexpr int JREC_NB = 128;
-__global__ void __launch_bounds__(256) lq_pack_kernel(const LqDesc* __restrict__ descs)
-{
-    const LqDesc d = descs[blockIdx.y];
+__global__ void __launch_bounds__(256) lq_pack_kernel(const LqDesc* __restrict__ descs, const WorkItem* __restrict__ items)
+{
+    const WorkItem it = items[blockIdx.x];
+    const LqDesc d = descs[it.mat];
     gcp Jc = (gcp)d.Jc;
     gp C = (gp)d.Cq2;
     const int lane = threadIdx.x & 63;
-    for (int i = blockIdx.x * 4 + (threadIdx.x >> 6); i < d.k; i += gridDim.x * 4) {
+    for (int i = it.begin + (threadIdx.x >> 6); i < it.end; i += 4) {
         for (int c = lane; c < d.k; c += 64) {
             double v;
             if (i < d.r0) {
@@ -650,13 +743,14 @@
         }
     }
 }
-__global__ void __launch_bounds__(256) lq_rows_kernel(const LqDesc* __restrict__ descs)
-{
-    const LqDesc d = descs[blockIdx.y];
+__global__ void __launch_bounds__(256) lq_rows_kernel(const LqDesc* __restrict__ descs, const WorkItem* __restrict__ items)
+{
+    const WorkItem it = items[blockIdx.x];
+    const LqDesc d = descs[it.mat];
     gcp Wq = (gcp)d.Wq;
     gp Jc = (gp)d.Jc;
     const int lane = threadIdx.x & 63;
-    for (int i = blockIdx.x * 4 + (threadIdx.x >> 6); i < d.r0; i += gridDim.x * 4) {
+    for (int i = it.begin + (threadIdx.x >> 6); i < it.end; i += 4) {
         double s = 0.0;
         for (int c = lane; c < d.r0; c += 64) {
             const double v = Wq[(int64_t)i * d.rp + c];
@@ -679,15 +773,16 @@
         }
     }
 }
-__global__ void __launch_bounds__(256) jrec_check_kernel(const LqDesc* __restrict__ descs)
-{
-    const LqDesc d = descs[blockIdx.y];
+__global__ void __launch_bounds__(256) jrec_check_kernel(const LqDesc* __restrict__ descs, const WorkItem* __restrict__ items)
+{
+    const WorkItem it = items[blockIdx.x];
+    const LqDesc d = descs[it.mat];
     if (!d.jrec) return;
     gcp G = (gcp)d.G;
     const int lane = threadIdx.x & 63;
     double mx = 0.0;
     bool nan = false;
-    for (int i = blockIdx.x * 4 + (threadIdx.x >> 6); i < d.r0; i += gridDim.x * 4) {
+    for (int i = it.begin + (threadIdx.x >> 6); i < it.end; i += 4) {
         for (int c = i / JREC_NB * JREC_NB + lane; c < d.r0; c += 64) {
             const double v = fabs(G[(int64_t)i * d.r0 + c] - (c == i ? 1.0 : 0.0));
             nan = nan || !(v == v);
@@ -703,12 +798,12 @@
         if (!(mx <= JREC_BOUND)) *(gp)d.bad = 1.0;
     }
 }
-__global__ void __launch_bounds__(256) lq_check_kernel(const LqDesc* __restrict__ descs)
-{
-    const LqDesc d = descs[blockIdx.y];
+__global__ void __launch_bounds__(256) lq_check_kernel(const LqDesc* __restrict__ descs, const WorkItem* __restrict__ items)
+{
+    const WorkItem it = items[blockIdx.x];
+    const LqDesc d = descs[it.mat];
     gcp Jc = (gcp)d.Jc;
     const int lane = threadIdx.x & 63;
-    const int wid = blockIdx.x * 4 + (threadIdx.x >> 6), nw = gridDim.x * 4;
     for (int i0 = 0; i0 < d.r0; i0 += 64) {
         bool fl = false;
         if (i0 + lane < d.r0) {
@@ -720,7 +815,7 @@
             const int i = i0 + __ffsll((long long)msk) - 1;
             msk &= msk - 1;
             double worst = 0.0;
-            for (int j = wid; j < d.r0; j += nw) {
+            for (int j = it.begin + (threadIdx.x >> 6); j < it.end; j += 4) {
                 if (j == i) continue;
                 double t = 0.0;
                 for (int c = lane; c < d.r0; c += 64) t = fma(Jc[(int64_t)i * d.rp + c], Jc[(int64_t)j * d.rp + c], t);
@@ -732,13 +827,14 @@
         }
     }
 }
-__global__ void __launch_bounds__(256) lq_unpack_kernel(const LqDesc* __restrict__ descs)
-{
-    const LqDesc d = descs[blockIdx.y];
+__global__ void __launch_bounds__(256) lq_unpack_kernel(const LqDesc* __restrict__ descs, const WorkItem* __restrict__ items)
+{
+    const WorkItem it = items[blockIdx.x];
+    const LqDesc d = descs[it.mat];
     gcp C = (gcp)d.Cq2;
     gp Wc = (gp)d.Wc;
     const int lane = threadIdx.x & 63;
-    for (int i = blockIdx.x * 4 + (threadIdx.x >> 6); i < d.r0; i += gridDim.x * 4) {
+    for (int i = it.begin + (threadIdx.x >> 6); i < it.end; i += 4) {
         const double sg = ((gcp)d.sig2)[i];
         const double sm = d.cplx ? fmax(sg, ((gcp)d.sig2)[i ^ 1]) : sg;
         double f = sm * sm > d.thr2 ? sg : 0.0;
@@ -755,12 +851,14 @@
 static int launch_row_moves(cyb_ctx_t ctx, const std::vector<RowMoveDesc>& v, bool jscatter = false)
 {
     if (v.empty()) return CYB_OK;
-    void* d = nullptr;
-    CYB_TRY(ctx->upload(v.data(), sizeof(RowMoveDesc) * v.size(), &d));
-    if (jscatter)
-        hipLaunchKernelGGL(j_scatter_kernel, dim3(64, (unsigned)v.size()), dim3(256), 0, ctx->stream, static_cast<const RowMoveDesc*>(d));
-    else
-        hipLaunchKernelGGL(row_move_kernel, dim3(helper_grid_x(v.size()), (unsigned)v.size()), dim3(256), 0, ctx->stream, static_cast<const RowMoveDesc*>(d));
+    std::vector<WorkItem> items;
+    row_items(v, [&](const RowMoveDesc& m) { return WorkList{m.cnt, 8 * (int64_t)(jscatter ? m.cnt : m.ncols)}; }, items);
+    if (items.empty()) return CYB_OK;
+    const RowMoveDesc* d = nullptr;
+    const WorkItem* di = nullptr;
+    CYB_TRY(upload_with_items(ctx, v, items, &d, &di));
+    if (jscatter) CYB_LAUNCH_ITEMS(j_scatter_kernel, items.size(), d, di);
+    else CYB_LAUNCH_ITEMS(row_move_kernel, items.size(), d, di);
     CYB_HIP(hipGetLastError());
     return CYB_OK;
 }
@@ -923,13 +1021,11 @@
         q.null_scale = 1.0;
         q.cplx = cplx ? 1 : 0;
     }
-    void* d_post = nullptr;
-    const PostDesc* dpost = nullptr;
+    PostDev pd;
     std::vector<double> h_sig(sig_bytes / sizeof(double));
     auto sig_of = [&](const Lay& l) { return h_sig.data() + (l.sig - sig_begin) / sizeof(double); };
-    CYB_TRY(ctx->upload(post.data(), sizeof(PostDesc) * post.size(), &d_post));
-    dpost = static_cast<const PostDesc*>(d_post);
-    hipLaunchKernelGGL(row_norm_kernel, dim3(helper_grid_x((size_t)nmat), (unsigned)nmat), dim3(256), 0, st, dpost);
+    CYB_TRY(upload_post(ctx, post, true, false, pd));
+    CYB_LAUNCH_ITEMS(row_norm_kernel, pd.n_rows, pd.d, pd.rows);
     CYB_HIP(hipGetLastError());
     CYB_TRY(ctx->d2h(h_sig.data(), base + sig_begin, sig_bytes));
     {
@@ -1071,11 +1167,14 @@
         jst = jacobi_orthogonalise(ctx, jm, 40, sweeps, cplx);
         if (jst != CYB_OK && jst != CYB_ERR_NOCONV) return jst;
         if (!qm3.empty()) {
-            void* d = nullptr;
-            CYB_TRY(ctx->upload(lqd.data(), sizeof(LqDesc) * lqd.size(), &d));
-            const LqDesc* dl = static_cast<const LqDesc*>(d);
-            hipLaunchKernelGGL(lq_pack_kernel, dim3(64, (unsigned)lqd.size()), dim3(256), 0, st, dl);
-            hipLaunchKernelGGL(lq_rows_kernel, dim3(64, (unsigned)lqd.size()), dim3(256), 0, st, dl);
+            const LqDesc* dl = nullptr;
+            const WorkItem *di = nullptr, *di2 = nullptr;
+            std::vector<WorkItem> it_a, it_b;
+            row_items(lqd, [](const LqDesc& q) { return WorkList{q.k, 8 * (int64_t)q.k}; }, it_a);
+            row_items(lqd, [](const LqDesc& q) { return WorkList{q.r0, 8 * (int64_t)q.r0}; }, it_b);
+            CYB_TRY(upload_with_items(ctx, lqd, it_a, &dl, &di, &it_b, &di2));
+            CYB_LAUNCH_ITEMS(lq_pack_kernel, it_a.size(), dl, di);
+            CYB_LAUNCH_ITEMS(lq_rows_kernel, it_b.size(), dl, di2);
             if (!jrec_blocks.empty()) {
                 int64_t tiles = 0;
                 for (int b : jrec_blocks) tiles += (int64_t)((lay[(size_t)b].r0 + 127) / 128) * ((lay[(size_t)b].r0 + 127) / 128);
@@ -1093,15 +1192,16 @@
                 }
                 CYB_TRY(g_rec.launch(ctx));
                 CYB_TRY(g_chk.launch(ctx));
-                CYB_TRY(ctx->upload(lqd.data(), sizeof(LqDesc) * lqd.size(), &d));
-                dl = static_cast<const LqDesc*>(d);
-                hipLaunchKernelGGL(jrec_check_kernel, dim3(16, (unsigned)lqd.size()), dim3(256), 0, st, dl);
-            }
-            hipLaunchKernelGGL(lq_check_kernel, dim3(helper_grid_x(lqd.size()), (unsigned)lqd.size()), dim3(256), 0, st, dl);
+                row_items(lqd, [](const LqDesc& q) { return WorkList{q.jrec ? q.r0 : 0, 8 * (int64_t)q.r0}; }, it_a);
+                CYB_TRY(upload_with_items(ctx, lqd, it_a, &dl, &di, &it_b, &di2));
+                CYB_LAUNCH_ITEMS(jrec_check_kernel, it_a.size(), dl, di);
+            }
+            CYB_LAUNCH_ITEMS(lq_check_kernel, it_b.size(), dl, di2);
             CYB_HIP(hipGetLastError());
             CYB_TRY(bqr_apply_q(ctx, qm3, tg3));
-            CYB_TRY(ctx->upload(lqd.data(), sizeof(LqDesc) * lqd.size(), &d));
-            hipLaunchKernelGGL(lq_unpack_kernel, dim3(64, (unsigned)lqd.size()), dim3(256), 0, st, static_cast<const LqDesc*>(d));
+            row_items(lqd, [](const LqDesc& q) { return WorkList{q.r0, 8 * (int64_t)q.kp}; }, it_a);
+            CYB_TRY(upload_with_items(ctx, lqd, it_a, &dl, &di));
+            CYB_LAUNCH_ITEMS(lq_unpack_kernel, it_a.size(), dl, di);
             CYB_HIP(hipGetLastError());
         }
         return CYB_OK;
@@ -1155,9 +1255,8 @@
         CYB_TRY(launch_row_moves(ctx, sj, true));
     }
     for (int64_t b = 0; b < nmat; ++b) post[(size_t)b].sig_lq = lay[(size_t)b].lq ? dp(lay[(size_t)b].sigo) : nullptr;
-    CYB_TRY(ctx->upload(post.data(), sizeof(PostDesc) * post.size(), &d_post));
-    dpost = static_cast<const PostDesc*>(d_post);
-    hipLaunchKernelGGL(row_norm_kernel, dim3(helper_grid_x((size_t)nmat), (unsigned)nmat), dim3(256), 0, st, dpost);
+    CYB_TRY(upload_post(ctx, post, true, false, pd));
+    CYB_LAUNCH_ITEMS(row_norm_kernel, pd.n_rows, pd.d, pd.rows);
     CYB_HIP(hipGetLastError());
     CYB_TRY(ctx->d2h(h_sig.data(), base + sig_begin, sig_bytes));
     {
@@ -1228,31 +1327,34 @@
                 scat.push_back(RowsDesc{dp(l.W), dp(l.sig), reinterpret_cast<const int32_t*>(base + l.idx) + c.r, dp(l.Cn), l.kp, l.k, c.q, 0, nullptr});
             }
             if (!gath.empty()) {
-                void* d = nullptr;
-                CYB_TRY(ctx->upload(gath.data(), sizeof(RowsDesc) * gath.size(), &d));
-                hipLaunchKernelGGL(gather_rows_kernel, dim3(64, (unsigned)gath.size()), dim3(256), 0, st,
-                                   static_cast<const RowsDesc*>(d));
+                const RowsDesc* d = nullptr;
+                const WorkItem* di = nullptr;
+                std::vector<WorkItem> items;
+                row_items(gath, [](const RowsDesc& q) { return WorkList{q.cnt, 8 * (int64_t)q.k}; }, items);
+                CYB_TRY(upload_with_items(ctx, gath, items, &d, &di));
+                CYB_LAUNCH_ITEMS(gather_rows_kernel, items.size(), d, di);
                 CYB_HIP(hipGetLastError());
                 CYB_TRY(bqr_factor(ctx, qm2));
             }
             CYB_TRY(eye_cols_batched(ctx, eyes));
             if (!tg2.empty()) CYB_TRY(bqr_apply_q(ctx, qm2, tg2));
-            void* d = nullptr;
             if (!cols_all.empty()) {
                 void* d_cols = nullptr;
                 CYB_TRY(ctx->upload(cols_all.data(), sizeof(int32_t) * cols_all.size(), &d_cols));
                 for (const auto& pr : lq_scat) scat[pr.first].col = static_cast<const int32_t*>(d_cols) + pr.second;
             }
-            CYB_TRY(ctx->upload(scat.data(), sizeof(RowsDesc) * scat.size(), &d));
-            hipLaunchKernelGGL(scatter_rows_kernel, dim3(64, (unsigned)scat.size()), dim3(256), 0, st,
-                               static_cast<const RowsDesc*>(d));
+            const RowsDesc* d = nullptr;
+            const WorkItem* di = nullptr;
+            std::vector<WorkItem> items;
+            row_items(scat, [](const RowsDesc& q) { return WorkList{q.cnt, 8 * (int64_t)q.k}; }, items);
+            CYB_TRY(upload_with_items(ctx, scat, items, &d, &di));
+            CYB_LAUNCH_ITEMS(scatter_rows_kernel, items.size(), d, di);
             CYB_HIP(hipGetLastError());
         }
     }
-    CYB_TRY(ctx->upload(post.data(), sizeof(PostDesc) * post.size(), &d_post));
-    dpost = static_cast<const PostDesc*>(d_post);
-    hipLaunchKernelGGL(rank_kernel, dim3(8, (unsigned)nmat), dim3(256), 0, st, dpost);
-    hipLaunchKernelGGL(write_factors_kernel, dim3(helper_grid_x((size_t)nmat), (unsigned)nmat), dim3(256), 0, st, dpost);
+    CYB_TRY(upload_post(ctx, post, false, true, pd));
+    launch_rank(ctx, pd);
+    launch_write_factors(ctx, pd);
     CYB_HIP(hipGetLastError());
     std::vector<JcqDesc> jc;
     std::vector<BqrTarget> tg;
@@ -1267,9 +1369,12 @@
             x_out.push_back(XposeDesc{dp(l.Cq), sd[b].Vh, l.L, sd[b].ldvh, l.k, l.n, 0, 0, 1, 0});
     }
     {
-        void* d = nullptr;
-        CYB_TRY(ctx->upload(jc.data(), sizeof(JcqDesc) * jc.size(), &d));
-        hipLaunchKernelGGL(j_to_cq_kernel, dim3(helper_grid_x((size_t)nmat), (unsigned)nmat), dim3(256), 0, st, static_cast<const JcqDesc*>(d));
+        const JcqDesc* d = nullptr;
+        const WorkItem* di = nullptr;
+        std::vector<WorkItem> items;
+        row_items(jc, [](const JcqDesc& q) { return WorkList{q.k, 8 * (int64_t)q.k}; }, items);
+        CYB_TRY(upload_with_items(ctx, jc, items, &d, &di));
+        CYB_LAUNCH_ITEMS(j_to_cq_kernel, items.size(), d, di);
         CYB_HIP(hipGetLastError());
     }
     CYB_TRY(bqr_apply_q(ctx, qm, tg));
diff --git a/cyten_amd/csrc/truncation.hip b/cyten_amd/csrc/truncation.hip
--- a/cyten_amd/csrc/truncation.hip
+++ b/cyten_amd/csrc/truncation.hip
@@ -54,6 +54,40 @@
     }
     if (total) *total = all;
     return base + inc - v;
+}
+
+constexpr int RK_T = 256, RK_CH = 1024;
+__global__ void __launch_bounds__(RK_T) truncate_rank_kernel(const SDesc* __restrict__ descs, int n_sectors, int n,
+                                                             double* __restrict__ s_all, double* __restrict__ gkey, int* __restrict__ cnt)
+{
+    __shared__ double ck[RK_CH];
+    auto key_at = [&](int e, double* val) {
+        int lo = 0, hi = n_sectors - 1;
+        while (lo < hi) {
+            const int mid = (lo + hi + 1) >> 1;
+            if (descs[mid].offset <= e) lo = mid;
+            else hi = mid - 1;
+        }
+        const SDesc d = descs[lo];
+        const double v = d.S[e - d.offset];
+        *val = v;
+        return d.w * (v * v);
+    };
+    const int tid = threadIdx.x;
+    const int k0 = blockIdx.y * RK_CH, kn = min(RK_CH, n - k0);
+    double v;
+    for (int k = tid; k < kn; k += RK_T) ck[k] = key_at(k0 + k, &v);
+    __syncthreads();
+    const int e = blockIdx.x * RK_T + tid;
+    if (e >= n) return;
+    const double ka = key_at(e, &v);
+    if (blockIdx.y == 0) {
+        s_all[e] = v;
+        gkey[e] = ka;
+    }
+    int r = 0;
+    for (int k = 0; k < kn; ++k) r += key_less(ck[k], k0 + k, ka, e) ? 1 : 0;
+    cnt[(size_t)blockIdx.y * n + e] = r;
 }
 
 template <bool BIG>
@@ -74,7 +108,7 @@
     __shared__ double dtot[NT / 64];
     __shared__ int s_cut;
     const int tid = threadIdx.x;
-    for (int s = 0; s < n_sectors; ++s) {
+    for (int s = 0; BIG && s < n_sectors; ++s) {
         const SDesc d = descs[s];
         for (int64_t e = tid; e < d.n; e += NT) {
             const double v = d.S[e];
@@ -83,7 +117,7 @@
             idx[d.offset + e] = (int)(d.offset + e);
         }
     }
-    for (int e = n + tid; e < n2; e += NT) {
+    for (int e = (BIG ? n : 0) + tid; e < n2; e += NT) {
         key[e] = __builtin_huge_val();
         idx[e] = e;
     }
@@ -98,15 +132,14 @@
         }
     };
     if (!BIG) {
-        for (int k = 2; k <= n2; k <<= 1) {
-            for (int j = k >> 1; j > 0; j >>= 1) {
-                for (int t = tid; t < n2 / 2; t += NT) {
-                    const int e = ((t & ~(j - 1)) << 1) | (t & (j - 1));
-                    cmpx(key, idx, e, e + j, (e & k) == 0);
-                }
-                __syncthreads();
-            }
-        }
+        const int n_ch = (n + RK_CH - 1) / RK_CH;
+        for (int e = tid; e < n; e += NT) {
+            int r = 0;
+            for (int c = 0; c < n_ch; ++c) r += gidx[(size_t)c * n + e];
+            key[r] = gkey[e];
+            idx[r] = e;
+        }
+        __syncthreads();
     } else {
         auto chunk_steps = [&](int base, int k, int jmax) {
             for (int e = tid; e < NMAX; e += NT) {
@@ -257,7 +290,8 @@
     if (big) n2 = std::max(n2, 2 * NMAX);
     const size_t off_key = (sizeof(double) * (size_t)n + 255) & ~(size_t)255;
     const size_t off_idx = off_key + sizeof(double) * (size_t)n2, off_good = off_idx + sizeof(int) * (size_t)n2;
-    CYB_TRY(ctx->workspace(big ? off_good + (size_t)n2 : sizeof(double) * (size_t)n, &ws, 2));
+    const unsigned n_ch = (unsigned)((n + RK_CH - 1) / RK_CH);
+    CYB_TRY(ctx->workspace(big ? off_good + (size_t)n2 : off_idx + sizeof(int) * (size_t)n * n_ch, &ws, 2));
     Opts o{opts->chi_max, opts->chi_min, opts->degeneracy_tol, opts->trunc_cut, opts->svd_min, opts->has_svd_min,
            opts->minimize_error};
     char* w8 = static_cast<char*>(ws);
@@ -266,10 +300,14 @@
                            (int)n_sectors, (int)n, n2, o, static_cast<double*>(ws), keep_idx_dev, mask_dev, result_dev,
                            reinterpret_cast<double*>(w8 + off_key), reinterpret_cast<int*>(w8 + off_idx),
                            reinterpret_cast<unsigned char*>(w8 + off_good));
-    else
+    else {
+        hipLaunchKernelGGL(truncate_rank_kernel, dim3((unsigned)((n + RK_T - 1) / RK_T), n_ch), dim3(RK_T), 0, ctx->stream,
+                           static_cast<const SDesc*>(d_descs), (int)n_sectors, (int)n, static_cast<double*>(ws),
+                           reinterpret_cast<double*>(w8 + off_key), reinterpret_cast<int*>(w8 + off_idx));
         hipLaunchKernelGGL(truncate_select_kernel<false>, dim3(1), dim3(NT), 0, ctx->stream, static_cast<const SDesc*>(d_descs),
                            (int)n_sectors, (int)n, n2, o, static_cast<double*>(ws), keep_idx_dev, mask_dev, result_dev,
-                           (double*)nullptr, (int*)nullptr, (unsigned char*)nullptr);
+                           reinterpret_cast<double*>(w8 + off_key), reinterpret_cast<int*>(w8 + off_idx), (unsigned char*)nullptr);
+    }
     CYB_HIP(hipGetLastError());
     return CYB_OK;
 }
diff --git a/cyten_amd/csrc/work_items.h b/cyten_amd/csrc/work_items.h
--- /dev/null
+++ b/cyten_amd/csrc/work_items.h
@@ -0,0 +1,47 @@
+#pragma once
+#include <cstddef>
+#include <cstdint>
+#include <vector>
+
+namespace cyb {
+
+struct WorkItem {
+    int32_t mat;
+    int32_t begin, end;
+    int32_t pad;
+};
+
+struct WorkList {
+    int64_t units, unit_bytes;
+};
+
+constexpr int64_t kWorkItems = 2048;
+
+inline void make_work_items(const WorkList* lists, size_t n_lists, int64_t gran, std::vector<WorkItem>& out,
+                            int64_t n_items = kWorkItems)
+{
+    out.clear();
+    if (gran < 1) gran = 1;
+    if (n_items < 1) n_items = 1;
+    long double total = 0.0L;
+    for (size_t b = 0; b < n_lists; ++b)
+        if (lists[b].units > 0) total += (long double)lists[b].units * (long double)(lists[b].unit_bytes > 0 ? lists[b].unit_bytes : 1);
+    const long double target = total / (long double)n_items;
+    for (size_t b = 0; b < n_lists; ++b) {
+        const int64_t u = lists[b].units;
+        if (u <= 0) continue;
+        const long double ub = (long double)(lists[b].unit_bytes > 0 ? lists[b].unit_bytes : 1);
+        long double perf = target / ub;
+        int64_t per = perf >= (long double)u ? u : (int64_t)perf;
+        if ((long double)per < perf) ++per;
+        per = (per + gran - 1) / gran * gran;
+        if (per < gran) per = gran;
+        if (per > u) per = u;
+        for (int64_t r = 0; r < u; r += per) {
+            const int64_t e = r + per < u ? r + per : u;
+            out.push_back(WorkItem{(int32_t)b, (int32_t)r, (int32_t)e, 0});
+        }
+    }
+}
+
+}
```

Result: slower. 5400 (-1.2%).
